# dwofk/fast-depth

Hardware: AMD Instinct MI355X
Metric: frames/sec (224x224) MobileNet-NNConv5dw-skipadd inference forward (higher is better)
Workload: dtype f32; 1 GPU; configs[1]: MobileNet-NNConv5(dw)+skipadd unpruned, batch=32 per GPU, 224x224 fp32 inference forward, inputs resident in HBM; batch_per_gpu=32, global_batch=32, parallelism=frames sharded over 1 GPU(s), no collective, rccl_ranks=0, input_batches_in_rotation=8

## Files before the change

### fast-depth_amd/csrc/fd_api.hip

```cpp
#include "fd_kernels_f32.h"
#include "fd_kernels_gemm16_f32.h"
#include "fd_kernels_h16.h"
#include "fd_kernels_gemm16_h16.h"
#include "fd_kernels_dwpw_f32.h"
#include "fd_kernels_dw5p.h"
#include "fd_kernels_dwt.h"
#include "fd_kernels_dws.h"
#include "fd_kernels_dwb.h"
#include "fd_kernels_conv.h"
#include "../../include/fastdepth_hip.h"
#include "fd_tuning.h"

#include <algorithm>
#include <cstdarg>
#include <cstdio>
#include <cstdlib>
#include <cstring>
#include <string>
#include <type_traits>
#include <vector>

#ifndef FD_EMU
#include <hip/hip_ext.h>
#endif

#define FD_DEFINE_HOST_STATE
#include "fd_host_common.h"
#include "fd_plan_select.h"
#include "fd_infer_launch.h"
#include "fd_plan_build.h"


extern "C" {

void fd_tuning_next(uint32_t mask) { fd_hs().tune_next = mask; }

const char *fd_last_error(void) { return fd_hs().err.c_str(); }
#ifndef FD_SOURCE_HASH
#define FD_SOURCE_HASH "unstamped"
#endif
const char *fd_version(void) { return "fastdepth_hip 0.5 (gfx950; inference f32/f16/bf16, train step f32/bf16; sources " FD_SOURCE_HASH ")"; }

int fd_plan_create(const fd_layer_desc *layers, int32_t n_layers, int32_t batch, int32_t height, int32_t width,
                   int32_t dtype, uint32_t flags, fd_plan **out_plan)
{
    const uint32_t tune = fd_take_tuning();
    if (!layers || !out_plan || n_layers <= 0) return fail(FD_ERR_INVALID, "null/empty layer list");
    if (batch <= 0 || height <= 0 || width <= 0 || height % 32 || width % 32)
        return fail(FD_ERR_INVALID, "batch must be > 0 and height/width positive multiples of 32 (got %d, %dx%d)", batch, height, width);
    if (dtype != FD_F32 && dtype != FD_F16 && dtype != FD_BF16) return fail(FD_ERR_INVALID, "unknown dtype %d", dtype);
    if (flags & ~FD_PLAN_ALL_FLAGS) return fail(FD_ERR_INVALID, "unknown plan flag bits 0x%x", flags & ~FD_PLAN_ALL_FLAGS);
    if (tune & ~FD_TUNE_ALL) return fail(FD_ERR_INVALID, "unknown tuning bits 0x%x", tune & ~FD_TUNE_ALL);
    fd_plan *p = new fd_plan();
    p->B = batch; p->H = height; p->W = width; p->dtype = dtype; p->flags = flags; p->tune = tune;
    p->layers.resize(n_layers);
    size_t woff = 0;
    int rc = plan_layers(p, layers, &woff);
    if (rc) { delete p; return rc; }
    p->weights_bytes = woff;
    plan_fuse_epilogues(p);
    plan_fuse_units(p);
    plan_fuse_head_h16(p);
    plan_arena(p, woff);
    plan_describe(p);
    *out_plan = p;
    return FD_OK;
}

void fd_plan_destroy(fd_plan *plan) { delete plan; }

size_t fd_plan_workspace_bytes(const fd_plan *plan) { return plan ? plan->ws_bytes : 0; }

int fd_plan_bind_workspace(fd_plan *plan, void *device_ptr, size_t bytes)
{
    if (!plan || !device_ptr) return fail(FD_ERR_INVALID, "null plan/workspace");
    if (bytes < plan->ws_bytes) return fail(FD_ERR_INVALID, "workspace too small: %zu < %zu", bytes, plan->ws_bytes);
    if (reinterpret_cast<uintptr_t>(device_ptr) % 256) return fail(FD_ERR_INVALID, "workspace must be 256-byte aligned");
    plan->ws = static_cast<unsigned char *>(device_ptr);
    plan->packed = false;
    return FD_OK;
}

int fd_plan_pack_weights(fd_plan *plan, const fd_layer_params *params, int32_t n_layers, float bn_eps, void *stream)
{
    if (!plan || !params) return fail(FD_ERR_INVALID, "null plan/params");
    if (!plan->ws) return fail(FD_ERR_STATE, "bind a workspace before packing weights");
    if (n_layers != (int)plan->layers.size()) return fail(FD_ERR_INVALID, "expected %zu layer parameter sets", plan->layers.size());
    hipStream_t s = static_cast<hipStream_t>(stream);
    for (int i = 0; i < n_layers; ++i) {
        const Layer &L = plan->layers[i];
        const fd_layer_params &q = params[i];
        if (!q.conv_weight || !q.bn_weight || !q.bn_bias || !q.bn_mean || !q.bn_var) return fail(FD_ERR_INVALID, "layer %d: null parameter pointer", i);
        if (L.conv) {
            const size_t cesz = plan->dtype == FD_F32 ? 4 : 2;
            const int kk = L.d.ksize * L.d.ksize, cpad = L.cv_ktpt * fd_conv_bk(cesz);
            const long upto = (long)(L.w_bytes / cesz);
            float *cb = reinterpret_cast<float *>(plan->ws + L.b_off);
            if (plan->dtype == FD_F16)
                hipLaunchKernelGGL((fd_conv_pack<fd_half>), dim3(ceil_div(upto, 256)), dim3(256), 0, s, q.conv_weight, q.bn_weight, q.bn_var, bn_eps, reinterpret_cast<fd_half *>(plan->ws + L.w_off), L.d.cout, L.d.cin, kk, cpad, upto);
            else if (plan->dtype == FD_BF16)
                hipLaunchKernelGGL((fd_conv_pack<fd_bf16>), dim3(ceil_div(upto, 256)), dim3(256), 0, s, q.conv_weight, q.bn_weight, q.bn_var, bn_eps, reinterpret_cast<fd_bf16 *>(plan->ws + L.w_off), L.d.cout, L.d.cin, kk, cpad, upto);
            else
                hipLaunchKernelGGL((fd_conv_pack<float>), dim3(ceil_div(upto, 256)), dim3(256), 0, s, q.conv_weight, q.bn_weight, q.bn_var, bn_eps, reinterpret_cast<float *>(plan->ws + L.w_off), L.d.cout, L.d.cin, kk, cpad, upto);
            int rcc = check_launch("fd_conv_pack");
            if (rcc) return rcc;
            hipLaunchKernelGGL(fd_dwt_fold_bias, dim3(ceil_div(L.d.cout, 256)), dim3(256), 0, s, q.bn_weight, q.bn_bias, q.bn_mean, q.bn_var, bn_eps, cb, L.d.cout);
            rcc = check_launch("fd_dwt_fold_bias");
            if (rcc) return rcc;
            continue;
        }
        const int inner = (int)(L.w_elems / L.d.cout);
        const int transpose = (L.d.op == FD_OP_PW) ? 0 : 1;
        const int pitch = transpose ? inner : (L.w_pitch ? L.w_pitch : inner);
        const long total = std::max<long>((long)L.d.cout * std::max(inner, pitch), L.d.cout);
        float *bptr = reinterpret_cast<float *>(plan->ws + L.b_off);
        if (L.pw_packed_t && plan->dtype == FD_F16)
            hipLaunchKernelGGL((fd_pack_fold<fd_half>), dim3(ceil_div(total, 256)), dim3(256), 0, s, q.conv_weight, q.bn_weight, q.bn_bias, q.bn_mean, q.bn_var, bn_eps,
                               reinterpret_cast<fd_half *>(plan->ws + L.w_off), bptr, L.d.cout, inner, transpose, pitch);
        else if (L.pw_packed_t)
            hipLaunchKernelGGL((fd_pack_fold<fd_bf16>), dim3(ceil_div(total, 256)), dim3(256), 0, s, q.conv_weight, q.bn_weight, q.bn_bias, q.bn_mean, q.bn_var, bn_eps,
                               reinterpret_cast<fd_bf16 *>(plan->ws + L.w_off), bptr, L.d.cout, inner, transpose, pitch);
        else
            hipLaunchKernelGGL((fd_pack_fold<float>), dim3(ceil_div(total, 256)), dim3(256), 0, s, q.conv_weight, q.bn_weight, q.bn_bias, q.bn_mean, q.bn_var, bn_eps,
                               reinterpret_cast<float *>(plan->ws + L.w_off), bptr, L.d.cout, inner, transpose, pitch);
        int rc = check_launch("fd_pack_fold");
        if (rc) return rc;
        if (L.dwt || L.dws || L.pws || L.dwb || L.pwb) {
            hipLaunchKernelGGL(fd_dwt_fold_bias, dim3(ceil_div(L.d.cout, 256)), dim3(256), 0, s, q.bn_weight, q.bn_bias, q.bn_mean, q.bn_var, bn_eps, bptr, L.d.cout);
            rc = check_launch("fd_dwt_fold_bias");
            if (rc) return rc;
        }
        if (L.dw5_cl) {
            const float *wf = reinterpret_cast<const float *>(plan->ws + L.w_off);
            unsigned *wpk = reinterpret_cast<unsigned *>(plan->ws + L.wpk_off);
            if (plan->dtype == FD_F16) hipLaunchKernelGGL((fd_pack_dw5_pairs<fd_half>), dim3(ceil_div(30L * L.d.cin, 256)), dim3(256), 0, s, wf, wpk, L.d.cin);
            else hipLaunchKernelGGL((fd_pack_dw5_pairs<fd_bf16>), dim3(ceil_div(30L * L.d.cin, 256)), dim3(256), 0, s, wf, wpk, L.d.cin);
            rc = check_launch("fd_pack_dw5_pairs");
            if (rc) return rc;
        }
    }
    plan->packed = true;
    return FD_OK;
}

int fd_forward(fd_plan *plan, const void *x_nchw, void *y, void *stream)
{
    if (!plan || !x_nchw || !y) return fail(FD_ERR_INVALID, "null argument");
    if (!plan->ws || !plan->packed) return fail(FD_ERR_STATE, "plan needs a bound workspace and packed weights");
    if (misaligned(x_nchw, 16)) return fail(FD_ERR_INVALID, "x must be 16-byte aligned");
    if (misaligned(y, 8)) return fail(FD_ERR_INVALID, "y must be 8-byte aligned");
    hipStream_t s = static_cast<hipStream_t>(stream);
    for (size_t i = 0; i < plan->layers.size(); ++i) {
        const Layer &L = plan->layers[i];
        if (L.skipped || L.fused_into >= 0) continue;
        fd_hs().trace_layer = (int)i;
        int rc = run_layer(plan, L, static_cast<const float *>(x_nchw), static_cast<float *>(y), s);
        if (rc) return rc;
    }
    fd_hs().trace_layer = -1;
    return FD_OK;
}

#include "fd_bundle_impl.h"

int fd_plan_shape(const fd_plan *plan, int32_t *batch, int32_t *height, int32_t *width, int32_t *dtype)
{
    if (!plan) return fail(FD_ERR_INVALID, "null plan");
    if (batch) *batch = plan->B;
    if (height) *height = plan->H;
    if (width) *width = plan->W;
    if (dtype) *dtype = plan->dtype;
    return FD_OK;
}

#include "fd_trace_impl.h"

int fd_layer_output(const fd_plan *plan, int32_t layer, const void **device_ptr, int32_t *n, int32_t *h, int32_t *w, int32_t *c)
{
    if (!plan || layer < 0 || layer >= (int)plan->layers.size()) return fail(FD_ERR_INVALID, "bad layer index");
    if (!(plan->flags & FD_PLAN_KEEP_ACTIVATIONS)) return fail(FD_ERR_STATE, "plan was not created with FD_PLAN_KEEP_ACTIVATIONS");
    const Layer &L = plan->layers[layer];
    if (L.to_output) return fail(FD_ERR_STATE, "the last layer writes the caller's output buffer");
    if (L.skipped) return fail(FD_ERR_STATE, "layer %d is fused into its consumer and has no stored output", layer);
    if (!plan->ws) return fail(FD_ERR_STATE, "no workspace bound");
    if (device_ptr) *device_ptr = plan->ws + L.out_off;
    if (n) *n = plan->B;
    if (h) *h = L.out_h;
    if (w) *w = L.out_w;
    if (c) *c = L.d.cout;
    return FD_OK;
}

int32_t fd_plan_num_kernels(const fd_plan *plan) { return plan ? (int32_t)plan->layers.size() : 0; }

const char *fd_plan_kernel_info(const fd_plan *plan, int32_t layer)
{
    if (!plan || layer < 0 || layer >= (int)plan->layers.size()) return "";
    return plan->layers[layer].info.c_str();
}

const char *fd_plan_kernel_symbol(const fd_plan *plan, int32_t layer)
{
    if (!plan || layer < 0 || layer >= (int)plan->layers.size()) return "";
    return plan->layers[layer].sym.c_str();
}

double fd_plan_algorithmic_bytes(const fd_plan *plan) { return plan ? plan->alg_bytes : 0.0; }
double fd_plan_algorithmic_flops(const fd_plan *plan) { return plan ? plan->alg_flops : 0.0; }

int fd_plan_layer_stats(const fd_plan *plan, int32_t layer, double *algorithmic_bytes, double *algorithmic_flops)
{
    if (!plan || layer < 0 || layer >= (int)plan->layers.size()) return fail(FD_ERR_INVALID, "bad layer index");
    const Layer &L = plan->layers[layer];
    double b = (L.skipped || L.fused_into >= 0) ? 0.0 : L.alg_bytes, f = (L.skipped || L.fused_into >= 0) ? 0.0 : L.alg_flops;
    if (L.fused_dw >= 0) { b += plan->layers[L.fused_dw].alg_bytes; f += plan->layers[L.fused_dw].alg_flops; }
    if (L.fuse_next_dw >= 0) { b += plan->layers[L.fuse_next_dw].alg_bytes; f += plan->layers[L.fuse_next_dw].alg_flops; }
    if (L.fuse_head >= 0) { b += plan->layers[L.fuse_head].alg_bytes; f += plan->layers[L.fuse_head].alg_flops; }
    if (algorithmic_bytes) *algorithmic_bytes = b;
    if (algorithmic_flops) *algorithmic_flops = f;
    return FD_OK;
}

int fd_plan_layer_traffic(const fd_plan *plan, int32_t layer, double *needed_bytes)
{
    if (!plan || layer < 0 || layer >= (int)plan->layers.size() || !needed_bytes) return fail(FD_ERR_INVALID, "bad layer index / null output");
    const Layer &L = plan->layers[layer];
    const double esz = plan->dtype == FD_F32 ? 4.0 : 2.0;
    auto out_b = [&](const Layer &X) { return (double)plan->B * X.out_h * X.out_w * X.d.cout * (X.to_output ? 4.0 : esz); };
    double b = (L.skipped || L.fused_into >= 0) ? 0.0 : L.alg_bytes;
    if (L.fused_dw >= 0) { const Layer &D = plan->layers[L.fused_dw]; b += D.alg_bytes - 2.0 * out_b(D); }
    if (L.fuse_next_dw >= 0) {
        const Layer &D = plan->layers[L.fuse_next_dw];
        b += D.alg_bytes - ((plan->flags & FD_PLAN_KEEP_ACTIVATIONS) ? 1.0 : 2.0) * out_b(L);
    }
    if (L.fuse_head >= 0) { const Layer &H = plan->layers[L.fuse_head]; b += H.alg_bytes - 2.0 * out_b(L); }
    *needed_bytes = b;
    return FD_OK;
}

}
```

### fast-depth_amd/csrc/fd_device.h

```cpp
#pragma once
#ifdef FD_EMU
#include "hipemu.h"
#else
#include <hip/hip_runtime.h>
#define FD_DYN_SMEM(name) extern __shared__ __attribute__((aligned(16))) unsigned char name[]
#endif

#ifdef FD_EMU
inline void fd_glds16(const float *g, float *lds_wave_base) { memcpy((char *)lds_wave_base + hipemu::lane_id() * 16, g, 16); }
template <int N> inline void fd_wait_vmcnt() {}
#define FD_SCHED_FENCE() ((void)0)
#define FD_UNIFORM(x) (x)
#define FD_OPAQUE(x) ((void)0)
#define FD_SCALAR_PTR(p) ((void)0)
template <typename P> inline P *fd_uniform_ptr(P *p) { return p; }
inline void fd_store_u32_sbase(char *base, unsigned off, unsigned v) { memcpy(base + off, &v, 4); }
inline void fd_block_barrier_lds() { __syncthreads(); }
inline void fd_block_barrier() { __syncthreads(); }
inline void fd_wave_lds_fence() { __syncthreads(); }
#else
__device__ __forceinline__ void fd_glds16(const float *g, float *lds_wave_base)
{
    __builtin_amdgcn_global_load_lds((const __attribute__((address_space(1))) void *)g,
                                     (__attribute__((address_space(3))) void *)lds_wave_base, 16, 0, 0);
}
template <int N> __device__ __forceinline__ void fd_wait_vmcnt() { asm volatile("s_waitcnt vmcnt(%0)" ::"n"(N) : "memory"); }
#define FD_SCHED_FENCE() __builtin_amdgcn_sched_barrier(0)
#define FD_UNIFORM(x) __builtin_amdgcn_readfirstlane(x)
#define FD_OPAQUE(x) asm volatile("" : "+v"(x))
#define FD_SCALAR_PTR(p) asm volatile("" : "+s"(p))
__device__ __forceinline__ void fd_store_u32_sbase(char *base, unsigned off, unsigned v)
{
    asm volatile("global_store_dword %0, %1, %2" : : "v"(off), "v"(v), "s"(base) : "memory");
}
template <typename P> __device__ __forceinline__ P *fd_uniform_ptr(P *p)
{
    const unsigned long long v = reinterpret_cast<unsigned long long>(p);
    const unsigned lo = __builtin_amdgcn_readfirstlane((unsigned)v), hi = __builtin_amdgcn_readfirstlane((unsigned)(v >> 32));
    return reinterpret_cast<P *>(((unsigned long long)hi << 32) | lo);
}
__device__ __forceinline__ void fd_wave_lds_fence() { asm volatile("s_waitcnt lgkmcnt(0)" ::: "memory"); }
__device__ __forceinline__ void fd_block_barrier() { __builtin_amdgcn_s_barrier(); }
__device__ __forceinline__ void fd_block_barrier_lds() { asm volatile("s_waitcnt lgkmcnt(0)" ::: "memory"); __builtin_amdgcn_s_barrier(); }
#endif

#ifdef FD_EMU
inline void fd_wave_fence() { (void)__shfl(0.0f, 0); }
inline void fd_wave_dma_wait() { (void)__shfl(0.0f, 0); }
#else
__device__ __forceinline__ void fd_wave_fence() { asm volatile("s_waitcnt lgkmcnt(0)" ::: "memory"); }
__device__ __forceinline__ void fd_wave_dma_wait() { asm volatile("s_waitcnt vmcnt(0)" ::: "memory"); }
#endif

struct fd_blk3 { int x, y, z; };
__device__ __forceinline__ fd_blk3 fd_xcd_map(unsigned b, unsigned per, unsigned nimg)
{
    const unsigned grp = b / (8u * per), rem = b - grp * 8u * per;
    const unsigned m = nimg - grp * 8u < 8u ? nimg - grp * 8u : 8u;
    fd_blk3 r;
    r.z = (int)(grp * 8u + rem % m); r.x = (int)(rem / m); r.y = 0;
    return r;
}
__device__ __forceinline__ fd_blk3 fd_xcd_image_map()
{
    const unsigned gx = gridDim.x, gy = gridDim.y;
    fd_blk3 r = fd_xcd_map(blockIdx.x + gx * (blockIdx.y + gy * blockIdx.z), gx * gy, gridDim.z);
    r.y = (int)((unsigned)r.x / gx); r.x -= r.y * (int)gx;
    return r;
}
__device__ __forceinline__ fd_blk3 fd_xcd_image_map2()
{
    return fd_xcd_map(blockIdx.x + gridDim.x * blockIdx.y, gridDim.x, gridDim.y);
}

template <int N> struct fd_int { static constexpr int value = N; };

__device__ __forceinline__ float fd_row_stride4_sum(float v)
{
#ifdef FD_EMU
    v += __shfl_xor(v, 8); v += __shfl_xor(v, 4);
#else
    v += __builtin_bit_cast(float, __builtin_amdgcn_update_dpp(0, __builtin_bit_cast(int, v), 0x128, 0xF, 0xF, true));
    v += __builtin_bit_cast(float, __builtin_amdgcn_update_dpp(0, __builtin_bit_cast(int, v), 0x124, 0xF, 0xF, true));
#endif
    return v;
}

typedef float fd_f32x4 __attribute__((ext_vector_type(4)));
typedef float fd_f32x2 __attribute__((ext_vector_type(2)));
typedef float fd_f32x16 __attribute__((ext_vector_type(16)));

#define FD_ACT_NONE_ 0
#define FD_ACT_RELU_ 1
#define FD_ACT_RELU6_ 2

__device__ __forceinline__ float fd_relu_clamp(float v, float hi) { return __builtin_elementwise_minimum(__builtin_elementwise_maximum(v, 0.0f), hi); }
template <int ACT>
__device__ __forceinline__ float fd_act(float v)
{
    if (ACT == FD_ACT_RELU_) return __builtin_elementwise_maximum(v, 0.0f);
    if (ACT == FD_ACT_RELU6_) return fd_relu_clamp(v, 6.0f);
    return v;
}
template <int ACT>
__device__ __forceinline__ float fd_act_raw(float v)
{
#ifdef FD_EMU
    return fd_act<ACT>(v);
#else
    float r = v;
    if (ACT == FD_ACT_RELU_) asm("v_maximum3_f32 %0, %1, 0, 0" : "=v"(r) : "v"(v));
    if (ACT == FD_ACT_RELU6_) { const float six = 6.0f; asm("v_maximum3_f32 %0, %1, 0, 0\n\tv_minimum3_f32 %0, %0, %2, %2" : "=&v"(r) : "v"(v), "s"(six)); }
    return r;
#endif
}
template <int ACT>
__device__ __forceinline__ fd_f32x4 fd_act4(fd_f32x4 v)
{
    fd_f32x4 r;
    r.x = fd_act<ACT>(v.x); r.y = fd_act<ACT>(v.y); r.z = fd_act<ACT>(v.z); r.w = fd_act<ACT>(v.w);
    return r;
}
__device__ __forceinline__ fd_f32x4 fd_ld4(const float *p) { return *reinterpret_cast<const fd_f32x4 *>(p); }
__device__ __forceinline__ void fd_st4(float *p, fd_f32x4 v) { *reinterpret_cast<fd_f32x4 *>(p) = v; }

typedef float fd_f32x2_t __attribute__((ext_vector_type(2)));
typedef _Float16 fd_half;
struct fd_bf16 { unsigned short v; };
typedef _Float16 fd_f16x4 __attribute__((ext_vector_type(4)));
typedef _Float16 fd_f16x8 __attribute__((ext_vector_type(8)));
typedef unsigned short fd_u16x4 __attribute__((ext_vector_type(4)));
typedef unsigned short fd_u16x8 __attribute__((ext_vector_type(8)));

__device__ __forceinline__ float fd_bf16_to_f32(unsigned short b) { return __builtin_bit_cast(float, (unsigned)b << 16); }
#ifdef FD_EMU
__device__ __forceinline__ unsigned short fd_f32_to_bf16(float f)
{
    unsigned u = __builtin_bit_cast(unsigned, f);
    if ((u & 0x7fffffffu) > 0x7f800000u) return (unsigned short)((u >> 16) | 0x40u);
    u += 0x7fffu + ((u >> 16) & 1u);
    return (unsigned short)(u >> 16);
}
__device__ __forceinline__ unsigned fd_f32x2_to_bf16x2(float a, float b) { return (unsigned)fd_f32_to_bf16(a) | ((unsigned)fd_f32_to_bf16(b) << 16); }
#else
__device__ __forceinline__ unsigned short fd_f32_to_bf16(float f) { return __builtin_bit_cast(unsigned short, (__bf16)f); }
__device__ __forceinline__ unsigned fd_f32x2_to_bf16x2(float a, float b)
{
    typedef __bf16 fd_bf16x2_hw __attribute__((ext_vector_type(2)));
    const fd_f32x2_t v = {a, b};
    return __builtin_bit_cast(unsigned, __builtin_convertvector(v, fd_bf16x2_hw));
}
#endif
__device__ __forceinline__ fd_f32x4 fd_ld4(const fd_half *p)
{
    const fd_f16x4 h = *reinterpret_cast<const fd_f16x4 *>(p);
    fd_f32x4 r = {(float)h.x, (float)h.y, (float)h.z, (float)h.w};
    return r;
}
__device__ __forceinline__ void fd_st4(fd_half *p, fd_f32x4 v)
{
    fd_f16x4 h = {(_Float16)v.x, (_Float16)v.y, (_Float16)v.z, (_Float16)v.w};
    *reinterpret_cast<fd_f16x4 *>(p) = h;
}
__device__ __forceinline__ fd_f32x4 fd_ld4(const fd_bf16 *p)
{
    const fd_u16x4 h = *reinterpret_cast<const fd_u16x4 *>(p);
    fd_f32x4 r = {fd_bf16_to_f32(h.x), fd_bf16_to_f32(h.y), fd_bf16_to_f32(h.z), fd_bf16_to_f32(h.w)};
    return r;
}
__device__ __forceinline__ void fd_st4(fd_bf16 *p, fd_f32x4 v)
{
    typedef unsigned fd_u32x2 __attribute__((ext_vector_type(2)));
    const fd_u32x2 h = {fd_f32x2_to_bf16x2(v.x, v.y), fd_f32x2_to_bf16x2(v.z, v.w)};
    *reinterpret_cast<fd_u32x2 *>(p) = h;
}
__device__ __forceinline__ fd_f32x4 fd_ldraw4(const float *p) { return *reinterpret_cast<const fd_f32x4 *>(p); }
#ifdef FD_EMU
inline fd_u16x4 fd_lds_read_tr16(const void *p)
{
    unsigned short o[4];
    hipemu_lds_read_tr16_b64(p, o);
    fd_u16x4 r = {o[0], o[1], o[2], o[3]};
    return r;
}
#else
__device__ __forceinline__ fd_u16x4 fd_lds_read_tr16(const void *p)
{
    typedef short fd_s16x4_hw __attribute__((ext_vector_type(4)));
    const fd_s16x4_hw v = __builtin_amdgcn_ds_read_tr16_b64_v4i16((__attribute__((address_space(3))) fd_s16x4_hw *)(p));
    return __builtin_bit_cast(fd_u16x4, v);
}
#endif
__device__ __forceinline__ fd_u16x4 fd_ldraw4(const fd_half *p) { return *reinterpret_cast<const fd_u16x4 *>(p); }
__device__ __forceinline__ fd_u16x4 fd_ldraw4(const fd_bf16 *p) { return *reinterpret_cast<const fd_u16x4 *>(p); }
__device__ __forceinline__ fd_f32x4 fd_cvt4(float, fd_f32x4 r) { return r; }
__device__ __forceinline__ fd_f32x4 fd_cvt4(fd_half, fd_u16x4 r)
{
    const fd_f16x4 h = __builtin_bit_cast(fd_f16x4, r);
    fd_f32x4 v = {(float)h.x, (float)h.y, (float)h.z, (float)h.w};
    return v;
}
__device__ __forceinline__ fd_f32x4 fd_cvt4(fd_bf16, fd_u16x4 r)
{
    fd_f32x4 v = {fd_bf16_to_f32(r.x), fd_bf16_to_f32(r.y), fd_bf16_to_f32(r.z), fd_bf16_to_f32(r.w)};
    return v;
}
__device__ __forceinline__ float fd_ld1(const float *p) { return *p; }
__device__ __forceinline__ float fd_ld1(const fd_half *p) { return (float)*p; }
__device__ __forceinline__ float fd_ld1(const fd_bf16 *p) { return fd_bf16_to_f32(p->v); }
__device__ __forceinline__ void fd_st1(float *p, float v) { *p = v; }
__device__ __forceinline__ void fd_st1(fd_half *p, float v) { *p = (_Float16)v; }
__device__ __forceinline__ void fd_st1(fd_bf16 *p, float v) { p->v = fd_f32_to_bf16(v); }
struct fd_px_walk {
    int iy, ix, dy, dx, w;
    __device__ __forceinline__ fd_px_walk(int start, int step, int w_) : w(w_) { iy = start / w_; ix = start - iy * w_; dy = step / w_; dx = step - dy * w_; }
    __device__ __forceinline__ void next() { ix += dx; iy += dy; if (ix >= w) { ix -= w; ++iy; } }
};
__device__ __forceinline__ fd_f32x4 fd_zero4() { fd_f32x4 z = {0.f, 0.f, 0.f, 0.f}; return z; }

#ifdef FD_EMU
inline unsigned fd_mul24(unsigned a, unsigned b) { return (a & 0xffffffu) * (b & 0xffffffu); }
#else
__device__ __forceinline__ unsigned fd_mul24(unsigned a, unsigned b) { return __umul24(a, b); }
#endif
__device__ __forceinline__ long fd_nhwc(int n, int H, int y, int W, int x, int C, int c)
{
    return (long)n * H * W * C + (long)(fd_mul24(fd_mul24((unsigned)y, (unsigned)W) + (unsigned)x, (unsigned)C) + (unsigned)c);
}

typedef float fd_f32x8 __attribute__((ext_vector_type(8)));
__device__ __forceinline__ fd_f32x8 fd_zero8() { fd_f32x8 z = {0.f, 0.f, 0.f, 0.f, 0.f, 0.f, 0.f, 0.f}; return z; }
__device__ __forceinline__ fd_f32x8 fd_cvt8(fd_half, fd_u16x8 r)
{
    const fd_f16x8 h = __builtin_bit_cast(fd_f16x8, r);
    fd_f32x8 v = {(float)h[0], (float)h[1], (float)h[2], (float)h[3], (float)h[4], (float)h[5], (float)h[6], (float)h[7]};
    return v;
}
__device__ __forceinline__ fd_f32x8 fd_cvt8(fd_bf16, fd_u16x8 r)
{
    typedef unsigned fd_u32x4_ __attribute__((ext_vector_type(4)));
    const fd_u32x4_ d = __builtin_bit_cast(fd_u32x4_, r);
    fd_f32x8 v = {__builtin_bit_cast(float, d[0] << 16), __builtin_bit_cast(float, d[0] & 0xffff0000u), __builtin_bit_cast(float, d[1] << 16), __builtin_bit_cast(float, d[1] & 0xffff0000u),
                  __builtin_bit_cast(float, d[2] << 16), __builtin_bit_cast(float, d[2] & 0xffff0000u), __builtin_bit_cast(float, d[3] << 16), __builtin_bit_cast(float, d[3] & 0xffff0000u)};
    return v;
}
__device__ __forceinline__ fd_u16x8 fd_pack8v(fd_half, fd_f32x8 v)
{
    fd_f16x8 h = {(_Float16)v[0], (_Float16)v[1], (_Float16)v[2], (_Float16)v[3], (_Float16)v[4], (_Float16)v[5], (_Float16)v[6], (_Float16)v[7]};
    return __builtin_bit_cast(fd_u16x8, h);
}
__device__ __forceinline__ fd_u16x8 fd_pack8v(fd_bf16, fd_f32x8 v)
{
    typedef unsigned fd_u32x4_ __attribute__((ext_vector_type(4)));
    const fd_u32x4_ r = {fd_f32x2_to_bf16x2(v[0], v[1]), fd_f32x2_to_bf16x2(v[2], v[3]), fd_f32x2_to_bf16x2(v[4], v[5]), fd_f32x2_to_bf16x2(v[6], v[7])};
    return __builtin_bit_cast(fd_u16x8, r);
}
__device__ __forceinline__ fd_u16x8 fd_sum8(fd_half, fd_u16x8 a, fd_u16x8 b)
{
    return __builtin_bit_cast(fd_u16x8, __builtin_bit_cast(fd_f16x8, a) + __builtin_bit_cast(fd_f16x8, b));
}
__device__ __forceinline__ fd_u16x8 fd_sum8(fd_bf16, fd_u16x8 a, fd_u16x8 b) { return fd_pack8v(fd_bf16{}, fd_cvt8(fd_bf16{}, a) + fd_cvt8(fd_bf16{}, b)); }
template <int ACT>
__device__ __forceinline__ fd_f32x8 fd_act4(fd_f32x8 v)
{
    fd_f32x8 r;
#pragma unroll
    for (int j = 0; j < 8; ++j) r[j] = fd_act<ACT>(v[j]);
    return r;
}
__device__ __forceinline__ fd_f32x4 fd_round4(float, fd_f32x4 v) { return v; }
__device__ __forceinline__ fd_f32x4 fd_round4(fd_bf16, fd_f32x4 v)
{
    fd_f32x4 r = {fd_bf16_to_f32(fd_f32_to_bf16(v.x)), fd_bf16_to_f32(fd_f32_to_bf16(v.y)), fd_bf16_to_f32(fd_f32_to_bf16(v.z)), fd_bf16_to_f32(fd_f32_to_bf16(v.w))};
    return r;
}
__device__ __forceinline__ fd_f32x4 fd_round4(fd_half, fd_f32x4 v)
{
    fd_f32x4 r = {(float)(_Float16)v.x, (float)(_Float16)v.y, (float)(_Float16)v.z, (float)(_Float16)v.w};
    return r;
}
template <typename T, int N> struct fd_lane;
template <typename T> struct fd_lane<T, 4> {
    static constexpr int n = 4;
    typedef fd_f32x4 vec;
    typedef float lds_t;
    typedef decltype(fd_ldraw4((const T *)nullptr)) raw;
    static __device__ __forceinline__ vec zero() { return fd_zero4(); }
    static __device__ __forceinline__ vec ld(const T *p) { return fd_ld4(p); }
    static __device__ __forceinline__ raw ldraw(const T *p) { return fd_ldraw4(p); }
    static __device__ __forceinline__ vec cvt(raw r) { return fd_cvt4(T{}, r); }
    static __device__ __forceinline__ void st(T *p, vec v) { fd_st4(p, v); }
    static __device__ __forceinline__ vec ldf(const float *p) { return fd_ld4(p); }
    static __device__ __forceinline__ void stf(float *p, vec v) { fd_st4(p, v); }
    static __device__ __forceinline__ vec lds_ld(const lds_t *p) { return fd_ld4(p); }
    static __device__ __forceinline__ void lds_st(lds_t *p, vec v) { fd_st4(p, v); }
    static __device__ __forceinline__ void lds_st_raw(lds_t *p, raw r) { fd_st4(p, fd_cvt4(T{}, r)); }
    static __device__ __forceinline__ void lds_st_sum(lds_t *p, raw a, raw b) { fd_st4(p, fd_cvt4(T{}, a) + fd_cvt4(T{}, b)); }
    static __device__ __forceinline__ vec round(vec v) { return fd_round4(T{}, v); }
    static __device__ __forceinline__ vec lds_round(vec v) { return v; }
};
template <typename T> struct fd_lane<T, 8> {
    static constexpr int n = 8;
    typedef fd_f32x8 vec;
    typedef T lds_t;
    typedef fd_u16x8 raw;
    static __device__ __forceinline__ vec zero() { return fd_zero8(); }
    static __device__ __forceinline__ raw ldraw(const T *p) { return *reinterpret_cast<const fd_u16x8 *>(p); }
    static __device__ __forceinline__ vec cvt(raw r) { return fd_cvt8(T{}, r); }
    static __device__ __forceinline__ vec ld(const T *p) { return cvt(ldraw(p)); }
    static __device__ __forceinline__ void st(T *p, vec v) { *reinterpret_cast<fd_u16x8 *>(p) = fd_pack8v(T{}, v); }
    static __device__ __forceinline__ vec ldf(const float *p)
    {
        const fd_f32x4 a = fd_ld4(p), b = fd_ld4(p + 4);
        vec v = {a.x, a.y, a.z, a.w, b.x, b.y, b.z, b.w};
        return v;
    }
    static __device__ __forceinline__ void stf(float *p, vec v)
    {
        const fd_f32x4 a = {v[0], v[1], v[2], v[3]}, b = {v[4], v[5], v[6], v[7]};
        fd_st4(p, a); fd_st4(p + 4, b);
    }
    static __device__ __forceinline__ vec lds_ld(const lds_t *p) { return cvt(*reinterpret_cast<const fd_u16x8 *>(p)); }
    static __device__ __forceinline__ void lds_st(lds_t *p, vec v) { *reinterpret_cast<fd_u16x8 *>(p) = fd_pack8v(T{}, v); }
    static __device__ __forceinline__ void lds_st_raw(lds_t *p, raw r) { *reinterpret_cast<fd_u16x8 *>(p) = r; }
    static __device__ __forceinline__ void lds_st_sum(lds_t *p, raw a, raw b) { *reinterpret_cast<fd_u16x8 *>(p) = fd_sum8(T{}, a, b); }
    static __device__ __forceinline__ vec round(vec v) { return cvt(fd_pack8v(T{}, v)); }
    static __device__ __forceinline__ vec lds_round(vec v) { return cvt(fd_pack8v(T{}, v)); }
};

#define FD_BUF_OOB 0x80000000u
#ifdef FD_EMU
struct fd_bufrsrc { char *base; unsigned bytes; };
inline fd_bufrsrc fd_make_rsrc(const void *p, unsigned bytes) { fd_bufrsrc r = {const_cast<char *>(static_cast<const char *>(p)), bytes}; return r; }
inline unsigned fd_buf_ld32(fd_bufrsrc r, unsigned voff, unsigned soff)
{
    if (voff >= r.bytes || (unsigned long long)voff + soff + 4 > r.bytes) return 0u;
    unsigned v; memcpy(&v, r.base + voff + soff, 4); return v;
}
inline void fd_buf_st32(fd_bufrsrc r, unsigned voff, unsigned soff, unsigned v)
{
    if (voff >= r.bytes || (unsigned long long)voff + soff + 4 > r.bytes) return;
    memcpy(r.base + voff + soff, &v, 4);
}
#else
typedef __amdgpu_buffer_rsrc_t fd_bufrsrc;
__device__ __forceinline__ fd_bufrsrc fd_make_rsrc(const void *p, unsigned bytes) { return __builtin_amdgcn_make_buffer_rsrc(const_cast<void *>(p), 0, (int)bytes, 0x00020000); }
__device__ __forceinline__ unsigned fd_buf_ld32(fd_bufrsrc r, unsigned voff, unsigned soff) { return __builtin_amdgcn_raw_buffer_load_b32(r, (int)voff, (int)soff, 0); }
__device__ __forceinline__ void fd_buf_st32(fd_bufrsrc r, unsigned voff, unsigned soff, unsigned v) { __builtin_amdgcn_raw_buffer_store_b32(v, r, (int)voff, (int)soff, 0); }
#endif
#ifdef FD_EMU
inline unsigned fd_perm(unsigned s0, unsigned s1, unsigned sel)
{
    const unsigned long long cat = ((unsigned long long)s0 << 32) | s1;
    unsigned r = 0;
    for (int k = 0; k < 4; ++k) r |= (unsigned)((cat >> (8 * ((sel >> (8 * k)) & 7u))) & 0xffu) << (8 * k);
    return r;
}
inline float fd_h16_bits_to_f32(unsigned short b) { return (float)__builtin_bit_cast(_Float16, b); }
inline float fd_dot2(fd_half, unsigned a, unsigned b, float c)
{
    return (float)((double)fd_h16_bits_to_f32((unsigned short)a) * fd_h16_bits_to_f32((unsigned short)b) +
                   (double)fd_h16_bits_to_f32((unsigned short)(a >> 16)) * fd_h16_bits_to_f32((unsigned short)(b >> 16)) + (double)c);
}
inline float fd_dot2(fd_bf16, unsigned a, unsigned b, float c)
{
    return (float)((double)fd_bf16_to_f32((unsigned short)a) * fd_bf16_to_f32((unsigned short)b) +
                   (double)fd_bf16_to_f32((unsigned short)(a >> 16)) * fd_bf16_to_f32((unsigned short)(b >> 16)) + (double)c);
}
#else
__device__ __forceinline__ unsigned fd_perm(unsigned s0, unsigned s1, unsigned sel) { return __builtin_amdgcn_perm(s0, s1, sel); }
__device__ __forceinline__ float fd_dot2(fd_half, unsigned a, unsigned b, float c)
{
    typedef _Float16 fd_h2_hw __attribute__((ext_vector_type(2)));
    return __builtin_amdgcn_fdot2(__builtin_bit_cast(fd_h2_hw, a), __builtin_bit_cast(fd_h2_hw, b), c, false);
}
__device__ __forceinline__ float fd_dot2(fd_bf16, unsigned a, unsigned b, float c)
{
    typedef __bf16 fd_b2_hw __attribute__((ext_vector_type(2)));
    return __builtin_amdgcn_fdot2_f32_bf16(__builtin_bit_cast(fd_b2_hw, a), __builtin_bit_cast(fd_b2_hw, b), c, false);
}
#endif
#ifdef FD_EMU
template <int N> inline void fd_dot2_done(float (&)[N][2]) {}
#else
template <int N> __device__ __forceinline__ void fd_dot2_done(float (&acc)[N][2])
{
    asm volatile("s_nop 4" ::: "memory");
#pragma unroll
    for (int i = 0; i < N; ++i) { asm volatile("" : "+v"(acc[i][0])); asm volatile("" : "+v"(acc[i][1])); }
}
#endif
#ifdef FD_EMU
template <typename T> inline void fd_dot2_acc(T, unsigned a, unsigned b, float &acc) { acc = fd_dot2(T{}, a, b, acc); }
template <typename T> inline float fd_dot2_first(T, unsigned a, unsigned b, float c) { return fd_dot2(T{}, a, b, c); }
#else
__device__ __forceinline__ void fd_dot2_acc(fd_half, unsigned a, unsigned b, float &acc) { asm volatile("v_dot2c_f32_f16 %0, %1, %2" : "+v"(acc) : "v"(a), "v"(b)); }
__device__ __forceinline__ void fd_dot2_acc(fd_bf16, unsigned a, unsigned b, float &acc) { asm volatile("v_dot2c_f32_bf16 %0, %1, %2" : "+v"(acc) : "v"(a), "v"(b)); }
__device__ __forceinline__ float fd_dot2_first(fd_half, unsigned a, unsigned b, float c)
{
    float r;
    asm volatile("v_dot2_f32_f16 %0, %1, %2, %3" : "=v"(r) : "v"(a), "v"(b), "v"(c));
    return r;
}
__device__ __forceinline__ float fd_dot2_first(fd_bf16, unsigned a, unsigned b, float c)
{
    float r;
    asm volatile("v_dot2_f32_bf16 %0, %1, %2, %3" : "=v"(r) : "v"(a), "v"(b), "v"(c));
    return r;
}
#endif
#define FD_PERM_LO 0x05040100u
#define FD_PERM_HI 0x07060302u
__device__ __forceinline__ unsigned fd_pack2(fd_half, float a, float b)
{
    typedef _Float16 fd_h2_ __attribute__((ext_vector_type(2)));
    const fd_h2_ h = {(_Float16)a, (_Float16)b};
    return __builtin_bit_cast(unsigned, h);
}
__device__ __forceinline__ unsigned fd_pack2(fd_bf16, float a, float b) { return fd_f32x2_to_bf16x2(a, b); }
__device__ __forceinline__ unsigned fd_pair_sum(fd_half, unsigned a, unsigned b)
{
    typedef _Float16 fd_h2_ __attribute__((ext_vector_type(2)));
    return __builtin_bit_cast(unsigned, __builtin_bit_cast(fd_h2_, a) + __builtin_bit_cast(fd_h2_, b));
}
__device__ __forceinline__ unsigned fd_pair_sum(fd_bf16, unsigned a, unsigned b)
{
    return fd_f32x2_to_bf16x2(__builtin_bit_cast(float, a << 16) + __builtin_bit_cast(float, b << 16),
                              __builtin_bit_cast(float, a & 0xffff0000u) + __builtin_bit_cast(float, b & 0xffff0000u));
}

#define FD_STAT_BINS 3
#define FD_STAT_MAX_ROWS 16
#define FD_STAT_MAX_PARTIALS (1L << 15)
#define FD_STAT_FWD 0
#define FD_STAT_BWD 1
struct fd_stat_rows { long long *rows; int nr, cs; };
#ifdef FD_EMU
inline void fd_atomic_add_i64(long long *p, long long v) { *p = (long long)((unsigned long long)*p + (unsigned long long)v); }
inline void fd_atomic_or_i64(long long *p, long long v) { *p |= v; }
#else
__device__ __forceinline__ void fd_atomic_add_i64(long long *p, long long v)
{
    (void)__hip_atomic_fetch_add(p, v, __ATOMIC_RELAXED, __HIP_MEMORY_SCOPE_AGENT);
}
__device__ __forceinline__ void fd_atomic_or_i64(long long *p, long long v)
{
    (void)__hip_atomic_fetch_or(p, v, __ATOMIC_RELAXED, __HIP_MEMORY_SCOPE_AGENT);
}
#endif
template <int DIR> struct fd_stat_fmt {
    static constexpr int lo = DIR == FD_STAT_FWD ? -8 : -32, hi = DIR == FD_STAT_FWD ? 16 : -8;
    static constexpr int f0 = DIR == FD_STAT_FWD ? 56 : 80, f1 = f0 - 24, f2 = f0 - 48;
};
__device__ __forceinline__ long fd_stat_flag_index(int nr, int cs, int which, int c) { return ((long)nr * FD_STAT_BINS * 2 + which) * cs + c; }
template <int DIR>
__device__ __forceinline__ void fd_stat_add(const fd_stat_rows &d, long blk, int , int which, int c, float v)
{
    typedef fd_stat_fmt<DIR> F;
    const unsigned u = __builtin_bit_cast(unsigned, v);
    int e = (int)((u >> 23) & 255u) - 127;
    if (e == -127) return;
    if (e == 128) {
        fd_atomic_or_i64(d.rows + fd_stat_flag_index(d.nr, d.cs, which, c), 1);
        return;
    }
    const int bin = e < F::lo ? 0 : (e < F::hi ? 1 : 2);
    const int frac = bin == 0 ? F::f0 : (bin == 1 ? F::f1 : F::f2);
    if (e > 47 - frac) e = 47 - frac;
    const long long m = (long long)((u & 0x7fffffu) | 0x800000u);
    const int sh = e + frac - 23;
    long long iv = sh >= 0 ? (m << sh) : (sh > -24 ? (m >> -sh) : 0);
    if (u >> 31) iv = -iv;
    if (iv == 0) return;
    fd_atomic_add_i64(d.rows + ((((long)(blk & (d.nr - 1)) * FD_STAT_BINS + bin) * 2 + which) * d.cs + c), iv);
}
template <int DIR>
__device__ __forceinline__ double fd_stat_total(const long long *__restrict__ rows, int nr, int C , int which, int c, int r0, int rstep)
{
    typedef fd_stat_fmt<DIR> F;
    long long a0 = 0, a1 = 0, a2 = 0;
    for (int r = r0; r < nr; r += rstep) {
        const long long *p = rows + (((long)r * FD_STAT_BINS) * 2 + which) * C + c;
        a0 += p[0]; a1 += p[2 * (long)C]; a2 += p[4 * (long)C];
    }
    const double t = ldexp((double)a0, -F::f0) + ldexp((double)a1, -F::f1) + ldexp((double)a2, -F::f2);
    return (r0 == 0 && rows[fd_stat_flag_index(nr, C, which, c)] != 0) ? __builtin_nan("") : t;
}

#ifdef FD_EMU
inline int fd_atomic_inc(int *p) { int o = *p; *p = o + 1; return o; }
inline void fd_store_dev(float *p, float v) { *p = v; }
inline float fd_load_dev(const float *p) { return *p; }
inline void fd_store_dev(int *p, int v) { *p = v; }
inline void fd_store_dev(double *p, double v) { *p = v; }
inline double fd_load_dev(const double *p) { return *p; }
inline void fd_release_wg() {}
inline void fd_acquire_wg() {}
#else
__device__ __forceinline__ int fd_atomic_inc(int *p) { return __hip_atomic_fetch_add(p, 1, __ATOMIC_RELAXED, __HIP_MEMORY_SCOPE_AGENT); }
__device__ __forceinline__ void fd_store_dev(float *p, float v) { __hip_atomic_store(p, v, __ATOMIC_RELAXED, __HIP_MEMORY_SCOPE_AGENT); }
__device__ __forceinline__ float fd_load_dev(const float *p) { return __hip_atomic_load(p, __ATOMIC_RELAXED, __HIP_MEMORY_SCOPE_AGENT); }
__device__ __forceinline__ void fd_store_dev(int *p, int v) { __hip_atomic_store(p, v, __ATOMIC_RELAXED, __HIP_MEMORY_SCOPE_AGENT); }
__device__ __forceinline__ void fd_store_dev(double *p, double v) { __hip_atomic_store(p, v, __ATOMIC_RELAXED, __HIP_MEMORY_SCOPE_AGENT); }
__device__ __forceinline__ double fd_load_dev(const double *p) { return __hip_atomic_load(p, __ATOMIC_RELAXED, __HIP_MEMORY_SCOPE_AGENT); }
__device__ __forceinline__ void fd_release_wg() { asm volatile("s_waitcnt vmcnt(0)" ::: "memory"); }
__device__ __forceinline__ void fd_acquire_wg() { asm volatile("" ::: "memory"); }
#endif
```

### fast-depth_amd/csrc/fd_infer_launch.h

```cpp
#pragma once
namespace {

template <typename T, int ACT>
int launch_stem(const Layer &L, const float *x, const float *wp, const float *bias, T *y, int B, hipStream_t s)
{
    switch (L.chunk) {
    case 32: FD_LAUNCH((fd_stem3x3s2<T, ACT, 32>), L.grid, dim3(256), L.lds, s, x, wp, bias, y, B, L.in_h, L.in_w, L.d.cout); break;
    case 16: FD_LAUNCH((fd_stem3x3s2<T, ACT, 16>), L.grid, dim3(256), L.lds, s, x, wp, bias, y, B, L.in_h, L.in_w, L.d.cout); break;
    default: FD_LAUNCH((fd_stem3x3s2<T, ACT, 8>), L.grid, dim3(256), L.lds, s, x, wp, bias, y, B, L.in_h, L.in_w, L.d.cout); break;
    }
    return check_launch("fd_stem3x3s2");
}

template <typename T, int K, int S, int MODE, int ACT>
int launch_dw_inst(const Layer &L, const T *in, const T *skip, const float *wp, const float *bias, T *out, hipStream_t s)
{
    if constexpr (!std::is_same<T, float>::value) {
        if (L.dw_n == 8) {
            FD_LAUNCH((fd_dwconv<T, K, S, MODE, ACT, 8>), L.grid, dim3(256), L.lds, s, in, skip, wp, bias, out,
                      L.in_h, L.in_w, L.out_h, L.out_w, L.d.cin, L.cbq, L.th, L.tw, L.tiles_x, L.csplit, L.pstr);
            return check_launch("fd_dwconv");
        }
    }
    FD_LAUNCH((fd_dwconv<T, K, S, MODE, ACT, 4>), L.grid, dim3(256), L.lds, s, in, skip, wp, bias, out,
                       L.in_h, L.in_w, L.out_h, L.out_w, L.d.cin, L.cbq, L.th, L.tw, L.tiles_x, L.csplit, L.pstr);
    return check_launch("fd_dwconv");
}

template <typename T, int ACT>
int launch_dw(const Layer &L, const T *in, const T *skip, const float *wp, const float *bias, T *out, hipStream_t s, const unsigned *wpk = nullptr)
{
    if (L.dw5_cl) {
        if constexpr (!std::is_same<T, float>::value) {
            if (L.dw5_cl == 64)
                FD_LAUNCH((fd_dw5_rows<T, ACT, 64>), L.grid, dim3(FD_DW5R_BLOCK), 0, s, in, skip, wpk, bias, out, L.in_h, L.in_w, L.d.cin, L.dw5_cbs, L.dw5_groups, L.dw5_bh);
            else
                FD_LAUNCH((fd_dw5_rows<T, ACT, 32>), L.grid, dim3(FD_DW5R_BLOCK), 0, s, in, skip, wpk, bias, out, L.in_h, L.in_w, L.d.cin, L.dw5_cbs, L.dw5_groups, L.dw5_bh);
            return check_launch("fd_dw5_rows");
        }
        return fail(FD_ERR_INVALID, "fd_dw5_rows is a 16-bit kernel");
    }
    if (L.dw_rows && L.dw_rows8) {
        if constexpr (!std::is_same<T, float>::value) {
            if (L.d.stride == 1)
                FD_LAUNCH((fd_dw3_rows8<T, 1, ACT>), L.grid, dim3(256), 0, s, in, wp, bias, out, L.in_h, L.in_w, L.out_h, L.out_w, L.d.cin, L.th);
            else
                FD_LAUNCH((fd_dw3_rows8<T, 2, ACT>), L.grid, dim3(256), 0, s, in, wp, bias, out, L.in_h, L.in_w, L.out_h, L.out_w, L.d.cin, L.th);
            return check_launch("fd_dw3_rows8");
        }
    }
    if (L.dw_rows) {
        if (L.d.stride == 1)
            FD_LAUNCH((fd_dw3_rows<T, 1, ACT>), L.grid, dim3(256), 0, s, in, wp, bias, out, L.in_h, L.in_w, L.out_h, L.out_w, L.d.cin, L.th);
        else
            FD_LAUNCH((fd_dw3_rows<T, 2, ACT>), L.grid, dim3(256), 0, s, in, wp, bias, out, L.in_h, L.in_w, L.out_h, L.out_w, L.d.cin, L.th);
        return check_launch("fd_dw3_rows");
    }
    const int key = L.d.ksize * 100 + L.d.stride * 10 + L.mode;
    switch (key) {
    case 310: return launch_dw_inst<T, 3, 1, 0, ACT>(L, in, skip, wp, bias, out, s);
    case 320: return launch_dw_inst<T, 3, 2, 0, ACT>(L, in, skip, wp, bias, out, s);
    case 510: return launch_dw_inst<T, 5, 1, 0, ACT>(L, in, skip, wp, bias, out, s);
    case 511: return launch_dw_inst<T, 5, 1, 1, ACT>(L, in, skip, wp, bias, out, s);
    case 512: return launch_dw_inst<T, 5, 1, 2, ACT>(L, in, skip, wp, bias, out, s);
    case 311: return launch_dw_inst<T, 3, 1, 1, ACT>(L, in, skip, wp, bias, out, s);
    case 312: return launch_dw_inst<T, 3, 1, 2, ACT>(L, in, skip, wp, bias, out, s);
    case 513: return launch_dw_inst<T, 5, 1, 3, ACT>(L, in, skip, wp, bias, out, s);
    }
    return fail(FD_ERR_INVALID, "depthwise k=%d stride=%d mode=%d has no kernel", L.d.ksize, L.d.stride, L.mode);
}

template <typename T, int ACT>
int launch_dwt(const Layer &L, const T *in, const float *wp, const float *bias, T *out, hipStream_t s)
{
    if (L.d.ksize == 5) FD_LAUNCH((fd_dwt_rows<T, 5, ACT>), L.grid, dim3(256), 0, s, in, wp, bias, out, L.in_h, L.in_w, L.d.cin, L.th);
    else FD_LAUNCH((fd_dwt_rows<T, 3, ACT>), L.grid, dim3(256), 0, s, in, wp, bias, out, L.in_h, L.in_w, L.d.cin, L.th);
    return check_launch("fd_dwt_rows");
}

template <typename T, int ACT>
int launch_dws(const Layer &L, const T *in, const float *wp, const float *bias, T *out, hipStream_t s)
{
    if (L.d.ksize == 5) FD_LAUNCH((fd_dws_rows<T, 5, ACT>), L.grid, dim3(256), 0, s, in, wp, bias, out, L.in_h / 2, L.in_w / 2, L.d.cin, L.th);
    else FD_LAUNCH((fd_dws_rows<T, 3, ACT>), L.grid, dim3(256), 0, s, in, wp, bias, out, L.in_h / 2, L.in_w / 2, L.d.cin, L.th);
    return check_launch("fd_dws_rows");
}

template <typename T, int ACT>
int launch_dwb(const Layer &L, const T *in, const float *wp, const float *bias, T *out, hipStream_t s)
{
    if (L.d.ksize == 5) FD_LAUNCH((fd_dwb_rows<T, 5, ACT>), L.grid, dim3(256), 0, s, in, wp, bias, out, L.in_h / 2, L.in_w / 2, L.d.cin, L.th);
    else FD_LAUNCH((fd_dwb_rows<T, 3, ACT>), L.grid, dim3(256), 0, s, in, wp, bias, out, L.in_h / 2, L.in_w / 2, L.d.cin, L.th);
    return check_launch("fd_dwb_rows");
}

template <typename T>
int launch_conv(const fd_plan *p, const Layer &L, const T *in, T *out, hipStream_t s)
{
    fd_conv_geo g{};
    g.H = L.out_h; g.W = L.out_w; g.up = L.d.upsample ? 1 : 0; g.ks = L.d.ksize; g.cin = L.d.cin; g.cout = L.d.cout;
    g.ktpt = L.cv_ktpt; g.m_tiles = L.m_tiles; g.n_tiles = L.n_tiles; g.tps = L.cv_tps;
    g.act = L.d.act == FD_ACT_RELU6 ? FD_ACT_RELU6_ : (L.d.act == FD_ACT_RELU ? FD_ACT_RELU_ : FD_ACT_NONE_);
    const long Ml = (long)p->B * L.out_h * L.out_w;
    const int M = (int)Ml;
    const T *wp = reinterpret_cast<const T *>(p->ws + L.w_off), *zero = reinterpret_cast<const T *>(p->ws + L.zero_off);
    const float *bias = reinterpret_cast<const float *>(p->ws + L.b_off);
    float *part = L.cv_splits > 1 ? reinterpret_cast<float *>(p->ws + p->conv_part_off) : nullptr;
    const bool split = L.cv_splits > 1;
    hipEvent_t ev0 = fd_hs().ev_start, ev1 = fd_hs().ev_stop;
    if (split && ev0) fd_hs().ev_stop = nullptr;
#define FD_CONV_CASE(a, b, c, d) \
    case a * 1000 + b * 100 + c * 10 + d: \
        if (L.lds > 64 * 1024) (void)hipFuncSetAttribute((const void *)fd_conv_gemm<T, a, b, c, d>, hipFuncAttributeMaxDynamicSharedMemorySize, (int)L.lds); \
        FD_LAUNCH((fd_conv_gemm<T, a, b, c, d>), L.grid, dim3(256), L.lds, s, in, wp, zero, bias, out, part, M, g); break;
    switch (L.cv_wgm * 1000 + L.cv_wgn * 100 + L.cv_tm * 10 + L.cv_tn) {
        FD_CONV_CASE(2, 2, 2, 2)
        FD_CONV_CASE(2, 2, 1, 1)
        FD_CONV_CASE(4, 1, 1, 1)
    default: fd_hs().ev_stop = ev1; return fail(FD_ERR_INVALID, "no fd_conv_gemm tile %dx%dx%dx%d", L.cv_wgm, L.cv_wgn, L.cv_tm, L.cv_tn);
    }
#undef FD_CONV_CASE
    fd_hs().ev_stop = ev1;
    int rc = check_launch("fd_conv_gemm");
    if (rc || !split) return rc;
    const long total = Ml * L.d.cout;
    if (ev0) fd_hs().ev_start = nullptr;
#ifndef FD_EMU
    if (ev0 && !fd_hs().trace_on)
        hipExtLaunchKernelGGL((fd_conv_reduce<T>), dim3(ceil_div(total / 4, 256)), dim3(256), 0, s, nullptr, ev1, 0, part, out, total, L.cv_splits, g.act);
    else
#endif
        FD_LAUNCH((fd_conv_reduce<T>), dim3(ceil_div(total / 4, 256)), dim3(256), 0, s, part, out, total, L.cv_splits, g.act);
    fd_hs().ev_start = ev0;
    return check_launch("fd_conv_reduce");
}

template <int ACT>
int launch_pw(const fd_plan *plan, const Layer &L, const float *A, const float *wp, const float *bias, float *out, long M, hipStream_t s)
{
    const int N = L.d.cout, K = L.d.cin;
    if (L.pw16_tm) {
        fd_dwfuse fz{};
        int fdw = 0;
        if (L.fuse_next_dw >= 0) {
            const Layer &D = plan->layers[L.fuse_next_dw];
            fz.w = reinterpret_cast<const float *>(plan->ws + D.w_off); fz.b = reinterpret_cast<const float *>(plan->ws + D.b_off);
            fz.out = reinterpret_cast<float *>(plan->ws + D.out_off);
            fz.H = L.out_h; fz.W = L.out_w; fz.S = D.d.stride; fz.up = D.d.upsample;
            fz.hi = D.d.act == FD_ACT_RELU6 ? 6.0f : __builtin_inff();
            fz.store_pw = (plan->flags & FD_PLAN_KEEP_ACTIVATIONS) ? 1 : 0;
            fdw = D.d.ksize;
        }
        constexpr int BR = FD_G16_STAGES == 4 ? 1 : 0;
#define FD_PW16_LAUNCH(TMV, FD_, BREGV) \
        do { (void)hipFuncSetAttribute((const void *)fd_pw_gemm16_f32<TMV, FD_G16_STAGES, ACT, 0, FD_, 0, BREGV>, hipFuncAttributeMaxDynamicSharedMemorySize, (int)L.lds); \
             FD_LAUNCH((fd_pw_gemm16_f32<TMV, FD_G16_STAGES, ACT, 0, FD_, 0, BREGV>), L.grid, dim3(512), L.lds, s, A, wp, bias, out, (int)M, N, K, L.w_pitch, L.pw16_stride, L.m_tiles, L.n_tiles, fz, fd_g16_train{}); } while (0)
#define FD_PW16_FDW(TMV, BREGV) \
        do { if (fdw == 3) FD_PW16_LAUNCH(TMV, 3, BREGV); else if (fdw == 5) FD_PW16_LAUNCH(TMV, 5, BREGV); else FD_PW16_LAUNCH(TMV, 0, BREGV); } while (0)
#define FD_PW16_CASE(TMV) \
    case TMV: if (L.pw16_breg) FD_PW16_FDW(TMV, BR); else FD_PW16_FDW(TMV, 0); break;
        switch (L.pw16_tm) {
        case 13: FD_PW16_FDW(13, 0); break;
            FD_PW16_CASE(7)
            FD_PW16_CASE(4)
        default: return fail(FD_ERR_INVALID, "no gemm16 instance for TM=%d", L.pw16_tm);
        }
#undef FD_PW16_CASE
#undef FD_PW16_FDW
#undef FD_PW16_LAUNCH
        return check_launch("fd_pw_gemm16_f32");
    }
    const int key = L.pw.wgm * 1000 + L.pw.wgn * 100 + L.pw.tm * 10 + L.pw.tn;
#define FD_PW_CASE(a, b, c, d) \
    case a * 1000 + b * 100 + c * 10 + d: \
        if (L.lds > 64 * 1024) (void)hipFuncSetAttribute((const void *)fd_pw_gemm_f32<a, b, c, d, ACT>, hipFuncAttributeMaxDynamicSharedMemorySize, (int)L.lds); \
        FD_LAUNCH((fd_pw_gemm_f32<a, b, c, d, ACT>), L.grid, dim3(256), L.lds, s, A, wp, bias, out, (int)M, N, K, L.w_pitch, L.m_tiles, L.n_tiles); break;
    switch (key) {
        FD_PW_CASE(2, 2, 2, 2)
        FD_PW_CASE(2, 2, 2, 1)
        FD_PW_CASE(2, 2, 1, 2)
        FD_PW_CASE(2, 2, 1, 1)
        FD_PW_CASE(4, 1, 1, 1)
    default: return fail(FD_ERR_INVALID, "no pointwise tile %d", key);
    }
#undef FD_PW_CASE
    return check_launch("fd_pw_gemm_f32");
}



template <int ACT>
int launch_dwpw(const fd_plan *p, const Layer &L, float *out, float *y, hipStream_t s)
{
    const Layer &D = p->layers[L.fused_dw];
    const float *din = reinterpret_cast<const float *>(p->ws + p->layers[D.d.src].out_off);
    const float *dskip = D.d.skip >= 0 ? reinterpret_cast<const float *>(p->ws + p->layers[D.d.skip].out_off) : nullptr;
    const float *wdw = reinterpret_cast<const float *>(p->ws + D.w_off), *bdw = reinterpret_cast<const float *>(p->ws + D.b_off);
    const float *wp = reinterpret_cast<const float *>(p->ws + L.w_off), *bias = reinterpret_cast<const float *>(p->ws + L.b_off);
    fd_dwpw_head hd{};
    if (L.fuse_head >= 0) {
        const Layer &H = p->layers[L.fuse_head];
        hd.w = reinterpret_cast<const float *>(p->ws + H.w_off); hd.b = reinterpret_cast<const float *>(p->ws + H.b_off);
        hd.y = y; hd.act = H.d.act == FD_ACT_RELU6 ? 2 : (H.d.act == FD_ACT_RELU ? 1 : 0); hd.up = H.d.upsample;
    }
    const int key = D.d.ksize * 1000 + D.d.stride * 100 + D.mode * 10 + L.dp_nt + (L.fuse_head >= 0 ? 10000 : 0);
#define FD_DWPW_CASE(KSV, SV, MODEV, WMV, NTV, NLDV, HEADV)                                                                            \
    case KSV * 1000 + SV * 100 + MODEV * 10 + NTV + HEADV * 10000:                                                                     \
        (void)hipFuncSetAttribute((const void *)fd_dwpw_f32<KSV, SV, MODEV, ACT, WMV, NTV, NLDV, HEADV>, hipFuncAttributeMaxDynamicSharedMemorySize, (int)L.lds); \
        FD_LAUNCH((fd_dwpw_f32<KSV, SV, MODEV, ACT, WMV, NTV, NLDV, HEADV>), L.grid, dim3(512), L.lds, s, din, dskip, wdw, bdw, wp, bias, out, p->B, D.in_h, D.in_w, \
                  D.out_h, D.out_w, D.d.cin, L.w_pitch, L.d.cout, L.dp_th, L.dp_tw, L.dp_tiles_x, L.dp_tiles_x * ceil_div(D.out_h, L.dp_th), L.dp_xcd, L.pstr, hd);  \
        break;
    switch (key) {
        FD_DWPW_CASE(3, 1, 0, 4, 1, 6, 0)
        FD_DWPW_CASE(3, 1, 0, 4, 2, 6, 0)
        FD_DWPW_CASE(3, 1, 0, 4, 4, 6, 0)
        FD_DWPW_CASE(5, 1, 2, 4, 1, 8, 0)
        FD_DWPW_CASE(5, 1, 2, 4, 1, 8, 1)
        FD_DWPW_CASE(5, 1, 2, 4, 2, 8, 0)
        FD_DWPW_CASE(5, 1, 2, 4, 4, 8, 0)
        FD_DWPW_CASE(3, 2, 0, 2, 2, 10, 0)
        FD_DWPW_CASE(3, 2, 0, 2, 4, 10, 0)
    default: return fail(FD_ERR_INVALID, "no fd_dwpw_f32 instance %d", key);
    }
#undef FD_DWPW_CASE
    return check_launch("fd_dwpw_f32");
}

template <int ACT>
int launch_pw_t(const fd_plan *plan, const Layer &L, const float *A, const void *wp, const float *bias, float *out, long M, hipStream_t s, float * = nullptr)
{
    return launch_pw<ACT>(plan, L, A, static_cast<const float *>(wp), bias, out, M, s);
}
template <int ACT, typename T>
int launch_pw_t(const fd_plan *plan, const Layer &L, const T *A, const void *wp, const float *bias, T *out, long M, hipStream_t s, float *y = nullptr)
{
    const int K = L.d.cin;
    if (L.pw16_tm) {
        fd_dwfuse fz{};
        int fdw = 0;
        if (L.fuse_next_dw >= 0) {
            const Layer &D = plan->layers[L.fuse_next_dw];
            fz.w = reinterpret_cast<const float *>(plan->ws + D.w_off); fz.b = reinterpret_cast<const float *>(plan->ws + D.b_off);
            fz.out = reinterpret_cast<float *>(plan->ws + D.out_off);
            fz.H = L.out_h; fz.W = L.out_w; fz.S = D.d.stride; fz.up = D.d.upsample;
            fz.hi = D.d.act == FD_ACT_RELU6 ? 6.0f : __builtin_inff();
            fz.store_pw = (plan->flags & FD_PLAN_KEEP_ACTIVATIONS) ? 1 : 0;
            fdw = D.d.ksize;
        }
#define FD_PW16H_LAUNCH(TMV, FD_) \
        do { (void)hipFuncSetAttribute((const void *)fd_pw_gemm16_h16<T, TMV, 4, ACT, FD_>, hipFuncAttributeMaxDynamicSharedMemorySize, (int)L.lds); \
             FD_LAUNCH((fd_pw_gemm16_h16<T, TMV, 4, ACT, FD_>), L.grid, dim3(512), L.lds, s, A, static_cast<const T *>(wp), bias, out, (int)M, L.d.cout, K, L.w_pitch, L.pw16_stride, L.m_tiles, L.n_tiles, fz, 0 ); } while (0)
#define FD_PW16H_CASE(TMV) \
    case TMV: if (fdw == 3) FD_PW16H_LAUNCH(TMV, 3); else if (fdw == 5) FD_PW16H_LAUNCH(TMV, 5); else FD_PW16H_LAUNCH(TMV, 0); break;
        switch (L.pw16_tm) {
            FD_PW16H_CASE(13)
            FD_PW16H_CASE(7)
            FD_PW16H_CASE(4)
        default: return fail(FD_ERR_INVALID, "no 16-bit gemm16 instance for TM=%d", L.pw16_tm);
        }
#undef FD_PW16H_CASE
#undef FD_PW16H_LAUNCH
        return check_launch("fd_pw_gemm16_h16");
    }
    if (L.fuse_head >= 0) {
        const Layer &H = plan->layers[L.fuse_head];
        fd_pw_head hd{};
        hd.w = reinterpret_cast<const float *>(plan->ws + H.w_off); hd.b = reinterpret_cast<const float *>(plan->ws + H.b_off);
        hd.y = y; hd.act = H.d.act == FD_ACT_RELU6 ? 2 : (H.d.act == FD_ACT_RELU ? 1 : 0); hd.up = H.d.upsample; hd.h = L.out_h; hd.w_ = L.out_w;
        FD_LAUNCH((fd_pw_gemm_head_h16<T, ACT>), L.grid, dim3(256), L.lds, s, A, static_cast<const T *>(wp), bias, (int)M, L.d.cout, K, (K + 63) / 64 * 64,
                  L.m_tiles, L.n_tiles, hd);
        return check_launch("fd_pw_gemm_head_h16");
    }
    FD_LAUNCH((fd_pw_gemm_h16<T, ACT>), L.grid, dim3(256), L.lds, s, A, static_cast<const T *>(wp), bias, out, (int)M, L.d.cout, K, (K + 63) / 64 * 64,
              L.m_tiles, L.n_tiles);
    return check_launch("fd_pw_gemm_h16");
}

template <typename T, int ACT>
int launch_layer(const fd_plan *p, const Layer &L, const float *x, float *y, hipStream_t s)
{
    const void *wp = p->ws + L.w_off;
    const float *wpf = reinterpret_cast<const float *>(p->ws + L.w_off);
    const float *bias = reinterpret_cast<const float *>(p->ws + L.b_off);
    T *out = reinterpret_cast<T *>(p->ws + L.out_off);
    const T *in = L.d.src < 0 ? nullptr : reinterpret_cast<const T *>(p->ws + p->layers[L.d.src].out_off);
    const T *skip = L.d.skip >= 0 ? reinterpret_cast<const T *>(p->ws + p->layers[L.d.skip].out_off) : nullptr;
    switch (L.d.op) {
    case FD_OP_STEM: return launch_stem<T, ACT>(L, x, wpf, bias, out, p->B, s);
    case FD_OP_DW: return launch_dw<T, ACT>(L, in, skip, wpf, bias, out, s, L.dw5_cl ? reinterpret_cast<const unsigned *>(p->ws + L.wpk_off) : nullptr);
    case FD_OP_DWT: return launch_dwt<T, ACT>(L, in, wpf, bias, out, s);
    case FD_OP_CONV: return launch_conv<T>(p, L, in, out, s);
    case FD_OP_DWS: return launch_dws<T, ACT>(L, in, wpf, bias, out, s);
    case FD_OP_PWS:
        FD_LAUNCH((fd_head_shuffle<T, ACT>), L.grid, dim3(256), 0, s, in, wpf, bias, y, (long)p->B * L.out_h * L.out_w, L.out_h, L.out_w, L.d.cin);
        return check_launch("fd_head_shuffle");
    case FD_OP_DWB: return launch_dwb<T, ACT>(L, in, wpf, bias, out, s);
    case FD_OP_PWB:
        FD_LAUNCH((fd_head_bilinear<T, ACT>), L.grid, dim3(256), 0, s, in, wpf, bias, y, L.in_h, L.in_w, L.d.cin);
        return check_launch("fd_head_bilinear");
    case FD_OP_PW:
        if (L.head) {
            const int h = L.d.upsample ? L.in_h / 2 : L.in_h, w = L.d.upsample ? L.in_w / 2 : L.in_w;
            const long npix = (long)p->B * h * w;
            FD_LAUNCH((fd_head_pw1<T, ACT>), L.grid, dim3(256), 0, s, in, wpf, bias, y, npix, h, w, L.d.cin, L.d.upsample);
            return check_launch("fd_head_pw1");
        }
        if (L.dwpw) {
            if constexpr (std::is_same<T, float>::value) return launch_dwpw<ACT>(p, L, out, y, s);
            else return fail(FD_ERR_INVALID, "fused units are fp32 only");
        }
        return launch_pw_t<ACT>(p, L, in, wp, bias, out, (long)p->B * L.out_h * L.out_w, s, y);
    }
    return fail(FD_ERR_INVALID, "bad op");
}

template <typename T>
int run_layer_t(fd_plan *plan, const Layer &L, const float *x, float *out, hipStream_t s)
{
    switch (L.d.act) {
    case FD_ACT_RELU: return launch_layer<T, FD_ACT_RELU_>(plan, L, x, out, s);
    case FD_ACT_RELU6: return launch_layer<T, FD_ACT_RELU6_>(plan, L, x, out, s);
    default: return launch_layer<T, FD_ACT_NONE_>(plan, L, x, out, s);
    }
}
int run_layer(fd_plan *plan, const Layer &L, const float *x, float *out, hipStream_t s)
{
    switch (plan->dtype) {
    case FD_F16: return run_layer_t<fd_half>(plan, L, x, out, s);
    case FD_BF16: return run_layer_t<fd_bf16>(plan, L, x, out, s);
    default: return run_layer_t<float>(plan, L, x, out, s);
    }
}

}
```

### fast-depth_amd/csrc/fd_kernels_gemm16_f32.h

```cpp
#pragma once
#include "fd_device.h"
#include "fd_bn_stats.h"

struct fd_dwfuse {
    const float *w;
    const float *b;
    float *out;
    int H, W;
    int S, up;
    float hi;
    int store_pw;
};

#ifdef FD_GEMM16_PROBE
__device__ long long fd_gemm16_probe[8 * 4096];
#endif

#ifndef FD_G16_TRAIN_AHEAD
#define FD_G16_TRAIN_AHEAD 2
#endif
struct fd_g16_train {
    const float *st;
    fd_stat_rows sr;
    fd_bn_fin fin;
};

template <int TM, int STAGES, int ACT, int ABL = 0, int FDW = 0, int TRAIN = 0, int BREG = 0>
__global__ void __launch_bounds__(512)
fd_pw_gemm16_f32(const float *__restrict__ A, const float *__restrict__ Wt, const float *__restrict__ bias,
                 float *__restrict__ out, int M, int N, int K, int K32, int m_stride, int m_tiles, int n_tiles, const fd_dwfuse fz, const fd_g16_train tr)
{
    static_assert(TRAIN == 0 || (FDW == 0 && ACT == 0), "train mode: raw output, no fused consumer");
    static_assert(BREG == 0 || (STAGES == 4 && (ABL == 0 || ABL == 4) && TRAIN == 0), "the register ring of the weight fragments is written for 4 stages, inference only (and has no K-loop ablations)");
    constexpr int BM = TM * 16, BN = 64, BK = 32, ROWS = BM + (BREG ? 0 : BN);
    constexpr int STAGE = ROWS * BK;
    constexpr int NG = ROWS / 8;
    constexpr int RG = (NG + 3) / 4;
    constexpr int OP = BN + 4;
    static_assert(STAGES * STAGE >= BM * OP + (TRAIN != 0 ? 8 * 2 * 64 : 0), "the output tile image (+ the statistics scratch) must fit the ring");
    FD_DYN_SMEM(smem_raw);
    float *smem = reinterpret_cast<float *>(smem_raw);
    const int tid = threadIdx.x, lane = tid & 63, wave = tid >> 6;
    const int wn = wave & 3, kh = wave >> 2;
    const int xcd = blockIdx.x & 7, slot = blockIdx.x >> 3;
    const int nt = slot % n_tiles, mt = (slot / n_tiles) * 8 + xcd;
    if (mt >= m_tiles) return;
    const long m0 = (long)mt * m_stride;
    const int n0 = nt * BN;
    const bool leader = kh == 0;
#ifdef FD_GEMM16_PROBE
    long long pc0 = 0, pw0 = 0, pc1 = 0;
    if (tid == 0) { pc0 = clock64(); pw0 = wall_clock64(); }
#endif

    const int wn_u = FD_UNIFORM(wn);
    unsigned src_off[RG];
#pragma unroll
    for (int i = 0; i < RG; ++i) {
        int g = wn_u + 4 * i;
        if (g >= NG) g = wn_u;
        const int r = g * 8 + (lane >> 3);
        const int chunk4 = ((lane & 7) ^ ((r >> 1) & 7)) * 4;
        if (r < BM) { long row = m0 + r; if (row > M - 1) row = M - 1; src_off[i] = (unsigned)((row * K + chunk4) * 4); }
        else { int row = n0 + (r - BM); if (row > N - 1) row = N - 1; src_off[i] = (unsigned)(((long)row * K32 + chunk4) * 4); }
    }
    const bool ragged_k = K != K32;
    auto piece = [&](int t, int i) {
        int g = wn_u + 4 * i;
        if (g >= NG) g = wn_u;
        const bool is_a = BREG != 0 || g < BM / 8;
        const char *base = reinterpret_cast<const char *>(is_a ? A : Wt) + (size_t)t * (BK * 4);
        const char *p = base + src_off[i];
        if (ragged_k && is_a && t == K32 / BK - 1) {
            const int chunk4 = ((lane & 7) ^ (((g * 8 + (lane >> 3)) >> 1) & 7)) * 4;
            if (t * BK + chunk4 >= K) p -= (t * BK + chunk4) * 4;
        }
        fd_glds16(reinterpret_cast<const float *>(p), smem + (t % STAGES) * STAGE + g * 8 * BK);
    };

    const int col = n0 + wn * 16 + (lane & 15);
    const float bv = (TRAIN == 0 && leader && col < N) ? bias[col] : 0.0f;
    fd_f32x4 acc[TM];
#pragma unroll
    for (int i = 0; i < TM; ++i) { acc[i].x = bv; acc[i].y = bv; acc[i].z = bv; acc[i].w = bv; }

    const int chunk = kh * 4 + (lane >> 4);
    const int a_off0 = (lane & 15) * BK + ((chunk ^ (((lane & 15) >> 1) & 7)) << 2);
    const int rowb = BM + wn * 16 + (lane & 15);
    const int b_off = rowb * BK + ((chunk ^ ((rowb >> 1) & 7)) << 2);

    const int T = K32 / BK;
    const float *b_src = Wt + (long)(col < N ? col : N - 1) * K32 + chunk * 4;
    auto b_load = [&](int t) { return fd_ld4(b_src + (size_t)t * BK); };

    fd_f32x4 fa[2][TM], fb[BREG ? STAGES : 2];
    float *tab = smem + STAGES * STAGE;
    fd_f32x4 sv[2], tv[2];
    constexpr int TABQ = 2;
    float tsc[TABQ], tsh[TABQ];
    if (TRAIN != 0 && !tr.fin.rows) {
#pragma unroll
        for (int j = 0; j < TABQ; ++j) {
            const int k = tid + 512 * j, kc = k < K ? k : 0;
            const float a = tr.st[kc], b = tr.st[K + kc];
            tsc[j] = k < K ? a : 0.0f; tsh[j] = k < K ? b : 0.0f;
        }
    }
    auto step = [&](auto buf, auto role, int t, auto mode) __attribute__((always_inline)) {
        constexpr int FB = decltype(buf)::value, B = BREG ? (FB & 1) : FB, MODE = decltype(mode)::value;
        constexpr bool LEAD = decltype(role)::value != 0;
        constexpr int NDMA = LEAD ? RG : 0, NL = NDMA + TM + (BREG ? 0 : 1), SP = (4 * TM) / NL;
        static_assert(SP >= 1, "not enough MFMA slots for the loads");
        static_assert(MODE == 0 || BREG != 0, "the LDS form decides everything at run time");
        const bool do_frags = MODE == 1 || (MODE >= 2 && MODE < 5) || (MODE == 0 && ABL != 2 && ABL != 3 && t + 1 < T);
        const bool do_dma = MODE == 1 || (MODE == 0 && ABL != 1 && ABL != 2 && ABL != 3 && t + STAGES < T);
        if (BREG && MODE == 1) {
            if (LEAD) fd_wait_vmcnt<(STAGES - 2) * (RG + 1)>();
            fd_block_barrier_lds();
        } else if (BREG && MODE >= 2) {
            if (MODE < 5) { if (LEAD) fd_wait_vmcnt<(MODE < 5 ? 4 - MODE : 0) * (RG + 1)>(); fd_block_barrier_lds(); }
        } else if (ABL != 3 && t + 1 < T) {
            if (LEAD && BREG) { if (t + STAGES - 1 < T) fd_wait_vmcnt<(STAGES - 2) * (RG + 1)>(); else fd_wait_vmcnt<0>(); }
            else if (LEAD) { if ((ABL == 0 || ABL == 4) && t + STAGES - 1 < T) fd_wait_vmcnt<(STAGES - 2) * RG>(); else fd_wait_vmcnt<0>(); }
            fd_block_barrier_lds();
        }
        const float *nxa = smem + ((t + 1) % STAGES) * STAGE + a_off0, *nxb = smem + ((t + 1) % STAGES) * STAGE + b_off;
        if (TRAIN != 0 && do_frags) { sv[1 - B] = fd_ld4(tab + (t + 1) * BK + chunk * 4); tv[1 - B] = fd_ld4(tab + K32 + (t + 1) * BK + chunk * 4); }
#pragma unroll
        for (int idx = 0; idx < 4 * TM; ++idx) {
            const int q = idx / TM, i = idx % TM;
            if (TRAIN != 0 && idx == 0) {
#pragma unroll
                for (int j = 0; j < FD_G16_TRAIN_AHEAD && j < TM; ++j) fa[B][j] = fd_act4<TRAIN>(fa[B][j] * sv[B] + tv[B]);
            }
            if (TRAIN != 0 && q == 0 && i + FD_G16_TRAIN_AHEAD < TM) fa[B][i + FD_G16_TRAIN_AHEAD] = fd_act4<TRAIN>(fa[B][i + FD_G16_TRAIN_AHEAD] * sv[B] + tv[B]);
            acc[i] = __builtin_amdgcn_mfma_f32_16x16x4f32(fa[B][i][q], fb[FB][q], acc[i], 0, 0, 0);
            if ((idx + 1) % SP == 0) {
                const int l = (idx + 1) / SP - 1;
                if (l < NDMA) {
                    if (do_dma) piece(t + STAGES, l);
                } else if (l < NDMA + TM) {
                    if (do_frags) fa[1 - B][l - NDMA] = fd_ld4(nxa + (l - NDMA) * 16 * BK);
                } else if (!BREG && l == NDMA + TM) {
                    if (do_frags) fb[1 - B] = fd_ld4(nxb);
                }
            }
        }
        if (BREG) {
            FD_SCHED_FENCE();
            if (do_dma) fb[FB] = b_load(t + STAGES);
            FD_SCHED_FENCE();
        }
    };
    auto first_frags = [&]() __attribute__((always_inline)) {
        if (TRAIN != 0) {
            if (tr.fin.rows) {
                if (!leader) fd_stat_table_all<256>(tr.fin, K, K32, tid - 256, blockIdx.x == 0, [&](int k, float a, float b) { tab[k] = a; tab[K32 + k] = b; });
            } else {
#pragma unroll
                for (int j = 0; j < TABQ; ++j) { const int k = tid + 512 * j; if (k < K32) { tab[k] = tsc[j]; tab[K32 + k] = tsh[j]; } }
            }
            fd_block_barrier_lds();
        } else {
            fd_block_barrier();
        }
#pragma unroll
        for (int i = 0; i < TM; ++i) fa[0][i] = fd_ld4(smem + a_off0 + i * 16 * BK);
        if (!BREG) fb[0] = fd_ld4(smem + b_off);
        if (TRAIN != 0) { sv[0] = fd_ld4(tab + chunk * 4); tv[0] = fd_ld4(tab + K32 + chunk * 4); }
#ifdef FD_GEMM16_PROBE
        if (tid == 0) pc1 = clock64();
#endif
    };

    if constexpr (BREG != 0) {
        auto run = [&](auto role) __attribute__((always_inline)) {
            constexpr bool LEAD = decltype(role)::value != 0;
            auto rest = [&](int t0) __attribute__((always_inline)) {
                for (int t = t0; t < T; t += 4) {
                    step(fd_int<0>{}, role, t, fd_int<0>{});
                    if (t + 1 < T) step(fd_int<1>{}, role, t + 1, fd_int<0>{});
                    if (t + 2 < T) step(fd_int<2>{}, role, t + 2, fd_int<0>{});
                    if (t + 3 < T) step(fd_int<3>{}, role, t + 3, fd_int<0>{});
                }
            };
            if (T >= 2 * STAGES) {
#pragma unroll
                for (int s = 0; s < STAGES; ++s) {
                    fb[s] = b_load(s);
                    FD_SCHED_FENCE();
                    if (LEAD) {
#pragma unroll
                        for (int i = 0; i < RG; ++i) piece(s, i);
                    }
                    FD_SCHED_FENCE();
                }
                if (LEAD) fd_wait_vmcnt<(STAGES - 1) * (RG + 1)>();
                first_frags();
#ifndef FD_EMU
                if (LEAD) __builtin_amdgcn_s_setprio(1);
#endif
                int t = 0;
                for (; t + 2 * STAGES <= T; t += 4) {
                    step(fd_int<0>{}, role, t, fd_int<1>{});
                    step(fd_int<1>{}, role, t + 1, fd_int<1>{});
                    step(fd_int<2>{}, role, t + 2, fd_int<1>{});
                    step(fd_int<3>{}, role, t + 3, fd_int<1>{});
                }
                if (T - t == 4) {
                    step(fd_int<0>{}, role, t, fd_int<2>{});
                    step(fd_int<1>{}, role, t + 1, fd_int<3>{});
                    step(fd_int<2>{}, role, t + 2, fd_int<4>{});
                    step(fd_int<3>{}, role, t + 3, fd_int<5>{});
                } else {
                    rest(t);
                }
            } else {
#pragma unroll
                for (int s = 0; s < STAGES; ++s)
                    if (s < T) {
                        fb[s] = b_load(s);
                        FD_SCHED_FENCE();
                        if (LEAD) {
#pragma unroll
                            for (int i = 0; i < RG; ++i) piece(s, i);
                        }
                        FD_SCHED_FENCE();
                    }
                if (LEAD) { if (T >= STAGES) fd_wait_vmcnt<(STAGES - 1) * (RG + 1)>(); else fd_wait_vmcnt<0>(); }
                first_frags();
#ifndef FD_EMU
                if (LEAD) __builtin_amdgcn_s_setprio(1);
#endif
                rest(0);
            }
#ifndef FD_EMU
            if (LEAD) __builtin_amdgcn_s_setprio(0);
#endif
        };
        if (leader) run(fd_int<1>{}); else run(fd_int<0>{});
    } else {
        if (leader) {
#pragma unroll
            for (int s = 0; s < STAGES; ++s)
                if (s < T) {
#pragma unroll
                    for (int i = 0; i < RG; ++i) piece(s, i);
                }
            if (T >= STAGES) fd_wait_vmcnt<(STAGES - 1) * RG>(); else fd_wait_vmcnt<0>();
        }
        first_frags();
        if (leader) {
#ifndef FD_EMU
            __builtin_amdgcn_s_setprio(1);
#endif
            for (int t = 0; t < T; t += 2) {
                step(fd_int<0>{}, fd_int<1>{}, t, fd_int<0>{});
                if (t + 1 < T) step(fd_int<1>{}, fd_int<1>{}, t + 1, fd_int<0>{});
            }
#ifndef FD_EMU
            __builtin_amdgcn_s_setprio(0);
#endif
        } else {
            for (int t = 0; t < T; t += 2) {
                step(fd_int<0>{}, fd_int<0>{}, t, fd_int<0>{});
                if (t + 1 < T) step(fd_int<1>{}, fd_int<0>{}, t + 1, fd_int<0>{});
            }
        }
    }
#ifdef FD_GEMM16_PROBE
    long long pc2 = 0;
    if (tid == 0) pc2 = clock64();
#endif

    constexpr int H = (TM + 1) / 2;
    constexpr int KD = FDW == 0 ? 1 : FDW;
    __shared__ int rowmap[FDW != 0 ? BM : 1];
    int rows = M - m0 < m_stride ? (int)(M - m0) : m_stride;
    if (rows > BM) rows = BM;
    const int fH = fz.H, fW = fz.W, fHW = fH * fW, us = (FDW != 0 && fz.up) ? 1 : 0;
    const int P = FDW == 0 ? 0 : (us ? (KD / 2 + 1) / 2 : KD / 2);
    const int PW = fW + 2 * P, PHW = (fH + 2 * P) * PW;
    const int frames = FDW != 0 ? rows / fHW : 0;
    fd_block_barrier_lds();
    if (FDW != 0) {
        const int img_rows = frames * PHW + 1;
        for (int i = tid; i < img_rows * (OP / 4); i += 512) fd_st4(smem + i * 4, fd_zero4());
        for (int t = tid; t < BM; t += 512) {
            const int fr = t / fHW, rem = t - fr * fHW, y = rem / fW, x = rem - y * fW;
            rowmap[t] = fr < frames ? fr * PHW + (y + P) * PW + (x + P) : frames * PHW;
        }
        __syncthreads();
    }
    int prow[TM][4];
#pragma unroll
    for (int i = 0; i < TM; ++i)
#pragma unroll
        for (int r = 0; r < 4; ++r) {
            const int t = i * 16 + 4 * (lane >> 4) + r;
            prow[i][r] = FDW != 0 ? rowmap[t] : t;
        }
    float *img = smem + wn * 16 + (lane & 15);
#pragma unroll
    for (int i = 0; i < TM; ++i) {
        const bool mine = leader ? i < H : i >= H;
        if (!mine) {
#pragma unroll
            for (int r = 0; r < 4; ++r) img[prow[i][r] * OP] = acc[i][r];
        }
    }
    __syncthreads();
#pragma unroll
    for (int i = 0; i < TM; ++i) {
        const bool mine = leader ? i < H : i >= H;
        if (mine) {
#pragma unroll
            for (int r = 0; r < 4; ++r) { float *o = img + prow[i][r] * OP; o[0] = fd_act<ACT>(acc[i][r] + o[0]); }
        }
    }
    __syncthreads();
#ifdef FD_GEMM16_PROBE
    if (tid == 0) { long long *pr = fd_gemm16_probe + 8 * blockIdx.x; pr[0] = pc0; pr[1] = clock64(); pr[2] = pw0; pr[3] = wall_clock64(); pr[4] = pc1; pr[5] = pc2; }
#endif
    if (ABL == 4) return;
    const int c4 = (lane & 15) * 4;
    if ((FDW == 0 || fz.store_pw) && n0 + c4 < N) {
        for (int r = wave * 4 + (lane >> 4); r < rows; r += 32)
            fd_st4(out + (m0 + r) * N + n0 + c4, fd_ld4(smem + (FDW != 0 ? rowmap[r] : r) * OP + c4));
    }
    if (TRAIN != 0) {
        float *red = smem + BM * OP;
        const int c = tid & 63, g = tid >> 6;
        float ssum = 0.0f, ssq = 0.0f;
        for (int r = g; r < rows; r += 8) { const float v = smem[r * OP + c]; ssum += v; ssq = fmaf(v, v, ssq); }
        red[(g * 2 + 0) * 64 + c] = ssum; red[(g * 2 + 1) * 64 + c] = ssq;
        __syncthreads();
        if (tid < 64 && n0 + tid < N) {
            float a = 0.0f, b = 0.0f;
#pragma unroll
            for (int gg = 0; gg < 8; ++gg) { a += red[(gg * 2 + 0) * 64 + tid]; b += red[(gg * 2 + 1) * 64 + tid]; }
            fd_stat_add<FD_STAT_FWD>(tr.sr, mt, N, 0, n0 + tid, a);
            fd_stat_add<FD_STAT_FWD>(tr.sr, mt, N, 1, n0 + tid, b);
        }
    }
    if (FDW != 0) {
        constexpr int PD = KD / 2;
        const int cg = tid & 15, pl = tid >> 4;
        const int c = n0 + cg * 4;
        if (c >= N) return;
        fd_f32x4 wv[KD * KD];
#pragma unroll
        for (int t = 0; t < KD * KD; ++t) wv[t] = fd_ld4(fz.w + (long)t * N + c);
        const fd_f32x4 b4 = fd_ld4(fz.b + c);
        const int S = fz.S;
        const int Ho = (fH << us) / S, Wo = (fW << us) / S, HWo = Ho * Wo;
        const long f0 = m0 / fHW;
        const int dy = 32 / Wo, dx = 32 - dy * Wo;
        for (int fr = 0; fr < frames; ++fr) {
            const float *img_f = smem + (long)fr * PHW * OP + cg * 4;
            int oy = pl / Wo, ox = pl - oy * Wo;
            for (int op = pl; op < HWo; op += 32) {
                fd_f32x4 a4 = b4;
                if (us) {
                    int ry[KD], rx[KD];
#pragma unroll
                    for (int k = 0; k < KD; ++k) { ry[k] = (((oy - PD + k) >> 1) + P) * PW; rx[k] = ((ox - PD + k) >> 1) + P; }
#pragma unroll
                    for (int ky = 0; ky < KD; ++ky)
#pragma unroll
                        for (int kx = 0; kx < KD; ++kx) a4 += fd_ld4(img_f + (ry[ky] + rx[kx]) * OP) * wv[ky * KD + kx];
                } else {
                    const float *p0 = img_f + ((oy * S) * PW + ox * S) * OP;
#pragma unroll
                    for (int ky = 0; ky < KD; ++ky)
#pragma unroll
                        for (int kx = 0; kx < KD; ++kx) a4 += fd_ld4(p0 + (ky * PW + kx) * OP) * wv[ky * KD + kx];
                }
                fd_f32x4 r4;
                r4.x = fd_relu_clamp(a4.x, fz.hi); r4.y = fd_relu_clamp(a4.y, fz.hi);
                r4.z = fd_relu_clamp(a4.z, fz.hi); r4.w = fd_relu_clamp(a4.w, fz.hi);
                fd_st4(fz.out + ((f0 + fr) * HWo + op) * N + c, r4);
                ox += dx; oy += dy;
                if (ox >= Wo) { ox -= Wo; ++oy; }
            }
        }
    }
#ifdef FD_GEMM16_PROBE
    if (tid == 0) fd_gemm16_probe[8 * blockIdx.x + 6] = clock64();
#endif
}
```

### fast-depth_amd/csrc/fd_plan_build.h

```cpp
#pragma once
namespace {

int plan_layers(fd_plan *p, const fd_layer_desc *layers, size_t *woff_out)
{
    const size_t esz = p->dtype == FD_F32 ? 4 : 2;
    const int n_layers = (int)p->layers.size(), batch = p->B, height = p->H, width = p->W, dtype = p->dtype;
    const uint32_t flags = p->flags, tune = p->tune;
    (void)n_layers; (void)batch; (void)height; (void)width; (void)dtype; (void)flags; (void)tune;
    size_t woff = 0;
    for (int i = 0; i < n_layers; ++i) {
        Layer &L = p->layers[i];
        L.d = layers[i];
        const fd_layer_desc &d = L.d;
#define FD_BAD(...) do { return fail(FD_ERR_INVALID, __VA_ARGS__); } while (0)
        if (d.src >= i || d.skip >= i) FD_BAD("layer %d: src/skip must reference earlier layers", i);
        if (d.act < FD_ACT_NONE || d.act > FD_ACT_RELU6) FD_BAD("layer %d: bad activation", i);
        if (d.cin <= 0 || d.cout <= 0) FD_BAD("layer %d: bad channel counts", i);
        int src_h, src_w, src_c;
        if (d.src < 0) { src_h = height; src_w = width; src_c = 3; }
        else { const Layer &S = p->layers[d.src]; src_h = S.out_h; src_w = S.out_w; src_c = S.d.cout; }
        const bool concat = d.concat != 0;
        if (concat && (d.skip < 0 || d.op != FD_OP_DW || !d.upsample)) FD_BAD("layer %d: concat needs an upsampled depthwise consumer with a skip tensor", i);
        if (concat) {
            L.csplit = src_c;
            if (src_c + p->layers[d.skip].d.cout != d.cin || src_c % 4) FD_BAD("layer %d: concat of %d + %d channels does not give cin %d", i, src_c, p->layers[d.skip].d.cout, d.cin);
        } else if (d.op == FD_OP_DWS) {
            if (d.src < 0 || src_c != 4 * d.cin) FD_BAD("layer %d: pixel-shuffle depthwise needs 4 * cin (%d) == producer channels %d", i, d.cin, src_c);
        } else if (d.op == FD_OP_DWB) {
            if (d.src < 0 || src_c != d.cin) FD_BAD("layer %d: bilinear depthwise (FD_OP_DWB) needs cin (%d) == producer channels %d", i, d.cin, src_c);
        } else if (src_c != d.cin) FD_BAD("layer %d: cin %d != producer channels %d", i, d.cin, src_c);
        const bool doubled_in = d.upsample || d.op == FD_OP_DWS || d.op == FD_OP_DWB;
        L.in_h = doubled_in ? 2 * src_h : src_h;
        L.in_w = doubled_in ? 2 * src_w : src_w;
        if (d.skip >= 0) {
            const Layer &S = p->layers[d.skip];
            if (!d.upsample) FD_BAD("layer %d: skip without upsample is not part of this path", i);
            if (S.out_h != L.in_h || S.out_w != L.in_w || (!concat && S.d.cout != d.cin))
                FD_BAD("layer %d: skip tensor %dx%dx%d does not match input %dx%dx%d", i, S.out_h, S.out_w, S.d.cout, L.in_h, L.in_w, d.cin);
        }
        switch (d.op) {
        case FD_OP_STEM:
            if (d.src != -1 || d.cin != 3 || d.ksize != 3 || d.stride != 2 || d.upsample || d.skip >= 0 || d.cout % 8)
                FD_BAD("layer %d: stem must be 3->8k channels, 3x3 stride 2 on the network input", i);
            L.out_h = L.in_h / 2; L.out_w = L.in_w / 2;
            L.chunk = d.cout % 32 == 0 ? 32 : (d.cout % 16 == 0 ? 16 : 8);
            if (d.cout > 64) FD_BAD("layer %d: the stem supports at most 64 output channels", i);
            {
                const int nrows = 2 * ceil_div(255, L.out_w) + 3;
                L.lds = std::max((size_t)3 * nrows * (L.in_w + 8) * 4, (size_t)4 * 64 * 36 * 4);
            }
            L.grid = dim3(ceil_div((long)L.out_h * L.out_w, 256), batch);
            L.w_bytes = (size_t)27 * d.cout * 4; L.w_elems = (size_t)27 * d.cout;
            break;
        case FD_OP_DW: {
            if (d.src < 0 || d.cin != d.cout || (d.ksize != 3 && d.ksize != 5) || (d.stride != 1 && d.stride != 2) || d.cin % 4)
                FD_BAD("layer %d: depthwise needs cin==cout (multiple of 4), k in {3,5}, stride in {1,2}", i);
            if (d.stride == 2 && (L.in_h % 2 || L.in_w % 2)) FD_BAD("layer %d: stride-2 depthwise on odd input", i);
            L.mode = d.upsample ? (d.skip >= 0 ? (concat ? 3 : 2) : 1) : 0;
            L.out_h = L.in_h / d.stride; L.out_w = L.in_w / d.stride;
            if (d.ksize == 3 && L.mode == 0) {
                L.dw_rows = true;
                L.dw_rows8 = dtype != FD_F32 && d.cin % 8 == 0 && d.stride == 1 && !(flags & FD_PLAN_NO_ROWS8);
                const int gx = ceil_div((long)L.out_w * (d.cin / (L.dw_rows8 ? 8 : 4)), 256);
                int th = L.out_h;
                while (th > 4 && (long)gx * ceil_div(L.out_h, th) * batch < 1024) th = (th + 1) / 2;
                L.th = th;
                L.grid = dim3(gx, ceil_div(L.out_h, th), batch);
                L.lds = 0;
                L.w_bytes = (size_t)9 * d.cin * 4; L.w_elems = (size_t)9 * d.cin;
                break;
            }
            if (dtype != FD_F32 && d.ksize == 5 && d.stride == 1 && L.mode == 2 && d.cin % 8 == 0 && L.out_w % 4 == 0 && L.in_h % 2 == 0 &&
                (double)L.in_h * L.in_w * d.cin * 2.0 < 2147483648.0 && !(tune & FD_TUNE_NO_DW5_ROWS)) {
                const int strips = L.out_w / 4;
                L.dw5_cl = (strips % 2 == 1 && d.cin >= 128) ? 64 : 32;
                const int cblocks = ceil_div(d.cin, 2 * L.dw5_cl);
                L.dw5_cbs = ceil_div(ceil_div(d.cin, cblocks), 8) * 8;
                L.dw5_groups = ceil_div(strips, 64 / L.dw5_cl);
                const int bands = std::max(1, (L.out_h + 7) / 14);
                L.dw5_bh = ceil_div(ceil_div(L.out_h, bands), 2) * 2;
                L.grid = dim3(ceil_div((long)L.dw5_groups * ceil_div(L.out_h, L.dw5_bh), FD_DW5R_BLOCK / 64), cblocks, batch);
                L.lds = 0;
                L.w_elems = (size_t)25 * d.cin;
                L.wpk_off = align_up((size_t)25 * d.cin * 4, 256);
                L.w_bytes = L.wpk_off + (size_t)30 * d.cin * 4;
                break;
            }
            const bool h8_ok = dtype != FD_F32 && d.cin % 8 == 0 && (!concat || L.csplit % 8 == 0) && !(tune & FD_TUNE_NO_DW_H8);
            const bool h8 = h8_ok && ((tune & FD_TUNE_FORCE_DW_H8) || (d.ksize == 5 && d.cin % 64 == 0 && (long)L.out_h * L.out_w >= 56 * 56));
            L.dw_n = h8 ? 8 : 4;
            int cb = d.cin >= 32 ? 32 : (d.cin >= 16 ? 16 : (d.cin >= 8 ? 8 : 4));
            if (h8 && d.cin >= 64 && ceil_div(d.cin, 64) * 64 <= ceil_div(d.cin, 32) * 32) cb = 64;
            L.cbq = ilog2(cb / L.dw_n);
            const int tmax_w = d.stride == 2 ? 8 : 16, tmax_h = d.ksize == 5 ? 7 : 8;
            L.tw = std::min((L.out_w + 3) / 4 * 4, tmax_w);
            L.th = std::min(L.out_h, tmax_h);
            L.tiles_x = ceil_div(L.out_w, L.tw); L.tiles_y = ceil_div(L.out_h, L.th);
            const int th_in = (L.th - 1) * d.stride + d.ksize, tw_in = (L.tw - 1) * d.stride + d.ksize;
            L.pstr = h8 ? 2 * pick_patch_pitch(cb / 2, L.tw, tw_in, d.stride) : pick_patch_pitch(cb, L.tw, tw_in, d.stride);
            L.lds = align_up((size_t)th_in * tw_in * L.pstr * (h8 ? 2 : 4), 16) + ((size_t)d.ksize * d.ksize * cb + cb) * 4;
            L.grid = dim3(L.tiles_x * L.tiles_y, ceil_div(d.cin, cb), batch);
            L.w_bytes = (size_t)d.ksize * d.ksize * d.cin * 4; L.w_elems = (size_t)d.ksize * d.ksize * d.cin;
            break;
        }
        case FD_OP_DWT: {
            if (d.src < 0 || d.cin != d.cout || (d.ksize != 3 && d.ksize != 5) || d.stride != 2 || d.upsample || d.skip >= 0 || concat || d.cin % (dtype == FD_F32 ? 4 : 8))
                FD_BAD("layer %d: transposed depthwise needs cin==cout (multiple of %d), k in {3,5}, stride 2, no upsample / skip / concat", i, dtype == FD_F32 ? 4 : 8);
            L.dwt = true;
            L.out_h = 2 * L.in_h; L.out_w = 2 * L.in_w;
            const int gx = ceil_div((long)L.in_w * (d.cin / 4), 256);
            int th = L.in_h;
            while (th > 4 && (long)gx * ceil_div(L.in_h, th) * batch < 1024) th = (th + 1) / 2;
            L.th = th;
            L.grid = dim3(gx, ceil_div(L.in_h, th), batch);
            L.lds = 0;
            L.w_bytes = (size_t)d.ksize * d.ksize * d.cin * 4; L.w_elems = (size_t)d.ksize * d.ksize * d.cin;
            break;
        }
        case FD_OP_DWS: {
            if (d.cin != d.cout || (d.ksize != 3 && d.ksize != 5) || d.stride != 1 || d.upsample || d.skip >= 0 || concat || d.cin % (dtype == FD_F32 ? 1 : 2))
                FD_BAD("layer %d: pixel-shuffle depthwise needs cin==cout (16-bit plans: a multiple of 2), k in {3,5}, stride 1, no upsample / skip / concat", i);
            L.dws = true;
            L.out_h = L.in_h; L.out_w = L.in_w;
            const int sh = L.in_h / 2, sw = L.in_w / 2;
            const int gx = ceil_div((long)sw * (d.cin / (dtype == FD_F32 ? 1 : 2)), 256);
            int th = sh;
            while (th > 4 && (long)gx * ceil_div(sh, th) * batch < 1024) th = (th + 1) / 2;
            L.th = th;
            L.grid = dim3(gx, ceil_div(sh, th), batch);
            L.lds = 0;
            L.w_bytes = (size_t)d.ksize * d.ksize * d.cin * 4; L.w_elems = (size_t)d.ksize * d.ksize * d.cin;
            break;
        }
        case FD_OP_PWS:
            if (d.src < 0 || d.ksize != 1 || d.stride != 1 || d.cin % 4 || d.cin > 64 || d.cout != 4 || d.upsample || d.skip >= 0 || concat)
                FD_BAD("layer %d: pixel-shuffle head needs k=1 stride=1, cin%%4==0, cin<=64, cout==4, no upsample / skip / concat", i);
            if (i != n_layers - 1) FD_BAD("layer %d: the pixel-shuffle head (FD_OP_PWS) is only valid as the last layer", i);
            L.pws = true;
            L.out_h = L.in_h; L.out_w = L.in_w;
            L.w_bytes = (size_t)d.cin * 4 * 4; L.w_elems = (size_t)d.cin * 4;
            L.grid = dim3(ceil_div((long)batch * L.out_h * L.out_w, 256));
            break;
        case FD_OP_DWB: {
            if (d.cin != d.cout || (d.ksize != 3 && d.ksize != 5) || d.stride != 1 || d.upsample || d.skip >= 0 || concat || d.cin % 2)
                FD_BAD("layer %d: bilinear depthwise (FD_OP_DWB) needs cin==cout (a multiple of 2), k in {3,5}, stride 1, no upsample / skip / concat", i);
            L.dwb = true;
            L.out_h = L.in_h; L.out_w = L.in_w;
            const int sh = L.in_h / 2, sw = L.in_w / 2;
            const int gx = ceil_div((long)sw * (d.cin / 2), 256);
            int th = sh;
            while (th > 4 && (long)gx * ceil_div(sh, th) * batch < 1024) th = (th + 1) / 2;
            L.th = th;
            L.grid = dim3(gx, ceil_div(sh, th), batch);
            L.lds = 0;
            L.w_bytes = (size_t)d.ksize * d.ksize * d.cin * 4; L.w_elems = (size_t)d.ksize * d.ksize * d.cin;
            break;
        }
        case FD_OP_PWB:
            if (d.src < 0 || d.ksize != 1 || d.stride != 1 || d.cin % 4 || d.cin > 64 || d.cout != 1 || d.upsample || d.skip >= 0 || concat)
                FD_BAD("layer %d: bilinear head (FD_OP_PWB) needs k=1 stride=1, cin%%4==0, cin<=64, cout==1, no upsample / skip / concat", i);
            if (i != n_layers - 1) FD_BAD("layer %d: the bilinear head (FD_OP_PWB) is only valid as the last layer", i);
            if (batch > 65535) FD_BAD("layer %d: the bilinear head (FD_OP_PWB) takes at most 65535 images per launch", i);
            L.pwb = true;
            L.out_h = 2 * L.in_h; L.out_w = 2 * L.in_w;
            L.w_bytes = (size_t)d.cin * 4; L.w_elems = (size_t)d.cin;
            L.grid = dim3(ceil_div(L.in_w, FD_HEADB_TILE), ceil_div(L.in_h, FD_HEADB_TILE), batch);
            break;
        case FD_OP_CONV: {
            const int q = dtype == FD_F32 ? 4 : 8;
            if (d.src < 0 || (d.ksize != 3 && d.ksize != 5) || d.stride != 1 || (d.upsample != 0 && d.upsample != 1) || d.skip >= 0 || concat || d.cin % q || d.cout % q)
                FD_BAD("layer %d: dense convolution (FD_OP_CONV) needs k in {3,5}, stride 1, cin and cout multiples of %d, upsample 0 or 1, no skip / concat", i, q);
            const long M = (long)batch * L.in_h * L.in_w;
            if (M >= (1L << 31) || (double)M * d.cout >= 9.0e18) FD_BAD("layer %d: dense convolution (FD_OP_CONV) over %ld output pixels exceeds the kernel's row indexing", i, M);
            L.conv = true;
            L.out_h = L.in_h; L.out_w = L.in_w;
            const int bk = fd_conv_bk(esz);
            L.cv_ktpt = ceil_div(d.cin, bk);
            if (d.cout <= 32) { L.cv_wgm = 4; L.cv_wgn = 1; L.cv_tm = 1; L.cv_tn = 1; }
            else if (d.cout >= 128 && M >= 1024) { L.cv_wgm = 2; L.cv_wgn = 2; L.cv_tm = 2; L.cv_tn = 2; }
            else { L.cv_wgm = 2; L.cv_wgn = 2; L.cv_tm = 1; L.cv_tn = 1; }
            const int bm = L.cv_wgm * L.cv_tm * 32, bn = L.cv_wgn * L.cv_tn * 32;
            L.m_tiles = ceil_div(M, bm); L.n_tiles = ceil_div(d.cout, bn);
            const int kt = d.ksize * d.ksize * L.cv_ktpt;
            const long tiles = (long)L.m_tiles * L.n_tiles;
            int splits = tiles >= 128 ? 1 : (int)std::min<long>(std::min(kt / 8, 32), 256 / tiles);
            L.cv_tps = ceil_div(kt, std::max(1, splits));
            L.cv_splits = ceil_div(kt, L.cv_tps);
            L.lds = (size_t)FD_CONV_STAGES * (bm + bn) * 128;
            L.grid = dim3((unsigned)((L.m_tiles + 7) / 8 * 8 * L.n_tiles), (unsigned)L.cv_splits);
            L.w_elems = (size_t)d.ksize * d.ksize * d.cin * d.cout;
            const size_t packed = (size_t)d.cout * kt * bk * esz;
            L.zero_off = align_up(packed, 256);
            L.w_bytes = L.zero_off + FD_CONV_ZERO_BYTES;
            if (L.cv_splits > 1) p->conv_part_bytes = std::max(p->conv_part_bytes, align_up((size_t)L.cv_splits * M * d.cout * 4, 256));
            break;
        }
        case FD_OP_PW:
            if (d.src < 0 || d.ksize != 1 || d.stride != 1 || d.cin % 4) FD_BAD("layer %d: pointwise needs k=1 stride=1 cin%%4==0", i);
            L.out_h = L.in_h; L.out_w = L.in_w;
            L.w_bytes = (size_t)d.cin * d.cout * 4;
            L.w_elems = (size_t)d.cin * d.cout;
            if (d.cout == 1) {
                if (d.skip >= 0) FD_BAD("layer %d: head with skip is not part of this path", i);
                L.head = true;
                const long npix = (long)batch * (L.in_h >> (d.upsample ? 1 : 0)) * (L.in_w >> (d.upsample ? 1 : 0));
                L.grid = dim3(ceil_div(npix * 8, 256));
            } else {
                if (d.upsample || d.skip >= 0) FD_BAD("layer %d: pointwise after upsample is only supported for the 1-channel head", i);
                const long M = (long)batch * L.out_h * L.out_w;
                if (dtype != FD_F32 && d.cin % 8) FD_BAD("layer %d: 16-bit pointwise needs cin %% 8 == 0", i);
                L.w_pitch = dtype == FD_F32 ? (d.cin + 31) / 32 * 32 : (d.cin + 63) / 64 * 64;
                L.w_bytes = (size_t)d.cout * L.w_pitch * esz;
                L.pw = dtype == FD_F32 ? choose_pw(M, d.cout) : PwCfg{2, 2, 1, 1};
                L.lds = pw_lds_bytes(L.pw);
                if (dtype != FD_F32) L.lds = (size_t)std::min(FD_H16_STAGES, ceil_div(d.cin, 64)) * 128 * 128;
                L.m_tiles = ceil_div(M, L.pw.wgm * L.pw.tm * 32);
                L.n_tiles = ceil_div(d.cout, L.pw.wgn * L.pw.tn * 32);
                L.grid = dim3((unsigned)((L.m_tiles + 7) / 8 * 8 * L.n_tiles));
                if ((dtype == FD_F32 || (tune & FD_TUNE_FORCE_GEMM16)) && !(flags & FD_PLAN_NO_GEMM16)) {
                    const Pw16Cfg c16 = choose_pw16(M, d.cout, d.cin, (tune & FD_TUNE_FORCE_GEMM16) != 0);
                    if (c16.tm) {
                        L.pw16_tm = c16.tm; L.pw16_stride = c16.stride;
                        L.pw16_breg = dtype == FD_F32 && g16_breg_pick(c16.tm, tune);
                        L.lds = dtype == FD_F32 ? g16_ring_bytes(c16.tm, L.pw16_breg != 0) : (size_t)4 * (c16.tm * 16 + 64) * 32 * 4;
                        L.m_tiles = ceil_div(M, c16.stride); L.n_tiles = ceil_div(d.cout, 64);
                        L.grid = dim3((unsigned)((L.m_tiles + 7) / 8 * 8 * L.n_tiles));
                    }
                }
            }
            break;
        default: FD_BAD("layer %d: unknown op %d", i, d.op);
        }
        if (L.lds > 160 * 1024) FD_BAD("layer %d: LDS request %zu exceeds 160 KiB", i, L.lds);
        const int big_h = std::max(L.in_h, L.out_h), big_w = std::max(L.in_w, L.out_w);
        if ((long)big_h * big_w >= (1L << 24) || d.cin >= (1 << 24) || d.cout >= (1 << 24) || (double)big_h * big_w * std::max(d.cin, d.cout) >= 4294967296.0)
            FD_BAD("layer %d: a %dx%d map with %d channels exceeds the kernels' 32-bit within-image addressing", i, big_h, big_w, std::max(d.cin, d.cout));
        L.w_off = woff; woff += align_up(L.w_bytes, 256);
        if (L.dw5_cl) L.wpk_off += L.w_off;
        if (L.conv) L.zero_off += L.w_off;
        L.b_off = woff; woff += align_up((size_t)d.cout * 4, 256);
        L.out_bytes = align_up((size_t)batch * L.out_h * L.out_w * d.cout * esz, 256);
        L.pw_packed_t = (d.op == FD_OP_PW && !L.head && dtype != FD_F32);
    }
    Layer &last = p->layers.back();
    if (last.pws ? (2 * last.out_h != height || 2 * last.out_w != width) : (last.d.cout != 1 || last.out_h != height || last.out_w != width))
        FD_BAD("the last layer must produce the [B,1,%d,%d] network output (got %dx%dx%d)", height, width, last.out_h, last.out_w, last.d.cout);
#undef FD_BAD
    last.to_output = true;
    p->weights_bytes = woff;

    *woff_out = woff;
    return FD_OK;
}

void plan_fuse_epilogues(fd_plan *p)
{
    const int n_layers = (int)p->layers.size(), batch = p->B, height = p->H, width = p->W, dtype = p->dtype;
    const uint32_t flags = p->flags, tune = p->tune;
    (void)n_layers; (void)batch; (void)height; (void)width; (void)dtype; (void)flags; (void)tune;
    if (!(flags & FD_PLAN_NO_EPILOGUE_FUSION)) {
        std::vector<int> readers(n_layers, 0);
        for (int i = 0; i < n_layers; ++i) {
            if (p->layers[i].d.src >= 0) ++readers[p->layers[i].d.src];
            if (p->layers[i].d.skip >= 0) ++readers[p->layers[i].d.skip];
        }
        for (int j = 1; j < n_layers; ++j) {
            Layer &D = p->layers[j];
            if (D.d.op != FD_OP_DW || D.d.src < 0 || D.d.skip >= 0 || D.d.concat) continue;
            if (D.d.act == FD_ACT_NONE) continue;
            Layer &Pw = p->layers[D.d.src];
            if (Pw.d.op != FD_OP_PW || Pw.head || readers[D.d.src] != 1) continue;
            const int hw = Pw.out_h * Pw.out_w;
            int tm = Pw.pw16_tm, stride = Pw.pw16_stride, m_tiles = Pw.m_tiles, n_tiles = Pw.n_tiles;
            size_t lds = Pw.lds;
            const bool want_all = (tune & FD_TUNE_FORCE_EPILOGUE_FUSION) != 0;
            const bool h16_pick = dtype != FD_F32 && !(flags & FD_PLAN_NO_GEMM16) && !(tune & FD_TUNE_FORCE_GEMM16) && hw <= 208 &&
                                  (want_all || (hw >= 128 && (long)batch * ceil_div(Pw.d.cout, 64) <= 272));
            if (h16_pick) {
                n_tiles = ceil_div(Pw.d.cout, 64);
                int f = 1;
                for (int cand : {4, 2}) if (cand * hw <= 208 && (long)ceil_div(batch, cand) * n_tiles >= 256) { f = cand; break; }
                stride = f * hw; tm = stride <= 64 ? 4 : (stride <= 112 ? 7 : 13);
                lds = (size_t)4 * (tm * 16 + 64) * 128;
                m_tiles = ceil_div((long)batch * hw, stride);
            }
            if (!tm) continue;
            if (stride % hw || D.d.cin % 4) continue;
            if (D.d.upsample && D.d.stride != 1) continue;
            {
                const int P = D.d.upsample ? (D.d.ksize / 2 + 1) / 2 : D.d.ksize / 2;
                const long img_rows = (long)(stride / hw) * (Pw.out_h + 2 * P) * (Pw.out_w + 2 * P) + 1;
                const size_t img = (size_t)img_rows * 68 * 4;
                if (img > lds) {
                    if (!Pw.pw16_breg || h16_pick || img > g16_ring_bytes(tm, false)) continue;
                    Pw.lds = img;
                }
            }
            if (h16_pick) {
                Pw.pw16_tm = tm; Pw.pw16_stride = stride; Pw.lds = lds; Pw.m_tiles = m_tiles; Pw.n_tiles = n_tiles;
                Pw.grid = dim3((unsigned)((m_tiles + 7) / 8 * 8 * n_tiles));
            }
            Pw.fuse_next_dw = j;
            D.fused_into = D.d.src;
        }
    }

}

void plan_fuse_units(fd_plan *p)
{
    const int n_layers = (int)p->layers.size(), batch = p->B, height = p->H, width = p->W, dtype = p->dtype;
    const uint32_t flags = p->flags, tune = p->tune;
    (void)n_layers; (void)batch; (void)height; (void)width; (void)dtype; (void)flags; (void)tune;
    if (dtype == FD_F32 && !(flags & FD_PLAN_NO_UNIT_FUSION) && (!(flags & FD_PLAN_KEEP_ACTIVATIONS) || (tune & FD_TUNE_FORCE_UNIT_FUSION))) {
        std::vector<int> readers(n_layers, 0);
        for (int i = 0; i < n_layers; ++i) {
            if (p->layers[i].d.src >= 0) ++readers[p->layers[i].d.src];
            if (p->layers[i].d.skip >= 0) ++readers[p->layers[i].d.skip];
        }
        for (int i = 0; i + 1 < n_layers; ++i) {
            Layer &D = p->layers[i], &Pw = p->layers[i + 1];
            if (D.d.op != FD_OP_DW || D.fused_into >= 0 || D.skipped || D.d.src < 0 || readers[i] != 1) continue;
            if (Pw.d.op != FD_OP_PW || Pw.head || Pw.d.src != i || Pw.d.upsample || Pw.fuse_next_dw >= 0 || Pw.to_output) continue;
            const int C = D.d.cin, N = Pw.d.cout, KS = D.d.ksize, S = D.d.stride;
            if (D.d.act != Pw.d.act || D.d.act == FD_ACT_NONE || C % 32 || C > 256 || N % 32) continue;
            if ((double)batch * D.in_h * D.in_w * C >= 2147483648.0 || (double)batch * D.out_h * D.out_w * N * 4.0 >= 4294967296.0) continue;
            int wm = 0, nld = 0;
            if (KS == 3 && S == 1 && D.mode == 0) { wm = 4; nld = 6; }
            else if (KS == 5 && S == 1 && D.mode == 2) { wm = 4; nld = 8; }
            else if (KS == 3 && S == 2 && D.mode == 0) { wm = 2; nld = 10; }
            else continue;
            const int wn = 4 / wm, nt = N / 32 / wn;
            if (nt * wn * 32 != N || !(nt == 1 || nt == 2 || nt == 4) || (wm == 2 && nt == 1)) continue;
            if (!(tune & FD_TUNE_FORCE_UNIT_FUSION) && (C > 64 || D.out_h * D.out_w < 28 * 28)) continue;
            const size_t lds = ((size_t)nld * 32 * 36 + 2 * 32 * wm * 32 + (size_t)N * C + (size_t)KS * KS * C + C) * 4;
            if ((C / 32) & (C / 32 - 1) || lds > 160 * 1024) continue;
            long best = -1; int bth = 0, btw = 0;
            for (int tws = 2; tws <= 5; ++tws) {
                const int tw = 1 << tws;
                if (tw > 32 * wm || (tw > 4 && tw >= 2 * D.out_w)) continue;
                for (int th = 1; th * tw <= 32 * wm && th <= D.out_h; ++th) {
                    const int ph = (th - 1) * S + KS, pw = (tw - 1) * S + KS;
                    if (ph * pw > 32 * nld) continue;
                    const long tiles = (long)ceil_div(D.out_h, th) * ceil_div(D.out_w, tw);
                    const long cost = tiles * (ph * pw + 32 * wm);
                    if (best < 0 || cost < best) { best = cost; bth = th; btw = tws; }
                }
            }
            if (best < 0) continue;
            D.skipped = true;
            Pw.fused_dw = i; Pw.dwpw = true; Pw.pw16_tm = 0;
            Pw.dp_th = bth; Pw.dp_tw = btw; Pw.dp_tiles_x = ceil_div(D.out_w, 1 << btw); Pw.dp_wm = wm; Pw.dp_nt = nt; Pw.dp_nld = nld;
            const long tiles = (long)Pw.dp_tiles_x * ceil_div(D.out_h, bth) * batch;
            Pw.dp_xcd = batch >= 8 ? 1 : 0;
            Pw.grid = dim3((unsigned)(Pw.dp_xcd ? 256 : std::min<long>(256, tiles)));
            Pw.pstr = pick_patch_pitch(32, 1 << btw, ((1 << btw) - 1) * S + KS, S, S == 2 ? 2 : 4);
            Pw.lds = lds + (size_t)nld * 32 * (Pw.pstr - 36) * 4;
            if (i + 2 < n_layers && !(flags & FD_PLAN_KEEP_ACTIVATIONS) && KS == 5 && D.mode == 2 && N == 32 && nt == 1 && wm == 4) {
                Layer &H = p->layers[i + 2];
                if (H.head && H.d.src == i + 1 && H.d.skip < 0 && readers[i + 1] == 1 && H.d.cin == 32) { Pw.fuse_head = i + 2; H.fused_into = i + 1; }
            }
        }
    }

}

void plan_fuse_head_h16(fd_plan *p)
{
    const int n_layers = (int)p->layers.size(), batch = p->B, height = p->H, width = p->W, dtype = p->dtype;
    const uint32_t flags = p->flags, tune = p->tune;
    (void)n_layers; (void)batch; (void)height; (void)width; (void)dtype; (void)flags; (void)tune;
    if (dtype != FD_F32 && !(flags & (FD_PLAN_KEEP_ACTIVATIONS | FD_PLAN_NO_EPILOGUE_FUSION))) {
        std::vector<int> rd(n_layers, 0);
        for (int i = 0; i < n_layers; ++i) {
            if (p->layers[i].d.src >= 0) ++rd[p->layers[i].d.src];
            if (p->layers[i].d.skip >= 0) ++rd[p->layers[i].d.skip];
        }
        for (int i = 0; i + 1 < n_layers; ++i) {
            Layer &Pw = p->layers[i], &H = p->layers[i + 1];
            if (Pw.d.op != FD_OP_PW || Pw.head || Pw.pw16_tm || Pw.dwpw || Pw.fuse_next_dw >= 0 || Pw.skipped || Pw.fused_into >= 0 || Pw.to_output) continue;
            if (!H.head || H.d.src != i || H.d.skip >= 0 || rd[i] != 1 || H.d.cin != Pw.d.cout || Pw.d.cout > 32 || Pw.d.cout % 8 || Pw.n_tiles != 1) continue;
            Pw.fuse_head = i + 1; H.fused_into = i;
        }
    }

}

void plan_arena(fd_plan *p, size_t woff)
{
    const int n_layers = (int)p->layers.size(), batch = p->B, height = p->H, width = p->W, dtype = p->dtype;
    const uint32_t flags = p->flags, tune = p->tune;
    (void)n_layers; (void)batch; (void)height; (void)width; (void)dtype; (void)flags; (void)tune;
    std::vector<int> last_use(n_layers, -1);
    for (int i = 0; i < n_layers; ++i) {
        if (p->layers[i].d.src >= 0) last_use[p->layers[i].d.src] = i;
        if (p->layers[i].d.skip >= 0) last_use[p->layers[i].d.skip] = i;
        if (p->layers[i].fused_dw >= 0) {
            const fd_layer_desc &dd = p->layers[p->layers[i].fused_dw].d;
            last_use[dd.src] = i;
            if (dd.skip >= 0) last_use[dd.skip] = i;
        }
    }
    FreeList fl;
    std::vector<char> released(n_layers, 0);
    for (int i = 0; i < n_layers; ++i) {
        Layer &L = p->layers[i];
        if (!(flags & FD_PLAN_KEEP_ACTIVATIONS))
            for (int j = 0; j < i; ++j)
                if (!released[j] && last_use[j] >= 0 && last_use[j] <= i - 1 && !p->layers[j].to_output && !p->layers[j].skipped) {
                    fl.release(p->layers[j].out_off - woff, p->layers[j].out_bytes);
                    released[j] = 1;
                }
        if (L.to_output || L.skipped) continue;
        if (L.fused_into >= 0) continue;
        L.out_off = woff + fl.alloc(L.out_bytes);
        if (L.fuse_next_dw >= 0) p->layers[L.fuse_next_dw].out_off = woff + fl.alloc(p->layers[L.fuse_next_dw].out_bytes);
    }
    p->conv_part_off = align_up(woff + fl.top, 256);
    p->ws_bytes = p->conv_part_bytes ? p->conv_part_off + p->conv_part_bytes : woff + fl.top;

}

void plan_describe(fd_plan *p)
{
    const int n_layers = (int)p->layers.size(), batch = p->B, height = p->H, width = p->W, dtype = p->dtype;
    const uint32_t flags = p->flags, tune = p->tune;
    (void)n_layers; (void)batch; (void)height; (void)width; (void)dtype; (void)flags; (void)tune;
    const size_t esz = dtype == FD_F32 ? 4 : 2;
    for (int i = 0; i < n_layers; ++i) {
        Layer &L = p->layers[i];
        const fd_layer_desc &d = L.d;
        const int c_src = L.csplit ? L.csplit : d.cin, c_skip = L.csplit ? d.cin - L.csplit : d.cin;
        const double src_elems = (double)batch * ((d.upsample || d.op == FD_OP_DWB) ? (L.in_h / 2) * (L.in_w / 2) : L.in_h * L.in_w) * c_src;
        const double skip_elems = d.skip >= 0 ? (double)batch * L.in_h * L.in_w * c_skip : 0.0;
        const double out_elems = (double)batch * L.out_h * L.out_w * d.cout;
        const double in_esz = d.src < 0 ? 4.0 : (double)esz, out_esz = L.to_output ? 4.0 : (double)esz;
        L.alg_bytes = (src_elems + skip_elems) * in_esz + out_elems * out_esz + (double)L.w_elems * (L.pw_packed_t ? esz : 4) + 2.0 * d.cout * 4;
        if (L.conv) L.alg_bytes = src_elems * in_esz + out_elems * out_esz + (double)L.w_elems * esz + d.cout * 4.0;
        p->alg_bytes += L.alg_bytes;
        const double taps = d.op == FD_OP_STEM ? 27.0 : ((d.op == FD_OP_DW || d.op == FD_OP_DWS || d.op == FD_OP_DWB) ? (double)d.ksize * d.ksize : (d.op == FD_OP_DWT ? d.ksize * d.ksize / 4.0 : (d.op == FD_OP_CONV ? (double)d.ksize * d.ksize * d.cin : (double)d.cin)));
        const double mac_px = L.pwb ? (double)L.in_h * L.in_w : (double)L.out_h * L.out_w;
        L.alg_flops = 2.0 * batch * mac_px * d.cout * taps;
        p->alg_flops += L.alg_flops;
        char buf[512];
        if (L.skipped)
            snprintf(buf, sizeof buf, "(fused into layer %d)", i + 1);
        else if (L.fused_into >= 0 && L.head)
            snprintf(buf, sizeof buf, "(pointwise head evaluated on the accumulators of layer %d's %s kernel)", L.fused_into, p->layers[L.fused_into].dwpw ? "dwpw" : "pw_gemm");
        else if (L.fused_into >= 0)
            snprintf(buf, sizeof buf, "(dw k%d s%d%s evaluated in the epilogue of layer %d's pw_gemm16)", d.ksize, d.stride, d.upsample ? " on up2" : "", L.fused_into);
        else if (L.dwpw)
            snprintf(buf, sizeof buf, "dwpw<dw k%d s%d mode%d + pw> persistent, 4 producer + 4 consumer waves; tile %dx%d px x all %d channels, C=%d in %d chunks, weights in LDS, grid=%u lds=%zu%s", p->layers[L.fused_dw].d.ksize,
                     p->layers[L.fused_dw].d.stride, p->layers[L.fused_dw].mode, L.dp_th, 1 << L.dp_tw, d.cout, d.cin, d.cin / 32, L.grid.x, L.lds,
                     L.fuse_head >= 0 ? " + the 32->1 head on the accumulators" : "");
        else if (d.op == FD_OP_STEM)
            snprintf(buf, sizeof buf, "stem3x3s2<mfma 32x32x2, LDS-staged rows, 256 px per workgroup> grid=%ux%u lds=%zu", L.grid.x, L.grid.y, L.lds);
        else if (d.op == FD_OP_CONV)
            snprintf(buf, sizeof buf, "conv_igemm<k%d s1%s, implicit GEMM on mfma %s, all k^2 taps (not pre-summed per parity), tile %dx%d BK %d> M=%ld N=%d K=%dx%d tiles=%dx%d split-K %d%s grid=%ux%u lds=%zu",
                     d.ksize, d.upsample ? " on up2" : "", dtype == FD_F32 ? "32x32x2 f32" : (dtype == FD_F16 ? "32x32x16 f16" : "32x32x16 bf16"), L.cv_wgm * L.cv_tm * 32, L.cv_wgn * L.cv_tn * 32,
                     fd_conv_bk(esz), (long)batch * L.out_h * L.out_w, d.cout, d.ksize * d.ksize, d.cin, L.m_tiles, L.n_tiles, L.cv_splits,
                     L.cv_splits > 1 ? " (fp32 partial tiles + fd_conv_reduce in split order)" : "", L.grid.x, L.grid.y, L.lds);
        else if (d.op == FD_OP_DWT)
            snprintf(buf, sizeof buf, "dwt_rows<k%d s2, polyphase: %d taps per 2x2 output quad, 4 channels per work-item> %d input rows per band, grid=%ux%ux%u, no LDS",
                     d.ksize, d.ksize == 5 ? 25 : 9, L.th, L.grid.x, L.grid.y, L.grid.z);
        else if (d.op == FD_OP_DWS)
            snprintf(buf, sizeof buf, "dws_rows<k%d s1 on the 2x pixel shuffle of the producer, %d output channels (16 source bytes) per work-item> %d source rows per band, grid=%ux%ux%u, no LDS",
                     d.ksize, dtype == FD_F32 ? 1 : 2, L.th, L.grid.x, L.grid.y, L.grid.z);
        else if (d.op == FD_OP_PWS)
            snprintf(buf, sizeof buf, "head_shuffle<%d -> 4, written as the 2x2 quads of the network output> grid=%u", d.cin, L.grid.x);
        else if (d.op == FD_OP_DWB)
            snprintf(buf, sizeof buf, "dwb_rows<k%d s1 on the bilinear x2 of the producer, 2 channels per work-item> %d source rows per band, grid=%ux%ux%u, no LDS",
                     d.ksize, L.th, L.grid.x, L.grid.y, L.grid.z);
        else if (d.op == FD_OP_PWB)
            snprintf(buf, sizeof buf, "head_bilinear<%d -> 1 on the %dx%d map, interpolated x2 into the network output> 16x16 source tiles, grid=%ux%ux%u", d.cin, L.in_h, L.in_w,
                     L.grid.x, L.grid.y, L.grid.z);
        else if (d.op == FD_OP_DW && L.dw5_cl)
            snprintf(buf, sizeof buf, "dw5_rows<k5 s1 mode2, pixel pairs + dot2, %d channel lanes per strip> bands of %d rows, %d strip groups, %d channels per block, grid=%ux%ux%u, no LDS",
                     L.dw5_cl, L.dw5_bh, L.dw5_groups, L.dw5_cbs, L.grid.x, L.grid.y, L.grid.z);
        else if (d.op == FD_OP_DW && L.dw_rows)
            snprintf(buf, sizeof buf, "dw3_rows%s<s%d> rows/item %d grid=%ux%ux%u", L.dw_rows8 ? "8" : "", d.stride, L.th, L.grid.x, L.grid.y, L.grid.z);
        else if (d.op == FD_OP_DW)
            snprintf(buf, sizeof buf, "dwconv<k%d s%d mode%d> tile %dx%dx%d pitch %d grid=%ux%ux%u lds=%zu, %d channels per work-item", d.ksize, d.stride, L.mode,
                     L.th, L.tw, L.dw_n << L.cbq, L.pstr, L.grid.x, L.grid.y, L.grid.z, L.lds, L.dw_n);
        else if (L.head)
            snprintf(buf, sizeof buf, "head_pw1 up=%d grid=%u", d.upsample, L.grid.x);
        else
            if (L.pw16_tm)
                snprintf(buf, sizeof buf, "pw_gemm16<TM=%d: %dx64 tile, stride %d> M=%ld N=%d K=%d tiles=%dx%d (%.2f per CU) lds=%zu%s", L.pw16_tm, L.pw16_tm * 16, L.pw16_stride,
                         (long)batch * L.out_h * L.out_w, d.cout, d.cin, L.m_tiles, L.n_tiles, L.m_tiles * L.n_tiles / 256.0, L.lds, L.pw16_breg ? ", weight fragments in registers" : ""),
                L.fuse_next_dw >= 0 ? (void)snprintf(buf + strlen(buf), sizeof buf - strlen(buf), " + fused dw k%d of layer %d", p->layers[L.fuse_next_dw].d.ksize, L.fuse_next_dw) : (void)0;
            else
            snprintf(buf, sizeof buf, "pw_gemm<%dx%d> M=%ld N=%d K=%d tiles=%dx%d lds=%zu", L.pw.wgm * L.pw.tm * 32,
                     L.pw.wgn * L.pw.tn * 32, (long)batch * L.out_h * L.out_w, d.cout, d.cin, L.m_tiles, L.n_tiles, L.lds),
            (L.fuse_head >= 0 && !L.dwpw) ? (void)snprintf(buf + strlen(buf), sizeof buf - strlen(buf), " + the %d->1 head on its output tile", d.cout) : (void)0;
        L.info = buf;
        const char *tn = dtype == FD_F32 ? "float" : (dtype == FD_F16 ? "_Float16" : "fd_bf16");
        if (L.skipped || L.fused_into >= 0) buf[0] = 0;
        else if (L.dwpw) snprintf(buf, sizeof buf, "fd_dwpw_f32<%d, %d, %d, %d, %d, %d, %d, %d, 0>", p->layers[L.fused_dw].d.ksize, p->layers[L.fused_dw].d.stride, p->layers[L.fused_dw].mode, d.act, L.dp_wm, L.dp_nt, L.dp_nld, L.fuse_head >= 0 ? 1 : 0);
        else if (d.op == FD_OP_STEM) snprintf(buf, sizeof buf, "fd_stem3x3s2<%s, %d, %d>", tn, d.act, L.chunk);
        else if (d.op == FD_OP_CONV) snprintf(buf, sizeof buf, "fd_conv_gemm<%s, %d, %d, %d, %d>", tn, L.cv_wgm, L.cv_wgn, L.cv_tm, L.cv_tn);
        else if (d.op == FD_OP_DWT) snprintf(buf, sizeof buf, "fd_dwt_rows<%s, %d, %d>", tn, d.ksize, d.act);
        else if (d.op == FD_OP_DWS) snprintf(buf, sizeof buf, "fd_dws_rows<%s, %d, %d>", tn, d.ksize, d.act);
        else if (d.op == FD_OP_PWS) snprintf(buf, sizeof buf, "fd_head_shuffle<%s, %d>", tn, d.act);
        else if (d.op == FD_OP_DWB) snprintf(buf, sizeof buf, "fd_dwb_rows<%s, %d, %d>", tn, d.ksize, d.act);
        else if (d.op == FD_OP_PWB) snprintf(buf, sizeof buf, "fd_head_bilinear<%s, %d>", tn, d.act);
        else if (d.op == FD_OP_DW && L.dw5_cl) snprintf(buf, sizeof buf, "fd_dw5_rows<%s, %d, %d>", tn, d.act, L.dw5_cl);
        else if (d.op == FD_OP_DW && L.dw_rows) snprintf(buf, sizeof buf, "fd_dw3_rows%s<%s, %d, %d>", L.dw_rows8 ? "8" : "", tn, d.stride, d.act);
        else if (d.op == FD_OP_DW) snprintf(buf, sizeof buf, "fd_dwconv<%s, %d, %d, %d, %d, %d>", tn, d.ksize, d.stride, L.mode, d.act, L.dw_n);
        else if (L.head) snprintf(buf, sizeof buf, "fd_head_pw1<%s, %d>", tn, d.act);
        else if (L.pw16_tm && dtype != FD_F32) snprintf(buf, sizeof buf, "fd_pw_gemm16_h16<%s, %d, 4, %d, %d, 1>", tn, L.pw16_tm, d.act, L.fuse_next_dw >= 0 ? p->layers[L.fuse_next_dw].d.ksize : 0);
        else if (L.pw16_tm) snprintf(buf, sizeof buf, "fd_pw_gemm16_f32<%d, %d, %d, 0, %d, 0, %d>", L.pw16_tm, FD_G16_STAGES, d.act, L.fuse_next_dw >= 0 ? p->layers[L.fuse_next_dw].d.ksize : 0, L.pw16_breg);
        else if (dtype == FD_F32) snprintf(buf, sizeof buf, "fd_pw_gemm_f32<%d, %d, %d, %d, %d>", L.pw.wgm, L.pw.wgn, L.pw.tm, L.pw.tn, d.act);
        else if (L.fuse_head >= 0) snprintf(buf, sizeof buf, "fd_pw_gemm_head_h16<%s, %d>", tn, d.act);
        else snprintf(buf, sizeof buf, "fd_pw_gemm_h16<%s, %d>", tn, d.act);
        L.sym = buf;
    }
}

}
```

### fast-depth_amd/csrc/fd_plan_select.h

```cpp
#pragma once
#ifndef FD_G16_STAGES
#define FD_G16_STAGES 4
#endif
namespace {

int pick_patch_pitch(int cb, int tw, int tw_in, int stride, int strip = 4)
{
    static const int grp[4][16] = {{0, 1, 2, 3, 12, 13, 14, 15, 20, 21, 22, 23, 24, 25, 26, 27}, {4, 5, 6, 7, 8, 9, 10, 11, 16, 17, 18, 19, 28, 29, 30, 31},
                                   {32, 33, 34, 35, 44, 45, 46, 47, 52, 53, 54, 55, 56, 57, 58, 59}, {36, 37, 38, 39, 40, 41, 42, 43, 48, 49, 50, 51, 60, 61, 62, 63}};
    const int lanes_c = cb / 4, tws = std::max(1, tw / strip);
    int cbq = 0; while ((1 << cbq) < lanes_c) ++cbq;
    int best = cb + 4; long best_cycles = -1;
    for (int pitch = cb + 4; pitch <= cb + 36; pitch += 4) {
        long cycles = 0;
        for (int wave = 0; wave < 4; ++wave)
            for (int g = 0; g < 4; ++g) {
                int first_addr[64][4], n_addr[64];
                for (int b = 0; b < 64; ++b) n_addr[b] = 0;
                for (int k = 0; k < 16; ++k) {
                    const int tid = wave * 64 + grp[g][k], c4 = tid & (lanes_c - 1), pt = tid >> cbq;
                    const int oy = pt / tws, ox = (pt - oy * tws) * strip;
                    const int addr = ((oy * stride) * tw_in + ox * stride) * pitch + c4 * 4;
                    for (int dw = 0; dw < 4; ++dw) {
                        const int b = (addr + dw) & 63;
                        bool seen = false;
                        for (int q = 0; q < n_addr[b] && q < 4; ++q) seen |= first_addr[b][q] == addr;
                        if (!seen) { if (n_addr[b] < 4) first_addr[b][n_addr[b]] = addr; ++n_addr[b]; }
                    }
                }
                int worst = 1;
                for (int b = 0; b < 64; ++b) worst = std::max(worst, n_addr[b]);
                cycles += worst;
            }
        if (best_cycles < 0 || cycles < best_cycles) { best_cycles = cycles; best = pitch; }
        if (cycles == 16) break;
    }
    return best;
}

struct PwCfg { int wgm, wgn, tm, tn; };

struct Layer {
    fd_layer_desc d;
    int in_h = 0, in_w = 0;
    int out_h = 0, out_w = 0;
    size_t out_off = 0, out_bytes = 0;
    size_t w_off = 0, w_bytes = 0, b_off = 0;
    size_t w_elems = 0;
    bool to_output = false;
    bool head = false;
    bool pw_packed_t = false;
    int cbq = 0, th = 0, tw = 0, tiles_x = 0, tiles_y = 0, mode = 0, pstr = 0;
    int dw_n = 4;
    int dw5_cl = 0, dw5_cbs = 0, dw5_groups = 0, dw5_bh = 0;
    size_t wpk_off = 0;
    int csplit = 0;
    bool skipped = false;
    int fuse_next_dw = -1;
    int fused_into = -1;
    int fused_dw = -1;
    int fuse_head = -1;
    bool dwpw = false;
    int dp_th = 0, dp_tw = 0 , dp_tiles_x = 0, dp_wm = 0, dp_nt = 0, dp_nld = 0, dp_xcd = 0;
    bool dw_rows = false;
    bool dw_rows8 = false;
    bool dwt = false;
    bool dws = false;
    bool pws = false;
    bool dwb = false;
    bool pwb = false;
    bool conv = false;
    int cv_wgm = 0, cv_wgn = 0, cv_tm = 0, cv_tn = 0;
    int cv_ktpt = 0, cv_splits = 1, cv_tps = 0;
    size_t zero_off = 0;
    int chunk = 0;
    PwCfg pw{};
    int m_tiles = 0, n_tiles = 0, w_pitch = 0;
    int pw16_tm = 0, pw16_stride = 0;
    int pw16_breg = 0;
    size_t lds = 0;
    dim3 grid;
    std::string info, sym;
    double alg_bytes = 0, alg_flops = 0;
};

}

struct fd_plan {
    std::vector<Layer> layers;
    int B = 0, H = 0, W = 0, dtype = 0;
    uint32_t flags = 0, tune = 0;
    size_t ws_bytes = 0, weights_bytes = 0;
    size_t conv_part_off = 0, conv_part_bytes = 0;
    unsigned char *ws = nullptr;
    bool packed = false;
    double alg_bytes = 0, alg_flops = 0;
};

namespace {

struct FreeList {
    std::vector<std::pair<size_t, size_t>> blocks;
    size_t top = 0;
    size_t alloc(size_t bytes)
    {
        for (size_t i = 0; i < blocks.size(); ++i)
            if (blocks[i].second >= bytes) {
                size_t off = blocks[i].first;
                blocks[i].first += bytes;
                blocks[i].second -= bytes;
                if (blocks[i].second == 0) blocks.erase(blocks.begin() + i);
                return off;
            }
        if (!blocks.empty() && blocks.back().first + blocks.back().second == top) {
            size_t off = blocks.back().first;
            top = off + bytes;
            blocks.pop_back();
            return off;
        }
        size_t off = top;
        top += bytes;
        return off;
    }
    void release(size_t off, size_t bytes)
    {
        auto it = std::lower_bound(blocks.begin(), blocks.end(), std::make_pair(off, (size_t)0));
        it = blocks.insert(it, {off, bytes});
        if (it + 1 != blocks.end() && it->first + it->second == (it + 1)->first) { it->second += (it + 1)->second; blocks.erase(it + 1); }
        if (it != blocks.begin() && (it - 1)->first + (it - 1)->second == it->first) { (it - 1)->second += it->second; blocks.erase(it); }
    }
};

PwCfg choose_pw(long M, int N)
{
    const PwCfg c128x128{2, 2, 2, 2}, c128x64{2, 2, 2, 1}, c64x128{2, 2, 1, 2}, c64x64{2, 2, 1, 1}, c128x32{4, 1, 1, 1};
    if (N <= 32) return c128x32;
    auto blocks = [&](const PwCfg &c) { return (long)ceil_div(M, c.wgm * c.tm * 32) * ceil_div(N, c.wgn * c.tn * 32); };
    auto waste = [&](const PwCfg &c) { int bn = c.wgn * c.tn * 32; return (double)(ceil_div(N, bn) * bn) / N; };
    (void)blocks; (void)waste; (void)c128x128;
    if (M > 4096 && M <= 16384 && N >= 512) return c64x128;
    if (M > 16384 && M <= 32768 && N > 32 && N <= 128) return c128x64;
    return c64x64;
}

struct Pw16Cfg { int tm = 0, stride = 0; double score = 0; };
Pw16Cfg choose_pw16(long M, int N, int K, bool force)
{
    Pw16Cfg best;
    if (N % 4 || M <= 0) return best;
    if (force) {
        best.tm = M > 112 ? 13 : (M > 64 ? 7 : 4);
        const long mt = (M + 16 * best.tm - 1) / (16 * best.tm);
        best.stride = (int)((M + mt - 1) / mt); best.score = 1.0;
        return best;
    }
    const int nt = ceil_div(N, 64);
    for (int tm : {13, 7, 4}) {
        const long mtiles = std::max<long>(1, 256 / nt);
        long stride = (M + mtiles - 1) / mtiles;
        if (stride > 16 * tm) continue;
        const long wgs = ((M + stride - 1) / stride) * nt;
        const double score = std::min(1.0, wgs / 256.0) * ((double)stride / (16 * tm));
        if (score > best.score) { best.tm = tm; best.stride = (int)stride; best.score = score; }
    }
    if (best.score < 0.72 || K < 256) best = Pw16Cfg();
    return best;
}

bool g16_breg_pick(int tm, uint32_t tune)
{
    return FD_G16_STAGES == 4 && tm != 13 && !(tune & FD_TUNE_G16_B_LDS);
}
size_t g16_ring_bytes(int tm, bool breg) { return (size_t)FD_G16_STAGES * (tm * 16 + (breg ? 0 : 64)) * 32 * 4; }

int pw_lds_bytes(const PwCfg &c) { return FD_F32_STAGES * (c.wgm * c.tm * 32 + c.wgn * c.tn * 32) * 32 * 4; }

int ilog2(int v) { int r = 0; while ((1 << r) < v) ++r; return r; }
}
```

### fast-depth_amd/csrc/fd_tuning.h

```cpp
#pragma once
#include <stdint.h>

#define FD_TUNE_WGRAD_TILE_ROWS 1u
#define FD_TUNE_FORCE_GEMM16 2u
#define FD_TUNE_FORCE_EPILOGUE_FUSION 4u
#define FD_TUNE_FORCE_UNIT_FUSION 8u
#define FD_TUNE_NO_PW_PAIRING 16u
#define FD_TUNE_PW_PAIR_TN2 32u
#define FD_TUNE_DW_BWD1 64u
#define FD_TUNE_DW_BWD_PAIR 128u
#define FD_TUNE_DW_SMALL_TILES 256u
#define FD_TUNE_DW_PITCH4 512u
#define FD_TUNE_DW_PITCH8 1024u
#define FD_TUNE_DW_WGRAD_TH4 2048u
#define FD_TUNE_DW_NO_ROWS 4096u
#define FD_TUNE_DW_FORCE_ROWS 8192u
#define FD_TUNE_DW_TH8 16384u
#define FD_TUNE_DW_CB16 32768u
#define FD_TUNE_NO_DW_H8 65536u
#define FD_TUNE_FORCE_DW_H8 131072u
#define FD_TUNE_NO_CONSUMER_FINALIZE 262144u
#define FD_TUNE_DW_BWD_FINALIZE 524288u
#define FD_TUNE_NO_DW5_ROWS 1048576u
#define FD_TUNE_G16_B_LDS 2097152u
#define FD_TUNE_ALL 4194303u

#ifdef __cplusplus
extern "C" {
#endif
void fd_tuning_next(uint32_t mask);
struct fd_train_plan;
int fd_train_plan_lds_rounding(const struct fd_train_plan *plan, int32_t layer);
int fd_train_plan_unit_kernels(const struct fd_train_plan *plan, int32_t layer);
int fd_train_plan_dw_geometry(const struct fd_train_plan *plan, int32_t layer, int32_t *out, int32_t n_out);
struct fd_comm;
void fd_comm_elide_collectives(struct fd_comm *comm, int32_t on);
int fd_comm_bind_library(const char *path);
#ifdef __cplusplus
}
#endif
```

### fast-depth_amd/fastdepth_hip/capi.py

```python
import ctypes
import os

HERE = os.path.dirname(os.path.abspath(__file__))
DEFAULT_LIB = os.path.join(HERE, "libfastdepth_hip.so")

FD_F32, FD_F16, FD_BF16 = 0, 1, 2


class _DtypeMap(dict):
    def __missing__(self, key):
        import torch
        m = {torch.float32: FD_F32, torch.float16: FD_F16, torch.bfloat16: FD_BF16}
        self.update(m)
        return m[key]


DTYPE_OF = _DtypeMap()
FD_OP_STEM, FD_OP_DW, FD_OP_PW, FD_OP_DWT, FD_OP_DWS, FD_OP_PWS, FD_OP_DWB, FD_OP_PWB, FD_OP_CONV = 0, 1, 2, 3, 4, 5, 6, 7, 8
FD_ACT_NONE, FD_ACT_RELU, FD_ACT_RELU6 = 0, 1, 2
FD_PLAN_KEEP_ACTIVATIONS = 1
FD_PLAN_NO_GEMM16 = 64
FD_PLAN_NO_ROWS8 = 256
FD_PLAN_NO_EPILOGUE_FUSION = 512
FD_PLAN_NO_UNIT_FUSION = 1024
FD_PLAN_NO_BWD_PAIRING = 4096
_TUNE_SHIFT = 32
FD_TUNE_WGRAD_TILE_ROWS = 1 << _TUNE_SHIFT
FD_TUNE_FORCE_GEMM16 = 2 << _TUNE_SHIFT
FD_TUNE_FORCE_EPILOGUE_FUSION = 4 << _TUNE_SHIFT
FD_TUNE_FORCE_UNIT_FUSION = 8 << _TUNE_SHIFT
FD_TUNE_NO_PW_PAIRING = 16 << _TUNE_SHIFT
FD_TUNE_PW_PAIR_TN2 = 32 << _TUNE_SHIFT
FD_TUNE_DW_BWD1 = 64 << _TUNE_SHIFT
FD_TUNE_DW_BWD_PAIR = 128 << _TUNE_SHIFT
FD_TUNE_DW_SMALL_TILES = 256 << _TUNE_SHIFT
FD_TUNE_DW_PITCH4 = 512 << _TUNE_SHIFT
FD_TUNE_DW_PITCH8 = 1024 << _TUNE_SHIFT
FD_TUNE_DW_WGRAD_TH4 = 2048 << _TUNE_SHIFT
FD_TUNE_DW_NO_ROWS = 4096 << _TUNE_SHIFT
FD_TUNE_DW_FORCE_ROWS = 8192 << _TUNE_SHIFT
FD_TUNE_DW_TH8 = 16384 << _TUNE_SHIFT
FD_TUNE_DW_CB16 = 32768 << _TUNE_SHIFT
FD_TUNE_NO_DW_H8 = 65536 << _TUNE_SHIFT
FD_TUNE_FORCE_DW_H8 = 131072 << _TUNE_SHIFT
FD_TUNE_NO_CONSUMER_FINALIZE = 262144 << _TUNE_SHIFT
FD_TUNE_DW_BWD_FINALIZE = 524288 << _TUNE_SHIFT
FD_TUNE_NO_DW5_ROWS = 1048576 << _TUNE_SHIFT
FD_TUNE_G16_B_LDS = 2097152 << _TUNE_SHIFT


def create_plan(lib, train, descs, n, batch, height, width, fd_dtype, flags, handle_ref):
    tuning = int(flags) >> _TUNE_SHIFT
    lib.fd_tuning_next(tuning)
    fn = lib.fd_train_plan_create if train else lib.fd_plan_create
    return fn(descs, n, batch, height, width, fd_dtype, int(flags) & 0xFFFFFFFF, handle_ref)


def parse_flags(text):
    v = 0
    for tok in str(text).replace(",", "|").split("|"):
        tok = tok.strip()
        if not tok:
            continue
        g = globals()
        if "FD_PLAN_" + tok in g:
            v |= g["FD_PLAN_" + tok]
        elif "FD_TUNE_" + tok in g:
            v |= g["FD_TUNE_" + tok]
        else:
            v |= int(tok, 0)
    return v


class LayerDesc(ctypes.Structure):
    _fields_ = [(n, ctypes.c_int32) for n in
                ("op", "cin", "cout", "ksize", "stride", "act", "src", "upsample", "skip", "concat")]


class LayerParams(ctypes.Structure):
    _fields_ = [(n, ctypes.c_void_p) for n in ("conv_weight", "bn_weight", "bn_bias", "bn_mean", "bn_var", "bn_num_batches_tracked")]


class LayerGrads(ctypes.Structure):
    _fields_ = [(n, ctypes.c_void_p) for n in ("conv_weight", "bn_weight", "bn_bias")]


class GradBucket(ctypes.Structure):
    _fields_ = [("from_layer", ctypes.c_int32), ("to_layer", ctypes.c_int32), ("grad", ctypes.c_void_p), ("numel", ctypes.c_int64), ("grad16", ctypes.c_void_p)]


class TraceRecord(ctypes.Structure):
    _fields_ = [("kernel", ctypes.c_char_p), ("layer", ctypes.c_int32), ("ms", ctypes.c_float)]


class SgdTensor(ctypes.Structure):
    _fields_ = [("param", ctypes.c_void_p), ("grad", ctypes.c_void_p), ("momentum_buf", ctypes.c_void_p), ("numel", ctypes.c_int64)]


class AugParams(ctypes.Structure):
    _fields_ = [("s", ctypes.c_double), ("angle", ctypes.c_double), ("brightness", ctypes.c_float), ("contrast", ctypes.c_float),
                ("saturation", ctypes.c_float), ("flip", ctypes.c_int32), ("order", ctypes.c_int32 * 3), ("reserved", ctypes.c_int32)]


class FastDepthError(RuntimeError):
    pass


def load(path=None):
    path = path or DEFAULT_LIB
    if not os.path.exists(path):
        raise FastDepthError("HIP extension not built: %s is missing (run `python fast-depth_amd/build.py`)" % path)
    lib = ctypes.CDLL(path)
    vp, i32, u32 = ctypes.c_void_p, ctypes.c_int32, ctypes.c_uint32
    lib.fd_plan_create.argtypes = [ctypes.POINTER(LayerDesc), i32, i32, i32, i32, i32, u32, ctypes.POINTER(vp)]
    lib.fd_plan_create.restype = ctypes.c_int
    lib.fd_tuning_next.argtypes = [u32]
    lib.fd_tuning_next.restype = None
    lib.fd_plan_destroy.argtypes = [vp]
    lib.fd_plan_destroy.restype = None
    lib.fd_plan_workspace_bytes.argtypes = [vp]
    lib.fd_plan_workspace_bytes.restype = ctypes.c_size_t
    lib.fd_plan_bind_workspace.argtypes = [vp, vp, ctypes.c_size_t]
    lib.fd_plan_bind_workspace.restype = ctypes.c_int
    lib.fd_plan_pack_weights.argtypes = [vp, ctypes.POINTER(LayerParams), i32, ctypes.c_float, vp]
    lib.fd_plan_pack_weights.restype = ctypes.c_int
    lib.fd_forward.argtypes = [vp, vp, vp, vp]
    lib.fd_forward.restype = ctypes.c_int
    lib.fd_forward_timed.argtypes = [vp, vp, vp, vp, ctypes.POINTER(ctypes.c_float), i32]
    lib.fd_forward_timed.restype = ctypes.c_int
    lib.fd_layer_output.argtypes = [vp, i32, ctypes.POINTER(vp)] + [ctypes.POINTER(i32)] * 4
    lib.fd_layer_output.restype = ctypes.c_int
    lib.fd_plan_num_kernels.argtypes = [vp]
    lib.fd_plan_num_kernels.restype = i32
    lib.fd_plan_kernel_info.argtypes = [vp, i32]
    lib.fd_plan_kernel_info.restype = ctypes.c_char_p
    lib.fd_plan_kernel_symbol.argtypes = [vp, i32]
    lib.fd_plan_kernel_symbol.restype = ctypes.c_char_p
    lib.fd_plan_algorithmic_bytes.argtypes = [vp]
    lib.fd_plan_algorithmic_bytes.restype = ctypes.c_double
    lib.fd_plan_algorithmic_flops.argtypes = [vp]
    lib.fd_plan_algorithmic_flops.restype = ctypes.c_double
    lib.fd_plan_layer_stats.argtypes = [vp, i32, ctypes.POINTER(ctypes.c_double), ctypes.POINTER(ctypes.c_double)]
    lib.fd_plan_layer_stats.restype = ctypes.c_int
    lib.fd_plan_layer_traffic.argtypes = [vp, i32, ctypes.POINTER(ctypes.c_double)]
    lib.fd_plan_layer_traffic.restype = ctypes.c_int
    if hasattr(lib, "fd_train_plan_create"):
        lib.fd_train_plan_create.argtypes = [ctypes.POINTER(LayerDesc), i32, i32, i32, i32, i32, u32, ctypes.POINTER(vp)]
        lib.fd_train_plan_create.restype = ctypes.c_int
        lib.fd_train_plan_destroy.argtypes = [vp]
        lib.fd_train_plan_destroy.restype = None
        lib.fd_train_plan_workspace_bytes.argtypes = [vp]
        lib.fd_train_plan_workspace_bytes.restype = ctypes.c_size_t
        lib.fd_train_plan_bind_workspace.argtypes = [vp, vp, ctypes.c_size_t]
        lib.fd_train_plan_bind_workspace.restype = ctypes.c_int
        lib.fd_train_forward.argtypes = [vp, ctypes.POINTER(LayerParams), i32, ctypes.c_float, ctypes.c_float, vp, vp, vp]
        lib.fd_train_forward.restype = ctypes.c_int
        lib.fd_train_layer_tensor.argtypes = [vp, i32, i32, ctypes.POINTER(vp)] + [ctypes.POINTER(i32)] * 4
        lib.fd_train_layer_tensor.restype = ctypes.c_int
    if hasattr(lib, "fd_train_backward"):
        lib.fd_train_backward.argtypes = [vp, ctypes.POINTER(LayerParams), ctypes.POINTER(LayerGrads), i32, vp, vp]
        lib.fd_train_backward.restype = ctypes.c_int
        lib.fd_train_backward_range.argtypes = [vp, ctypes.POINTER(LayerParams), ctypes.POINTER(LayerGrads), i32, vp, i32, i32, vp]
        lib.fd_train_backward_range.restype = ctypes.c_int
        lib.fd_l1_loss_scratch_bytes.argtypes = [ctypes.c_int64]
        lib.fd_l1_loss_scratch_bytes.restype = ctypes.c_size_t
        lib.fd_l1_loss.argtypes = [vp, vp, vp, vp, ctypes.c_int64, vp, vp]
        lib.fd_l1_loss.restype = ctypes.c_int
        lib.fd_l1_loss_masked.argtypes = [vp, vp, vp, vp, ctypes.c_int64, vp, vp]
        lib.fd_l1_loss_masked.restype = ctypes.c_int
        lib.fd_sgd_step.argtypes = [vp, i32, ctypes.c_int64, ctypes.c_float, ctypes.c_float, ctypes.c_float, ctypes.c_float, i32, vp]
        lib.fd_sgd_step.restype = ctypes.c_int
        lib.fd_cast_gradients.argtypes = [vp, vp, ctypes.c_int64, i32, vp]
        lib.fd_cast_gradients.restype = ctypes.c_int
        lib.fd_comm_unique_id.argtypes = [vp]
        lib.fd_comm_unique_id.restype = ctypes.c_int
        lib.fd_comm_create.argtypes = [vp, i32, i32, ctypes.POINTER(vp)]
        lib.fd_comm_create.restype = ctypes.c_int
        lib.fd_comm_destroy.argtypes = [vp]
        lib.fd_comm_destroy.restype = None
        lib.fd_train_backward_allreduce.argtypes = [vp, ctypes.POINTER(LayerParams), ctypes.POINTER(LayerGrads), i32, vp, vp, ctypes.POINTER(GradBucket), i32, vp]
        lib.fd_train_backward_allreduce.restype = ctypes.c_int
        lib.fd_comm_last_exchange_ms.argtypes = [vp, ctypes.POINTER(ctypes.c_float), ctypes.POINTER(ctypes.c_float)]
        lib.fd_comm_last_exchange_ms.restype = ctypes.c_int
    lib.fd_val_transform.argtypes = [vp, vp, i32, i32, i32, i32, i32, vp, vp, vp, vp, vp]
    lib.fd_val_transform.restype = ctypes.c_int
    lib.fd_train_transform_scratch_bytes.argtypes = [i32, i32, i32]
    lib.fd_train_transform_scratch_bytes.restype = ctypes.c_size_t
    lib.fd_train_transform.argtypes = [vp, vp, i32, i32, i32, i32, i32, vp, vp, vp, vp, vp]
    lib.fd_train_transform.restype = ctypes.c_int
    lib.fd_depth_rows_scratch_bytes.argtypes = [i32]
    lib.fd_depth_rows_scratch_bytes.restype = ctypes.c_size_t
    lib.fd_depth_rows.argtypes = [vp, vp, vp, vp, i32, i32, i32, vp, vp, ctypes.c_int64, vp, vp]
    lib.fd_depth_rows.restype = ctypes.c_int
    lib.fd_depth_metrics_scratch_bytes.argtypes = []
    lib.fd_depth_metrics_scratch_bytes.restype = ctypes.c_size_t
    lib.fd_depth_metrics.argtypes = [vp, vp, ctypes.c_int64, vp, vp, vp]
    lib.fd_depth_metrics.restype = ctypes.c_int
    lib.fd_depth_metrics_frames_scratch_bytes.argtypes = [i32]
    lib.fd_depth_metrics_frames_scratch_bytes.restype = ctypes.c_size_t
    lib.fd_depth_metrics_frames.argtypes = [vp, vp, i32, ctypes.c_int64, vp, vp, vp]
    lib.fd_depth_metrics_frames.restype = ctypes.c_int
    lib.fd_plan_export_bytes.argtypes = [vp]
    lib.fd_plan_export_bytes.restype = ctypes.c_size_t
    lib.fd_plan_export.argtypes = [vp, vp, ctypes.c_size_t, vp]
    lib.fd_plan_export.restype = ctypes.c_int
    lib.fd_plan_import.argtypes = [vp, ctypes.c_size_t, i32, ctypes.POINTER(vp)]
    lib.fd_plan_import.restype = ctypes.c_int
    lib.fd_plan_import_weights.argtypes = [vp, vp, ctypes.c_size_t, vp]
    lib.fd_plan_import_weights.restype = ctypes.c_int
    lib.fd_plan_shape.argtypes = [vp] + [ctypes.POINTER(i32)] * 4
    lib.fd_plan_shape.restype = ctypes.c_int
    lib.fd_trace_begin.argtypes = []
    lib.fd_trace_begin.restype = ctypes.c_int
    lib.fd_trace_end.argtypes = [vp, ctypes.POINTER(TraceRecord), i32, ctypes.POINTER(i32)]
    lib.fd_trace_end.restype = ctypes.c_int
    lib.fd_last_error.restype = ctypes.c_char_p
    lib.fd_version.restype = ctypes.c_char_p
    return lib


EXPORTS = ("fd_plan_create", "fd_plan_destroy", "fd_plan_workspace_bytes", "fd_plan_bind_workspace",
           "fd_plan_pack_weights", "fd_forward", "fd_forward_timed", "fd_layer_output", "fd_plan_num_kernels", "fd_plan_kernel_info", "fd_plan_kernel_symbol",
           "fd_plan_algorithmic_bytes", "fd_plan_algorithmic_flops", "fd_plan_layer_stats", "fd_plan_layer_traffic",
           "fd_train_plan_create", "fd_train_plan_destroy", "fd_train_plan_workspace_bytes", "fd_train_plan_bind_workspace",
           "fd_train_forward", "fd_train_backward", "fd_train_backward_range", "fd_train_layer_tensor", "fd_l1_loss_scratch_bytes",
           "fd_l1_loss", "fd_l1_loss_masked", "fd_sgd_step", "fd_cast_gradients", "fd_comm_unique_id", "fd_comm_create", "fd_comm_destroy",
           "fd_train_backward_allreduce", "fd_comm_last_exchange_ms", "fd_val_transform", "fd_train_transform_scratch_bytes", "fd_train_transform",
           "fd_depth_rows_scratch_bytes", "fd_depth_rows",
           "fd_depth_metrics_scratch_bytes", "fd_depth_metrics",
           "fd_depth_metrics_frames_scratch_bytes", "fd_depth_metrics_frames", "fd_plan_export_bytes", "fd_plan_export",
           "fd_plan_import", "fd_plan_import_weights", "fd_plan_shape", "fd_trace_begin", "fd_trace_end", "fd_last_error", "fd_version")


def check(lib, rc, what):
    if rc != 0:
        raise FastDepthError("%s failed (%d): %s" % (what, rc, lib.fd_last_error().decode()))
```

Baseline: 42840 frames/s.

## Run 512x512 pointwise GEMM as split-bf16 x3 MFMA with producer-written planes

Adds a split-bf16 GEMM form for the fp32 pointwise gemm16 kernel. The fused depthwise producer writes its output as hi/mid/lo bf16 planes, and the weights are pre-split into three planes at pack time. A new K-loop then drives bf16 16x16x32 MFMAs over those planes in place of the fp32 matrix path. The default picker enables this only for the M=6272, 512x512 layer. It aims to use the higher bf16 matrix throughput while keeping near-fp32 accuracy, at the cost of 3x operand bytes, extra split work in the epilogue and a different LDS ring.

Result: faster. 45160 frames/s (median of 6 runs) (+5.4%).

```diff
diff --git a/fast-depth_amd/csrc/fd_api.hip b/fast-depth_amd/csrc/fd_api.hip
--- a/fast-depth_amd/csrc/fd_api.hip
+++ b/fast-depth_amd/csrc/fd_api.hip
@@ -61,6 +61,7 @@
     plan_fuse_epilogues(p);
     plan_fuse_units(p);
     plan_fuse_head_h16(p);
+    plan_pick_x3(p);
     plan_arena(p, woff);
     plan_describe(p);
     *out_plan = p;
@@ -125,6 +126,13 @@
                                reinterpret_cast<float *>(plan->ws + L.w_off), bptr, L.d.cout, inner, transpose, pitch);
         int rc = check_launch("fd_pack_fold");
         if (rc) return rc;
+        if (L.wx3_off) {
+            const long n = (long)L.d.cout * L.w_pitch;
+            hipLaunchKernelGGL(fd_pack_x3_planes, dim3(ceil_div(n, 256)), dim3(256), 0, s, reinterpret_cast<const float *>(plan->ws + L.w_off),
+                               reinterpret_cast<unsigned short *>(plan->ws + L.wx3_off), n);
+            rc = check_launch("fd_pack_x3_planes");
+            if (rc) return rc;
+        }
         if (L.dwt || L.dws || L.pws || L.dwb || L.pwb) {
             hipLaunchKernelGGL(fd_dwt_fold_bias, dim3(ceil_div(L.d.cout, 256)), dim3(256), 0, s, q.bn_weight, q.bn_bias, q.bn_mean, q.bn_var, bn_eps, bptr, L.d.cout);
             rc = check_launch("fd_dwt_fold_bias");
@@ -191,6 +199,31 @@
     return FD_OK;
 }
 
+int fd_plan_x3_tensors(const fd_plan *plan, int32_t layer, const void **out, int64_t *dims)
+{
+    if (!plan || !plan->ws || !out || !dims || layer < 0 || layer >= (int)plan->layers.size()) return -1;
+    const Layer &L = plan->layers[layer];
+    for (int i = 0; i < 5; ++i) { out[i] = nullptr; dims[i] = 0; }
+    if (L.out_x3) {
+        out[0] = plan->ws + L.x3_off;
+        if (plan->flags & FD_PLAN_KEEP_ACTIVATIONS) out[1] = plan->ws + L.out_off;
+        dims[0] = (int64_t)plan->B * L.out_h * L.out_w; dims[1] = (L.d.cout + 31) / 32 * 32;
+    }
+    if (L.wx3_off) {
+        out[2] = plan->ws + L.wx3_off; out[3] = plan->ws + L.w_off; out[4] = plan->ws + L.b_off;
+        dims[2] = L.d.cout; dims[3] = L.w_pitch; dims[4] = L.pw16_x3;
+    }
+    return 0;
+}
+
+int fd_plan_run_gemm16_layer(fd_plan *plan, int32_t layer, void *stream)
+{
+    if (!plan || !plan->ws || !plan->packed || !(plan->flags & FD_PLAN_KEEP_ACTIVATIONS) || layer < 0 || layer >= (int)plan->layers.size()) return -1;
+    const Layer &L = plan->layers[layer];
+    if (L.d.op != FD_OP_PW || !L.pw16_tm || L.head || L.dwpw || L.skipped || L.fused_into >= 0 || L.to_output || L.fuse_head >= 0 || L.d.src < 0) return -1;
+    return run_layer(plan, L, nullptr, nullptr, static_cast<hipStream_t>(stream));
+}
+
 int32_t fd_plan_num_kernels(const fd_plan *plan) { return plan ? (int32_t)plan->layers.size() : 0; }
 
 const char *fd_plan_kernel_info(const fd_plan *plan, int32_t layer)
@@ -234,6 +267,8 @@
         b += D.alg_bytes - ((plan->flags & FD_PLAN_KEEP_ACTIVATIONS) ? 1.0 : 2.0) * out_b(L);
     }
     if (L.fuse_head >= 0) { const Layer &H = plan->layers[L.fuse_head]; b += H.alg_bytes - 2.0 * out_b(L); }
+    if (L.pw16_x3) b += 2.0 * ((double)plan->B * L.out_h * L.out_w * L.d.cin + (double)L.w_elems);
+    if (L.fuse_next_dw >= 0 && plan->layers[L.fuse_next_dw].out_x3) b += out_b(plan->layers[L.fuse_next_dw]) * ((plan->flags & FD_PLAN_KEEP_ACTIVATIONS) ? 1.5 : 0.5);
     *needed_bytes = b;
     return FD_OK;
 }
diff --git a/fast-depth_amd/csrc/fd_device.h b/fast-depth_amd/csrc/fd_device.h
--- a/fast-depth_amd/csrc/fd_device.h
+++ b/fast-depth_amd/csrc/fd_device.h
@@ -151,6 +151,24 @@
     return __builtin_bit_cast(unsigned, __builtin_convertvector(v, fd_bf16x2_hw));
 }
 #endif
+#ifdef FD_EMU
+inline fd_f32x4 fd_mfma_bf16_16x16x32(fd_u16x8 a, fd_u16x8 b, fd_f32x4 c) { return hipemu_mfma_f32_16x16x32_bf16(a, b, c); }
+#else
+__device__ __forceinline__ fd_f32x4 fd_mfma_bf16_16x16x32(fd_u16x8 a, fd_u16x8 b, fd_f32x4 c)
+{
+    typedef __bf16 fd_bf16x8_mfma __attribute__((ext_vector_type(8)));
+    return __builtin_amdgcn_mfma_f32_16x16x32_bf16(__builtin_bit_cast(fd_bf16x8_mfma, a), __builtin_bit_cast(fd_bf16x8_mfma, b), c, 0, 0, 0);
+}
+#endif
+__device__ __forceinline__ void fd_split3_bf16x2(float a, float b, unsigned &hi, unsigned &mid, unsigned &lo)
+{
+    hi = fd_f32x2_to_bf16x2(a, b);
+    const bool fa = (hi & 0x7f80u) != 0x7f80u, fb = (hi & 0x7f800000u) != 0x7f800000u;
+    float ra = fa ? a - fd_bf16_to_f32((unsigned short)hi) : 0.0f, rb = fb ? b - fd_bf16_to_f32((unsigned short)(hi >> 16)) : 0.0f;
+    mid = fd_f32x2_to_bf16x2(ra, rb);
+    ra -= fd_bf16_to_f32((unsigned short)mid); rb -= fd_bf16_to_f32((unsigned short)(mid >> 16));
+    lo = fd_f32x2_to_bf16x2(ra, rb);
+}
 __device__ __forceinline__ fd_f32x4 fd_ld4(const fd_half *p)
 {
     const fd_f16x4 h = *reinterpret_cast<const fd_f16x4 *>(p);
diff --git a/fast-depth_amd/csrc/fd_infer_launch.h b/fast-depth_amd/csrc/fd_infer_launch.h
--- a/fast-depth_amd/csrc/fd_infer_launch.h
+++ b/fast-depth_amd/csrc/fd_infer_launch.h
@@ -150,6 +150,28 @@
             fz.hi = D.d.act == FD_ACT_RELU6 ? 6.0f : __builtin_inff();
             fz.store_pw = (plan->flags & FD_PLAN_KEEP_ACTIVATIONS) ? 1 : 0;
             fdw = D.d.ksize;
+            if (D.out_x3) {
+                fz.planes = reinterpret_cast<unsigned short *>(plan->ws + D.x3_off);
+                fz.pM = (long)plan->B * D.out_h * D.out_w; fz.pK32 = (D.d.cout + 31) / 32 * 32;
+                if (!(plan->flags & FD_PLAN_KEEP_ACTIVATIONS)) fz.out = nullptr;
+            }
+        }
+        if (L.pw16_x3) {
+            const float *Ap = reinterpret_cast<const float *>(plan->ws + plan->layers[L.d.src].x3_off), *Wp = reinterpret_cast<const float *>(plan->ws + L.wx3_off);
+#define FD_PW16_X3_LAUNCH(TMV, SV, FD_) \
+        do { (void)hipFuncSetAttribute((const void *)fd_pw_gemm16_f32<TMV, SV, ACT, 0, FD_, 0, 0, FD_G16_X3_FORM>, hipFuncAttributeMaxDynamicSharedMemorySize, (int)L.lds); \
+             FD_LAUNCH((fd_pw_gemm16_f32<TMV, SV, ACT, 0, FD_, 0, 0, FD_G16_X3_FORM>), L.grid, dim3(512), L.lds, s, Ap, Wp, bias, out, (int)M, N, K, L.w_pitch, L.pw16_stride, L.m_tiles, L.n_tiles, fz, fd_g16_train{}); } while (0)
+#define FD_PW16_X3_CASE(TMV, SV) \
+    case TMV: if (fdw == 3) FD_PW16_X3_LAUNCH(TMV, SV, 3); else if (fdw == 5) FD_PW16_X3_LAUNCH(TMV, SV, 5); else FD_PW16_X3_LAUNCH(TMV, SV, 0); break;
+            switch (L.pw16_tm) {
+                FD_PW16_X3_CASE(13, 3)
+                FD_PW16_X3_CASE(7, 4)
+                FD_PW16_X3_CASE(4, 4)
+            default: return fail(FD_ERR_INVALID, "no split-bf16 gemm16 instance for TM=%d", L.pw16_tm);
+            }
+#undef FD_PW16_X3_CASE
+#undef FD_PW16_X3_LAUNCH
+            return check_launch("fd_pw_gemm16_f32");
         }
         constexpr int BR = FD_G16_STAGES == 4 ? 1 : 0;
 #define FD_PW16_LAUNCH(TMV, FD_, BREGV) \
diff --git a/fast-depth_amd/csrc/fd_kernels_gemm16_f32.h b/fast-depth_amd/csrc/fd_kernels_gemm16_f32.h
--- a/fast-depth_amd/csrc/fd_kernels_gemm16_f32.h
+++ b/fast-depth_amd/csrc/fd_kernels_gemm16_f32.h
@@ -1,6 +1,7 @@
 #pragma once
 #include "fd_device.h"
 #include "fd_bn_stats.h"
+#include "fd_kernels_gemm16_x3.h"
 
 struct fd_dwfuse {
     const float *w;
@@ -10,7 +11,23 @@
     int S, up;
     float hi;
     int store_pw;
+    unsigned short *planes;
+    long pM;
+    int pK32;
 };
+
+__device__ __forceinline__ void fd_x3_store4(unsigned short *planes, long pM, long m, int c, fd_f32x4 v)
+{
+    typedef unsigned fd_u32x2_ __attribute__((ext_vector_type(2)));
+    unsigned h0, m0, l0, h1, m1, l1;
+    fd_split3_bf16x2(v.x, v.y, h0, m0, l0);
+    fd_split3_bf16x2(v.z, v.w, h1, m1, l1);
+    unsigned short *p = planes + ((long)(c >> 5) * 3 * pM + m) * 32 + (c & 31);
+    const fd_u32x2_ vh = {h0, h1}, vm = {m0, m1}, vl = {l0, l1};
+    *reinterpret_cast<fd_u32x2_ *>(p) = vh;
+    *reinterpret_cast<fd_u32x2_ *>(p + pM * 32) = vm;
+    *reinterpret_cast<fd_u32x2_ *>(p + 2 * pM * 32) = vl;
+}
 
 #ifdef FD_GEMM16_PROBE
 __device__ long long fd_gemm16_probe[8 * 4096];
@@ -25,7 +42,7 @@
     fd_bn_fin fin;
 };
 
-template <int TM, int STAGES, int ACT, int ABL = 0, int FDW = 0, int TRAIN = 0, int BREG = 0>
+template <int TM, int STAGES, int ACT, int ABL = 0, int FDW = 0, int TRAIN = 0, int BREG = 0, int X3 = 0>
 __global__ void __launch_bounds__(512)
 fd_pw_gemm16_f32(const float *__restrict__ A, const float *__restrict__ Wt, const float *__restrict__ bias,
                  float *__restrict__ out, int M, int N, int K, int K32, int m_stride, int m_tiles, int n_tiles, const fd_dwfuse fz, const fd_g16_train tr)
@@ -33,7 +50,9 @@
     static_assert(TRAIN == 0 || (FDW == 0 && ACT == 0), "train mode: raw output, no fused consumer");
     static_assert(BREG == 0 || (STAGES == 4 && (ABL == 0 || ABL == 4) && TRAIN == 0), "the register ring of the weight fragments is written for 4 stages, inference only (and has no K-loop ablations)");
     constexpr int BM = TM * 16, BN = 64, BK = 32, ROWS = BM + (BREG ? 0 : BN);
-    constexpr int STAGE = ROWS * BK;
+    static_assert(X3 == 0 || X3 == 13, "one split-bf16 form is built");
+    static_assert(X3 == 0 || (BREG == 0 && TRAIN == 0 && (ABL == 0 || ABL == 4)), "the split-bf16 form is inference only and has no K-loop ablations");
+    constexpr int STAGE = X3 ? fd_g16_x3_geom<TM, STAGES>::STAGE_B / 4 : ROWS * BK;
     constexpr int NG = ROWS / 8;
     constexpr int RG = (NG + 3) / 4;
     constexpr int OP = BN + 4;
@@ -173,7 +192,14 @@
 #endif
     };
 
-    if constexpr (BREG != 0) {
+    if constexpr (X3 != 0) {
+        long long *stamp = nullptr;
+#ifdef FD_GEMM16_PROBE
+        stamp = &pc1;
+#endif
+        fd_g16_x3_kloop<TM, STAGES>(reinterpret_cast<const unsigned char *>(A), reinterpret_cast<const unsigned char *>(Wt), smem_raw, acc,
+                                                                   m0, n0, M, N, K32, stamp);
+    } else if constexpr (BREG != 0) {
         auto run = [&](auto role) __attribute__((always_inline)) {
             constexpr bool LEAD = decltype(role)::value != 0;
             auto rest = [&](int t0) __attribute__((always_inline)) {
@@ -347,7 +373,14 @@
         constexpr int PD = KD / 2;
         const int cg = tid & 15, pl = tid >> 4;
         const int c = n0 + cg * 4;
-        if (c >= N) return;
+        if (c >= N) {
+            if (fz.planes && c < fz.pK32) {
+                const int HWp = ((fH << us) / fz.S) * ((fW << us) / fz.S);
+                for (int fr = 0; fr < frames; ++fr)
+                    for (int op = pl; op < HWp; op += 32) fd_x3_store4(fz.planes, fz.pM, (m0 / fHW + fr) * HWp + op, c, fd_zero4());
+            }
+            return;
+        }
         fd_f32x4 wv[KD * KD];
 #pragma unroll
         for (int t = 0; t < KD * KD; ++t) wv[t] = fd_ld4(fz.w + (long)t * N + c);
@@ -379,7 +412,8 @@
                 fd_f32x4 r4;
                 r4.x = fd_relu_clamp(a4.x, fz.hi); r4.y = fd_relu_clamp(a4.y, fz.hi);
                 r4.z = fd_relu_clamp(a4.z, fz.hi); r4.w = fd_relu_clamp(a4.w, fz.hi);
-                fd_st4(fz.out + ((f0 + fr) * HWo + op) * N + c, r4);
+                if (fz.out) fd_st4(fz.out + ((f0 + fr) * HWo + op) * N + c, r4);
+                if (fz.planes) fd_x3_store4(fz.planes, fz.pM, (f0 + fr) * HWo + op, c, r4);
                 ox += dx; oy += dy;
                 if (ox >= Wo) { ox -= Wo; ++oy; }
             }
diff --git a/fast-depth_amd/csrc/fd_kernels_gemm16_x3.h b/fast-depth_amd/csrc/fd_kernels_gemm16_x3.h
--- /dev/null
+++ b/fast-depth_amd/csrc/fd_kernels_gemm16_x3.h
@@ -0,0 +1,178 @@
+#pragma once
+#include "fd_device.h"
+
+__device__ __forceinline__ int fd_g16_x3_swz(int q) { return (0x78 >> (2 * q)) & 3; }
+
+static __global__ void __launch_bounds__(256) fd_pack_x3_planes(const float *__restrict__ wf, unsigned short *__restrict__ planes, long total)
+{
+    const long idx = (long)blockIdx.x * 256 + threadIdx.x;
+    if (idx >= total) return;
+    const float w = wf[idx];
+    const unsigned u = __builtin_bit_cast(unsigned, w);
+    unsigned short q[3] = {(unsigned short)(u >> 16), 0, 0};
+    if ((u & 0x7f800000u) != 0x7f800000u && w != 0.0f) {
+        float r = w - fd_bf16_to_f32(q[0]);
+        q[1] = (unsigned short)(__builtin_bit_cast(unsigned, r) >> 16);
+        r -= fd_bf16_to_f32(q[1]);
+        q[2] = (unsigned short)(__builtin_bit_cast(unsigned, r) >> 16);
+        const unsigned short filler = (unsigned short)(((u >> 16) & 0x8000u) | 0x0380u);
+#pragma unroll
+        for (int i = 0; i < 3; ++i) if ((q[i] & 0x7fffu) == 0) q[i] = filler;
+    }
+#pragma unroll
+    for (int i = 0; i < 3; ++i) planes[(long)i * total + idx] = q[i];
+}
+
+template <int TM, int STAGES> struct fd_g16_x3_geom {
+    static constexpr int BM = TM * 16, BN = 64;
+    static constexpr int RT = 3 * (BM + BN);
+    static constexpr int STAGE_B = RT * 64;
+    static constexpr int NP = RT / 16;
+    static constexpr size_t ring_bytes = (size_t)STAGES * STAGE_B;
+};
+
+template <int TM, int STAGES>
+__device__ __forceinline__ void fd_g16_x3_kloop(const unsigned char *__restrict__ Ap, const unsigned char *__restrict__ Wp, unsigned char *ring, fd_f32x4 (&acc_io)[TM],
+                                                long m0, int n0, int M, int N, int K32, long long *stamp)
+{
+    static_assert(STAGES == 3 || STAGES == 4, "the landed-tile waits are written for 3 or 4 stages");
+    typedef fd_g16_x3_geom<TM, STAGES> G;
+    constexpr int BM = G::BM, STAGE_B = G::STAGE_B, NP = G::NP;
+    constexpr int NLW = 4;
+    constexpr int RG = (NP + NLW - 1) / NLW;
+    constexpr int NPL = 1;
+    const int tid = threadIdx.x, lane = tid & 63, wave = tid >> 6, wn = wave & 3;
+    const bool leader = wave < 4;
+    const int w_u = FD_UNIFORM(wn);
+    const int T = K32 / 32;
+    fd_f32x4 acc[TM];
+#pragma unroll
+    for (int i = 0; i < TM; ++i) acc[i] = acc_io[i];
+
+    unsigned src_off[RG];
+    const int csrc = ((lane & 3) ^ fd_g16_x3_swz((lane >> 4) & 3)) * 16, r16 = lane >> 2;
+#pragma unroll
+    for (int i = 0; i < RG; ++i) {
+        int g = w_u + NLW * i;
+        if (g >= NP) g = w_u;
+        if (g < 3 * TM) {
+            const int p = g / TM, it = g - p * TM;
+            long row = m0 + it * 16 + r16;
+            if (row > M - 1) row = M - 1;
+            src_off[i] = (unsigned)(((long)p * M + row) * 64 + csrc);
+        } else {
+            const int gw = g - 3 * TM, p = gw >> 2;
+            int colw = n0 + (gw & 3) * 16 + r16;
+            if (colw > N - 1) colw = N - 1;
+            src_off[i] = (unsigned)(((long)p * N + colw) * (K32 * 2) + csrc);
+        }
+    }
+    const size_t a_tstride = (size_t)3 * M * 64;
+    auto piece = [&](int t, int i) {
+        int g = w_u + NLW * i;
+        if (g >= NP) g = w_u;
+        const unsigned char *base = g < 3 * TM ? Ap + (size_t)t * a_tstride : Wp + (size_t)t * 64;
+        fd_glds16(reinterpret_cast<const float *>(base + src_off[i]), reinterpret_cast<float *>(ring + (t % STAGES) * STAGE_B + g * 1024));
+    };
+    auto wait_landed = [&](int k) {
+        const int younger = (k + STAGES - 2 < T - 1 ? k + STAGES - 2 : T - 1) - k;
+        if (younger >= 2) fd_wait_vmcnt<2 * RG>(); else if (younger == 1) fd_wait_vmcnt<RG>(); else fd_wait_vmcnt<0>();
+    };
+
+    const int fo = (lane & 15) * 64 + (((lane >> 4) ^ fd_g16_x3_swz((lane & 15) >> 2)) << 4);
+    const int wo = (3 * BM + wn * 16) * 64 + fo;
+    auto ld_a = [&](const unsigned char *st, int p, int i) { return *reinterpret_cast<const fd_u16x8 *>(st + (p * BM + i * 16) * 64 + fo); };
+    auto ld_w = [&](const unsigned char *st, int p) { return *reinterpret_cast<const fd_u16x8 *>(st + p * (64 * 64) + wo); };
+
+    if (leader) {
+#pragma unroll
+        for (int s = 0; s < STAGES - 1; ++s)
+            if (s < T) {
+#pragma unroll
+                for (int i = 0; i < RG; ++i) piece(s, i);
+            }
+        fd_u16x8 fa[2][TM], fw[2][NPL];
+        wait_landed(0);
+        fd_block_barrier();
+        if (STAGES - 1 < T) {
+#pragma unroll
+            for (int i = 0; i < RG; ++i) piece(STAGES - 1, i);
+        }
+#pragma unroll
+        for (int i = 0; i < TM; ++i) fa[0][i] = ld_a(ring, 0, i);
+#pragma unroll
+        for (int p = 0; p < NPL; ++p) fw[0][p] = ld_w(ring, p);
+#ifdef FD_GEMM16_PROBE
+        if (stamp && tid == 0) *stamp = clock64();
+#else
+        (void)stamp;
+#endif
+#ifndef FD_EMU
+        __builtin_amdgcn_s_setprio(1);
+#endif
+        auto mfmas = [&](auto par, const unsigned char *nx, int k, bool do_dma, bool do_frags) __attribute__((always_inline)) {
+            constexpr int P = decltype(par)::value, NM = NPL * TM, NL = RG + TM + NPL;
+#pragma unroll
+            for (int idx = 0; idx < NM; ++idx) {
+                const int p = idx / TM, i = idx % TM;
+                acc[i] = fd_mfma_bf16_16x16x32(fa[P][i], fw[P][p], acc[i]);
+#pragma unroll
+                for (int l = idx * NL / NM; l < (idx + 1) * NL / NM; ++l) {
+                    if (l < RG) { if (do_dma) piece(k + STAGES - 1, l); }
+                    else if (l < RG + TM) { if (do_frags) fa[1 - P][l - RG] = ld_a(nx, 0, l - RG); }
+                    else { if (do_frags) fw[1 - P][l - RG - TM] = ld_w(nx, l - RG - TM); }
+                }
+            }
+        };
+        auto lstep = [&](auto par, int k) __attribute__((always_inline)) {
+            wait_landed(k);
+            fd_block_barrier_lds();
+            mfmas(par, ring + (k % STAGES) * STAGE_B, k, k + STAGES - 1 < T, true);
+        };
+        for (int k = 1; k < T; k += 2) {
+            lstep(fd_int<0>{}, k);
+            if (k + 1 < T) lstep(fd_int<1>{}, k + 1);
+        }
+        if ((T - 1) & 1) mfmas(fd_int<1>{}, ring, 0, false, false); else mfmas(fd_int<0>{}, ring, 0, false, false);
+#ifndef FD_EMU
+        __builtin_amdgcn_s_setprio(0);
+#endif
+    } else {
+        fd_u16x8 fb[2][TM], wq[2][3];
+        fd_block_barrier();
+#pragma unroll
+        for (int i = 0; i < TM; ++i) fb[0][i] = ld_a(ring, 0, i);
+#pragma unroll
+        for (int p = 0; p < 3; ++p) wq[0][p] = ld_w(ring, p);
+        auto fstep = [&](auto par, int k) __attribute__((always_inline)) {
+            constexpr int P = decltype(par)::value;
+            const unsigned char *cur = ring + (k % STAGES) * STAGE_B, *nx = ring + ((k + 1) % STAGES) * STAGE_B;
+            const bool more = k + 1 < T;
+#pragma unroll
+            for (int idx = 0; idx < 2 * TM; ++idx) {
+                const int i = idx % TM;
+                acc[i] = fd_mfma_bf16_16x16x32(fb[P][i], wq[P][idx < TM ? 1 : 2], acc[i]);
+                if (idx & 1) fb[1 - P][idx >> 1] = ld_a(cur, 1, idx >> 1);
+            }
+#pragma unroll
+            for (int idx = 0; idx < 2 * TM; ++idx) {
+                const int i = idx % TM;
+                acc[i] = fd_mfma_bf16_16x16x32(fb[1 - P][i], wq[P][idx < TM ? 0 : 1], acc[i]);
+                if (idx & 1) fb[P][idx >> 1] = ld_a(cur, 2, idx >> 1);
+            }
+            if (more) fd_block_barrier_lds();
+#pragma unroll
+            for (int idx = 0; idx < TM; ++idx) {
+                acc[idx] = fd_mfma_bf16_16x16x32(fb[P][idx], wq[P][0], acc[idx]);
+                if (more) fb[1 - P][idx] = ld_a(nx, 0, idx);
+                if (more && idx < 3) wq[1 - P][idx] = ld_w(nx, idx);
+            }
+        };
+        for (int k = 0; k < T; k += 2) {
+            fstep(fd_int<0>{}, k);
+            if (k + 1 < T) fstep(fd_int<1>{}, k + 1);
+        }
+    }
+#pragma unroll
+    for (int i = 0; i < TM; ++i) acc_io[i] = acc[i];
+}
diff --git a/fast-depth_amd/csrc/fd_plan_build.h b/fast-depth_amd/csrc/fd_plan_build.h
--- a/fast-depth_amd/csrc/fd_plan_build.h
+++ b/fast-depth_amd/csrc/fd_plan_build.h
@@ -211,6 +211,10 @@
                 if (dtype != FD_F32 && d.cin % 8) FD_BAD("layer %d: 16-bit pointwise needs cin %% 8 == 0", i);
                 L.w_pitch = dtype == FD_F32 ? (d.cin + 31) / 32 * 32 : (d.cin + 63) / 64 * 64;
                 L.w_bytes = (size_t)d.cout * L.w_pitch * esz;
+                if (dtype == FD_F32) {
+                    L.wx3_off = align_up(L.w_bytes, 256);
+                    L.w_bytes = L.wx3_off + (size_t)d.cout * L.w_pitch * 6;
+                }
                 L.pw = dtype == FD_F32 ? choose_pw(M, d.cout) : PwCfg{2, 2, 1, 1};
                 L.lds = pw_lds_bytes(L.pw);
                 if (dtype != FD_F32) L.lds = (size_t)std::min(FD_H16_STAGES, ceil_div(d.cin, 64)) * 128 * 128;
@@ -237,6 +241,7 @@
             FD_BAD("layer %d: a %dx%d map with %d channels exceeds the kernels' 32-bit within-image addressing", i, big_h, big_w, std::max(d.cin, d.cout));
         L.w_off = woff; woff += align_up(L.w_bytes, 256);
         if (L.dw5_cl) L.wpk_off += L.w_off;
+        if (L.wx3_off) L.wx3_off += L.w_off;
         if (L.conv) L.zero_off += L.w_off;
         L.b_off = woff; woff += align_up((size_t)d.cout * 4, 256);
         L.out_bytes = align_up((size_t)batch * L.out_h * L.out_w * d.cout * esz, 256);
@@ -386,6 +391,40 @@
 
 }
 
+void plan_pick_x3(fd_plan *p)
+{
+    if (p->dtype != FD_F32) return;
+    const int n_layers = (int)p->layers.size();
+    const bool keep = (p->flags & FD_PLAN_KEEP_ACTIVATIONS) != 0;
+    std::vector<int> readers(n_layers, 0);
+    for (int i = 0; i < n_layers; ++i) {
+        if (p->layers[i].d.src >= 0) ++readers[p->layers[i].d.src];
+        if (p->layers[i].d.skip >= 0) ++readers[p->layers[i].d.skip];
+    }
+    for (int i = 0; i < n_layers; ++i) {
+        Layer &L = p->layers[i];
+        if (L.d.op != FD_OP_PW || L.head || L.dwpw || !L.pw16_tm || L.d.src < 0) continue;
+        Layer &D = p->layers[L.d.src];
+        if (D.d.op != FD_OP_DW || D.fused_into < 0 || (readers[L.d.src] != 1 && !keep)) continue;
+        const long M = (long)p->B * L.out_h * L.out_w;
+        if (!g16_x3_pick(L.pw16_tm, M, L.d.cout, L.d.cin, p->tune)) continue;
+        if ((double)M * 3 * 64 >= 4294967296.0) continue;
+        size_t lds = g16_x3_ring_bytes(L.pw16_tm), fixed = 4;
+        if (L.fuse_next_dw >= 0) {
+            const Layer &C = p->layers[L.fuse_next_dw];
+            const int P = C.d.upsample ? (C.d.ksize / 2 + 1) / 2 : C.d.ksize / 2;
+            const long img_rows = (long)(L.pw16_stride / (L.out_h * L.out_w)) * (L.out_h + 2 * P) * (L.out_w + 2 * P) + 1;
+            lds = std::max(lds, (size_t)img_rows * 68 * 4);
+            fixed = (size_t)L.pw16_tm * 16 * 4;
+        }
+        if (lds + fixed > 160 * 1024) continue;
+        L.pw16_x3 = 1; L.pw16_breg = 0; L.lds = lds;
+        D.out_x3 = true;
+        D.x3_bytes = align_up((size_t)M * L.w_pitch * 6, 256);
+        if (!keep) D.out_bytes = D.x3_bytes;
+    }
+}
+
 void plan_arena(fd_plan *p, size_t woff)
 {
     const int n_layers = (int)p->layers.size(), batch = p->B, height = p->H, width = p->W, dtype = p->dtype;
@@ -414,7 +453,11 @@
         if (L.to_output || L.skipped) continue;
         if (L.fused_into >= 0) continue;
         L.out_off = woff + fl.alloc(L.out_bytes);
-        if (L.fuse_next_dw >= 0) p->layers[L.fuse_next_dw].out_off = woff + fl.alloc(p->layers[L.fuse_next_dw].out_bytes);
+        if (L.fuse_next_dw >= 0) {
+            Layer &D = p->layers[L.fuse_next_dw];
+            D.out_off = woff + fl.alloc(D.out_bytes);
+            if (D.out_x3) D.x3_off = (flags & FD_PLAN_KEEP_ACTIVATIONS) ? woff + fl.alloc(D.x3_bytes) : D.out_off;
+        }
     }
     p->conv_part_off = align_up(woff + fl.top, 256);
     p->ws_bytes = p->conv_part_bytes ? p->conv_part_off + p->conv_part_bytes : woff + fl.top;
@@ -509,7 +552,7 @@
         else if (d.op == FD_OP_DW) snprintf(buf, sizeof buf, "fd_dwconv<%s, %d, %d, %d, %d, %d>", tn, d.ksize, d.stride, L.mode, d.act, L.dw_n);
         else if (L.head) snprintf(buf, sizeof buf, "fd_head_pw1<%s, %d>", tn, d.act);
         else if (L.pw16_tm && dtype != FD_F32) snprintf(buf, sizeof buf, "fd_pw_gemm16_h16<%s, %d, 4, %d, %d, 1>", tn, L.pw16_tm, d.act, L.fuse_next_dw >= 0 ? p->layers[L.fuse_next_dw].d.ksize : 0);
-        else if (L.pw16_tm) snprintf(buf, sizeof buf, "fd_pw_gemm16_f32<%d, %d, %d, 0, %d, 0, %d>", L.pw16_tm, FD_G16_STAGES, d.act, L.fuse_next_dw >= 0 ? p->layers[L.fuse_next_dw].d.ksize : 0, L.pw16_breg);
+        else if (L.pw16_tm) snprintf(buf, sizeof buf, "fd_pw_gemm16_f32<%d, %d, %d, 0, %d, 0, %d, %d>", L.pw16_tm, L.pw16_x3 ? g16_x3_stages(L.pw16_tm) : FD_G16_STAGES, d.act, L.fuse_next_dw >= 0 ? p->layers[L.fuse_next_dw].d.ksize : 0, L.pw16_breg, L.pw16_x3 ? FD_G16_X3_FORM : 0);
         else if (dtype == FD_F32) snprintf(buf, sizeof buf, "fd_pw_gemm_f32<%d, %d, %d, %d, %d>", L.pw.wgm, L.pw.wgn, L.pw.tm, L.pw.tn, d.act);
         else if (L.fuse_head >= 0) snprintf(buf, sizeof buf, "fd_pw_gemm_head_h16<%s, %d>", tn, d.act);
         else snprintf(buf, sizeof buf, "fd_pw_gemm_h16<%s, %d>", tn, d.act);
diff --git a/fast-depth_amd/csrc/fd_plan_select.h b/fast-depth_amd/csrc/fd_plan_select.h
--- a/fast-depth_amd/csrc/fd_plan_select.h
+++ b/fast-depth_amd/csrc/fd_plan_select.h
@@ -78,6 +78,10 @@
     int m_tiles = 0, n_tiles = 0, w_pitch = 0;
     int pw16_tm = 0, pw16_stride = 0;
     int pw16_breg = 0;
+    int pw16_x3 = 0;
+    size_t wx3_off = 0;
+    bool out_x3 = false;
+    size_t x3_off = 0, x3_bytes = 0;
     size_t lds = 0;
     dim3 grid;
     std::string info, sym;
@@ -171,6 +175,15 @@
 {
     return FD_G16_STAGES == 4 && tm != 13 && !(tune & FD_TUNE_G16_B_LDS);
 }
+#define FD_G16_X3_FORM 13
+int g16_x3_stages(int tm) { return tm == 13 ? 3 : 4; }
+size_t g16_x3_ring_bytes(int tm) { return (size_t)g16_x3_stages(tm) * 3 * (tm * 16 + 64) * 64; }
+bool g16_x3_pick(int tm, long m, int n, int k, uint32_t tune)
+{
+    if (tune & FD_TUNE_NO_G16_X3) return false;
+    if (tune & FD_TUNE_FORCE_G16_X3) return true;
+    return tm == 13 && m == 6272 && n == 512 && k == 512;
+}
 size_t g16_ring_bytes(int tm, bool breg) { return (size_t)FD_G16_STAGES * (tm * 16 + (breg ? 0 : 64)) * 32 * 4; }
 
 int pw_lds_bytes(const PwCfg &c) { return FD_F32_STAGES * (c.wgm * c.tm * 32 + c.wgn * c.tn * 32) * 32 * 4; }
diff --git a/fast-depth_amd/csrc/fd_tuning.h b/fast-depth_amd/csrc/fd_tuning.h
--- a/fast-depth_amd/csrc/fd_tuning.h
+++ b/fast-depth_amd/csrc/fd_tuning.h
@@ -23,12 +23,17 @@
 #define FD_TUNE_DW_BWD_FINALIZE 524288u
 #define FD_TUNE_NO_DW5_ROWS 1048576u
 #define FD_TUNE_G16_B_LDS 2097152u
-#define FD_TUNE_ALL 4194303u
+#define FD_TUNE_FORCE_G16_X3 4194304u
+#define FD_TUNE_NO_G16_X3 8388608u
+#define FD_TUNE_ALL 16777215u
 
 #ifdef __cplusplus
 extern "C" {
 #endif
 void fd_tuning_next(uint32_t mask);
+struct fd_plan;
+int fd_plan_x3_tensors(const struct fd_plan *plan, int32_t layer, const void **out, int64_t *dims);
+int fd_plan_run_gemm16_layer(struct fd_plan *plan, int32_t layer, void *stream);
 struct fd_train_plan;
 int fd_train_plan_lds_rounding(const struct fd_train_plan *plan, int32_t layer);
 int fd_train_plan_unit_kernels(const struct fd_train_plan *plan, int32_t layer);
diff --git a/fast-depth_amd/fastdepth_hip/capi.py b/fast-depth_amd/fastdepth_hip/capi.py
--- a/fast-depth_amd/fastdepth_hip/capi.py
+++ b/fast-depth_amd/fastdepth_hip/capi.py
@@ -47,6 +47,8 @@
 FD_TUNE_DW_BWD_FINALIZE = 524288 << _TUNE_SHIFT
 FD_TUNE_NO_DW5_ROWS = 1048576 << _TUNE_SHIFT
 FD_TUNE_G16_B_LDS = 2097152 << _TUNE_SHIFT
+FD_TUNE_FORCE_G16_X3 = 4194304 << _TUNE_SHIFT
+FD_TUNE_NO_G16_X3 = 8388608 << _TUNE_SHIFT
 
 
 def create_plan(lib, train, descs, n, batch, height, width, fd_dtype, flags, handle_ref):
@@ -130,6 +132,10 @@
     lib.fd_forward_timed.restype = ctypes.c_int
     lib.fd_layer_output.argtypes = [vp, i32, ctypes.POINTER(vp)] + [ctypes.POINTER(i32)] * 4
     lib.fd_layer_output.restype = ctypes.c_int
+    lib.fd_plan_x3_tensors.argtypes = [vp, i32, ctypes.POINTER(vp), ctypes.POINTER(ctypes.c_int64)]
+    lib.fd_plan_x3_tensors.restype = ctypes.c_int
+    lib.fd_plan_run_gemm16_layer.argtypes = [vp, i32, vp]
+    lib.fd_plan_run_gemm16_layer.restype = ctypes.c_int
     lib.fd_plan_num_kernels.argtypes = [vp]
     lib.fd_plan_num_kernels.restype = i32
     lib.fd_plan_kernel_info.argtypes = [vp, i32]
```
